# limacv/VideoLoop3D

Hardware: AMD Instinct MI355X
Metric: rendered Mpix/s (fwd+bwd) D=32 planes 720p (higher is better)
Workload: dtype f32; 1 GPU; cfg3 stage-2 MPV render fwd+bwd: D=32 planes, T=50 frames, 720x1280, mpv convention, plane stack (D,T,H,W,4) f32 resident in HBM; parallelism=single GPU, variant=0

## Files before the change

### include/vl3d.h

```cpp
#ifndef VL3D_H
#define VL3D_H

#include <stdint.h>

#ifdef __cplusplus
extern "C" {
#endif

typedef void *vl3d_stream_t;

enum { VL3D_OK = 0, VL3D_EINVAL = 1, VL3D_ELAUNCH = 2, VL3D_EUNSUPPORTED = 3 };

enum { VL3D_ACT_NONE = 0, VL3D_ACT_SIGMOID = 1, VL3D_ACT_RELU = 2, VL3D_ACT_CLAMP = 3, VL3D_ACT_ABS = 4 };
enum { VL3D_COORD_UTILS_MPI = 0, VL3D_COORD_AFFINE = 1, VL3D_COORD_AFFINE_PLANES = 2 };
enum { VL3D_BORDER_ZEROS = 0, VL3D_BORDER_HARDCUT = 1 };
enum { VL3D_ACT_PRE = 0, VL3D_ACT_POST = 1, VL3D_ACT_BAKED = 2 };
enum { VL3D_F32 = 0, VL3D_F16 = 1, VL3D_U8 = 2 };

const char *vl3d_last_error(void);
int vl3d_version(void);

typedef struct vl3d_render_desc {
    int32_t D, T, Hs, Ws;
    int32_t H, W;
    int32_t row0, col0;
    int32_t coord_mode, border_mode, act_order, rgb_act, alpha_act;
    int32_t stack_dtype;
    float pixel_center;
    float sx, sy, ox, oy;
    int32_t variant;
    int32_t cull_row0, cull_col0, cull_Hs, cull_Ws;
    int32_t grad_flags;
    uint32_t uv_noise_seed;
} vl3d_render_desc;
enum { VL3D_GRAD_CULLED_UNWRITTEN = 1 };

int vl3d_render_fwd(const vl3d_render_desc *desc, const void *stack, const float *homos, const uint8_t *quad_keep, int32_t QH, int32_t QW,
                    void *cull_scratch, float *rgb, float *alpha, float *alpha_sums, vl3d_stream_t stream);
int vl3d_render_fwd_frames(const vl3d_render_desc *desc, const void *stack, int32_t frame0, int32_t T_alloc, const float *homos,
                           const uint8_t *quad_keep, int32_t QH, int32_t QW, void *cull_scratch, float *rgb, float *alpha,
                           vl3d_stream_t stream);

typedef struct vl3d_baked_frames {
    int32_t frame0;
    int32_t n_cams;
    const int32_t *frame_cam, *frame_t;
} vl3d_baked_frames;
typedef struct vl3d_baked_out {
    float *rgb, *alpha;
    uint8_t *frames;
    int32_t channels;
    const float *bg;
} vl3d_baked_out;
typedef struct vl3d_baked_times {
    int32_t n_cams;
    int32_t reserved;
    const int32_t *frame_cam;
    const float *frame_time;
} vl3d_baked_times;
int vl3d_bake_rgba8(int64_t n_texels, const void *stack, int32_t stack_dtype, int32_t rgb_act, int32_t alpha_act, uint8_t *out,
                    vl3d_stream_t stream);
int64_t vl3d_render_path_cull_scratch_bytes(const vl3d_render_desc *desc, int32_t n_cams);
int vl3d_render_fwd_baked(const vl3d_render_desc *desc, const uint8_t *baked, int32_t T_alloc, const float *homos,
                          const vl3d_baked_frames *sel, const uint8_t *quad_keep, int32_t QH, int32_t QW, void *cull_scratch,
                          const vl3d_baked_out *out, vl3d_stream_t stream);
int vl3d_render_fwd_baked_pool(const vl3d_render_desc *desc, const int32_t *blocks, const uint8_t *pool, int32_t T_model, const float *homos,
                               const vl3d_baked_frames *sel, const uint8_t *quad_keep, int32_t QH, int32_t QW, uint32_t culled_rgba8,
                               void *cull_scratch, const vl3d_baked_out *out, vl3d_stream_t stream);
int vl3d_render_fwd_baked_times(const vl3d_render_desc *desc, const uint8_t *baked, int32_t T_alloc, const float *homos,
                                const vl3d_baked_times *sel, const uint8_t *quad_keep, int32_t QH, int32_t QW, void *cull_scratch,
                                const vl3d_baked_out *out, vl3d_stream_t stream);
int vl3d_render_fwd_baked_pool_times(const vl3d_render_desc *desc, const int32_t *blocks, const uint8_t *pool, int32_t T_model,
                                     const float *homos, const vl3d_baked_times *sel, const uint8_t *quad_keep, int32_t QH, int32_t QW,
                                     uint32_t culled_rgba8, void *cull_scratch, const vl3d_baked_out *out, vl3d_stream_t stream);

int vl3d_pool_from_atlas_rgba8(int32_t D, int32_t T, int32_t Hs, int32_t Ws, int32_t th, int32_t tw, int32_t QH, int32_t QW,
                               const int32_t *blocks, const int32_t *tile_src, const uint8_t *static_atlas, int32_t As_h, int32_t As_w,
                               const uint8_t *dyn_atlas, int32_t Ad_h, int32_t Ad_w, int32_t frame, uint32_t culled_rgba8, uint8_t *pool,
                               vl3d_stream_t stream);

int64_t vl3d_baked_trim_scratch_bytes(int32_t D, int32_t Hs, int32_t Ws);
int vl3d_baked_trim_classify(int32_t D, int32_t T, int32_t Hs, int32_t Ws, const int32_t *blocks, const uint8_t *pool, int64_t n_slots,
                             uint32_t culled_rgba8, void *scratch, int64_t scratch_bytes, int32_t *block_slots, uint8_t *texel_class,
                             vl3d_stream_t stream);
int vl3d_baked_trim_move(int32_t D, int32_t T, int32_t Hs, int32_t Ws, const int32_t *blocks, const uint8_t *pool, int64_t n_slots,
                         const int32_t *new_blocks, uint8_t *new_pool, int64_t new_n_slots, vl3d_stream_t stream);

int64_t vl3d_render_bwd_scratch_bytes(const vl3d_render_desc *desc);
int vl3d_render_bwd(const vl3d_render_desc *desc, const void *stack, const float *homos, const uint8_t *quad_keep, int32_t QH, int32_t QW,
                    const float *rgb, const float *alpha, const float *grad_rgb, const float *grad_alpha, const float *grad_reg,
                    const void *reg_state, const float *grad_alpha_sums, float *grad_stack, void *scratch, int64_t scratch_bytes,
                    vl3d_stream_t stream);

enum { VL3D_BWD_ENTRY_RENDER = 0, VL3D_BWD_ENTRY_MASK = 1, VL3D_BWD_ENTRY_ADAM = 2 };
enum { VL3D_BWD_ATOMICS = 0, VL3D_BWD_TILE = 1, VL3D_BWD_PAIR = 2, VL3D_BWD_PAIR12 = 3 };
typedef struct vl3d_bwd_choice {
    int32_t family;
    int32_t width, rows;
    int32_t reg, mask, adam, cull, f16;
    int32_t owner4;
    int32_t gather9;
} vl3d_bwd_choice;
int vl3d_render_bwd_choice(const vl3d_render_desc *desc, int32_t entry, int32_t has_quad_keep, int32_t has_reg_grads, int64_t scratch_bytes,
                           int32_t fused_step, vl3d_bwd_choice *out);

int64_t vl3d_render_cull_scratch_bytes(const vl3d_render_desc *desc);

int vl3d_render_fwd_plane_rows(const vl3d_render_desc *desc, const void *stack, const int32_t *plane_row0, int32_t R, const float *homos,
                               float *rgb, float *alpha, vl3d_stream_t stream);
int64_t vl3d_render_plane_rows_scratch_bytes(const vl3d_render_desc *desc, int32_t R);
int vl3d_render_bwd_plane_rows(const vl3d_render_desc *desc, const void *stack, const int32_t *plane_row0, int32_t R, const float *homos,
                               const float *rgb, const float *alpha, const float *grad_rgb, const float *grad_alpha, void *grad_stack,
                               void *scratch, int64_t scratch_bytes, vl3d_stream_t stream);

int vl3d_tie_static_grad(int32_t D, int32_t T, int32_t Hs, int32_t Ws, const uint8_t *quad_keep, const uint8_t *quad_dyn,
                         int32_t QH, int32_t QW, float *grad, int32_t mode, vl3d_stream_t stream);

int vl3d_adam_step_tiles(int32_t D, int32_t T, int32_t Hs, int32_t Ws, const uint8_t *quad_keep, const uint8_t *quad_dyn, int32_t QH, int32_t QW,
                         float *param, const float *grad, float *exp_avg, float *exp_avg_sq, float lr, float beta1, float beta2,
                         float eps, int64_t step, vl3d_stream_t stream);

int32_t vl3d_adam_window_tile(void);
typedef struct vl3d_adam_window {
    int32_t D, T;
    int32_t Hs, Ws;
    int32_t y0, x0, wh, ww;
    float *param, *exp_avg, *exp_avg_sq;
    int32_t *last_step;
    const float *hist;
    float lr, beta1, beta2, eps;
    int64_t step;
    const int32_t *plane_boxes;
    void *boxes_scratch;
    const uint8_t *quad_keep, *quad_dyn;
    int32_t QH, QW;
    void *class_scratch;
    const int32_t *blocks;
} vl3d_adam_window;
int vl3d_adam_window_catchup(const vl3d_adam_window *w, int32_t upto, float *compact, float culled_alpha, int32_t mirror_static,
                             vl3d_stream_t stream);
int vl3d_adam_window_step(const vl3d_adam_window *w, const float *grad_compact, int32_t static_tied, vl3d_stream_t stream);
int vl3d_adam_flush_older(const vl3d_adam_window *w, int32_t upto, int32_t min_depth, vl3d_stream_t stream);
void vl3d_adam_step_scalars(float lr, float beta1, float beta2, int64_t step, float *lr_bc1, float *bc2s);

int64_t vl3d_render_bwd_adam_class_bytes(const vl3d_render_desc *desc);
int vl3d_render_bwd_adam(const vl3d_render_desc *desc, const void *stack, const float *homos, const float *rgb, const float *alpha,
                         const float *grad_rgb, const float *grad_alpha, const float *grad_reg, const void *reg_state,
                         const float *grad_alpha_sums, float *grad_stack, void *scratch, int64_t scratch_bytes,
                         const vl3d_adam_window *adam, vl3d_stream_t stream);

int vl3d_packed_unpack_frames(int32_t D, int32_t T, int32_t Hs, int32_t Ws, const int32_t *blocks, const float *pool, int32_t n,
                              const int32_t *frames, float culled_alpha, float *out, vl3d_stream_t stream);
int vl3d_render_fwd_packed(const vl3d_render_desc *desc, const int32_t *blocks, const float *pool, const int32_t *frames, int32_t n,
                           const float *homos, const uint8_t *quad_keep, int32_t QH, int32_t QW, float culled_alpha, float *rgb,
                           float *alpha, vl3d_stream_t stream);

int64_t vl3d_render_reg_state_bytes(const vl3d_render_desc *desc);
int vl3d_render_reg_fwd(const vl3d_render_desc *desc, const void *stack, const float *homos, const uint8_t *quad_keep, int32_t QH, int32_t QW,
                        double *sums, void *reg_state, vl3d_stream_t stream);
int vl3d_render_fwd_reg(const vl3d_render_desc *desc, const void *stack, const float *homos, const uint8_t *quad_keep, int32_t QH, int32_t QW,
                        float *rgb, float *alpha, float *alpha_sums, double *sums, void *reg_state, vl3d_stream_t stream);

int vl3d_render_fwd_mask(const vl3d_render_desc *desc, const void *stack, const float *mask, const float *homos, float *rgb,
                         float *alpha, float *label, float *alpha_sums, double *sums, void *reg_state, vl3d_stream_t stream);
int vl3d_render_bwd_mask(const vl3d_render_desc *desc, const void *stack, const float *mask, const float *homos, const float *rgb,
                         const float *alpha, const float *grad_rgb, const float *grad_alpha, const float *grad_label,
                         const float *grad_reg, const void *reg_state, const float *grad_alpha_sums, float *grad_stack,
                         float *grad_mask, void *scratch, int64_t scratch_bytes, vl3d_stream_t stream);

int vl3d_label_noise_fwd(const vl3d_render_desc *desc, const float *stack, const float *mask, const float *homos, float *label, vl3d_stream_t stream);
int vl3d_label_noise_bwd(const vl3d_render_desc *desc, const float *stack, const float *mask, const float *homos, const float *grad_label,
                         float *grad_mask, vl3d_stream_t stream);

int vl3d_warp_fwd(int32_t N, int32_t C, int32_t Hs, int32_t Ws, int32_t h, int32_t w,
                  const float *homos, const float *images, float *out, vl3d_stream_t stream);
int vl3d_warp_bwd(int32_t N, int32_t C, int32_t Hs, int32_t Ws, int32_t h, int32_t w,
                  const float *homos, const float *grad_out, float *grad_images, vl3d_stream_t stream);

int vl3d_overcompose_fwd(int64_t P, int32_t D, int32_t C, const float *alpha, const float *content,
                         float *rgb, float *blendweight, vl3d_stream_t stream);
int vl3d_overcompose_bwd(int64_t P, int32_t D, int32_t C, const float *alpha, const float *content,
                         const float *grad_rgb, const float *grad_bw,
                         float *grad_alpha, float *grad_content, vl3d_stream_t stream);

int vl3d_overcompose_nto0_fwd(int32_t B, int32_t D, int32_t C, int64_t HW,
                              const float *alpha, int64_t a_sb, int64_t a_sd,
                              const float *content, int64_t c_sb, int64_t c_sd, int64_t c_sc,
                              float *rgb, float *trans, vl3d_stream_t stream);
int vl3d_overcompose_nto0_bwd(int32_t B, int32_t D, int32_t C, int64_t HW,
                              const float *alpha, int64_t a_sb, int64_t a_sd,
                              const float *content, int64_t c_sb, int64_t c_sd, int64_t c_sc,
                              const float *grad_rgb, float *grad_alpha, float *grad_content,
                              vl3d_stream_t stream);

typedef struct vl3d_loss_desc {
    int32_t Tx, Ty, H, W;
    int32_t ps, pt, stride, stridet;
    int32_t use_alpha;
    float alpha;
    int64_t x_sc, x_st, x_sr;
    int64_t y_sc, y_st, y_sr;
    int32_t variant;
} vl3d_loss_desc;

int64_t vl3d_patchnn_scratch_bytes(const vl3d_loss_desc *desc);

enum { VL3D_NN_ENTRY_PLAIN = 0, VL3D_NN_ENTRY_PREPARED = 1, VL3D_NN_ENTRY_GRAMS = 2 };
enum { VL3D_NN_LAYOUT_GRAM16 = 1, VL3D_NN_LAYOUT_PIXEL_MAJOR = 2 };
typedef struct vl3d_nn_choice {
    int32_t kernel;
    int32_t tyt, nl, nw, xs, ch;
    int32_t runsum;
    int32_t threads;
    int32_t kc;
    int32_t lds_bytes;
    int32_t scratch_layout;
} vl3d_nn_choice;
int vl3d_patchnn_choice(const vl3d_loss_desc *desc, int32_t entry, int32_t has_scratch, int32_t x_pitch, int32_t x_frames, int32_t y_pitch,
                        vl3d_nn_choice *out);
typedef struct vl3d_fold_choice {
    int32_t staged;
    int32_t shape;
    int32_t fw, fh, threads;
    int32_t nb;
    int32_t lds_bytes;
} vl3d_fold_choice;
int vl3d_vote_fold_choice(const vl3d_loss_desc *desc, int32_t fused, vl3d_fold_choice *out);

int vl3d_patchnn(const vl3d_loss_desc *desc, const float *x, const float *y, int32_t *nn,
                 void *scratch, vl3d_stream_t stream);

int64_t vl3d_gram_major_bytes(int32_t T, int32_t H, int32_t W);
int vl3d_video_to_gram_major(const float *y, int64_t sc, int64_t st, int64_t sr, int32_t T, int32_t H, int32_t W, float *out,
                             vl3d_stream_t stream);
int vl3d_patchnn_prepared(const vl3d_loss_desc *desc, const float *x, const float *y_gram, int32_t y_pitch, int32_t y_rows,
                          int32_t y_row0, int32_t y_col0, int32_t *nn, void *scratch, vl3d_stream_t stream);
int vl3d_patchnn_grams(const vl3d_loss_desc *desc, const float *x_gram, int32_t x_pitch, int32_t x_rows, int32_t x_frames, const float *y_gram,
                       int32_t y_pitch, int32_t y_rows, int32_t y_row0, int32_t y_col0, int32_t *nn, vl3d_stream_t stream);

int vl3d_nn_vectors(int64_t B, int32_t n1, int32_t n2, int32_t d, const float *X, const float *Y,
                    int32_t use_alpha, float alpha, int64_t *nn, vl3d_stream_t stream);

int vl3d_vote_fold(const vl3d_loss_desc *desc, const float *y, const int32_t *nn,
                   float *sum, float *weight, int32_t normalize, vl3d_stream_t stream);

int vl3d_patch_l1(const vl3d_loss_desc *desc, const float *x, const float *y, const int32_t *nn, float *err,
                  vl3d_stream_t stream);

int vl3d_vote_fold_robust(const vl3d_loss_desc *desc, const float *y, const int32_t *nn, const float *x, int32_t rho_kind,
                          float rou, float scale, float *y2x, float *weight, float *grad_x, double *loss_sum,
                          vl3d_stream_t stream);

int vl3d_vote_fold_robust_strided(const vl3d_loss_desc *desc, const float *y, const int32_t *nn, const float *x, int32_t rho_kind,
                                  float rou, float scale, float *y2x, float *weight, float *grad_x, int64_t gx_sc, int64_t gx_st,
                                  int64_t gx_sr, double *loss_sum, vl3d_stream_t stream);

int vl3d_scale_inplace(int64_t n, float *x, const float *scale, vl3d_stream_t stream);

int vl3d_loop_gain(int32_t T, int32_t F, int32_t h, int32_t w, const float *rgb, const float *res, double *log_sum, vl3d_stream_t stream);
int vl3d_loop_gain_strided(int32_t T, int32_t F, int32_t h, int32_t w, const float *rgb, const float *res, int64_t r_sf, int64_t r_sc, int64_t r_sr,
                           double *log_sum, vl3d_stream_t stream);
int vl3d_loop_pad_fwd(int32_t T, int32_t pad, int32_t h, int32_t w, const float *rgb, const double *log_sum, float *x, vl3d_stream_t stream);
int vl3d_loop_pad_fwd_gram(int32_t T, int32_t pad, int32_t h, int32_t w, const float *rgb, const double *log_sum, float *x, float *x_gram,
                           vl3d_stream_t stream);
int vl3d_loop_pad_bwd(int32_t T, int32_t pad, int32_t h, int32_t w, const float *grad_x, int64_t gx_sc, int64_t gx_st, const double *log_sum,
                      float *grad_rgb, vl3d_stream_t stream);

int vl3d_pixel_terms(int64_t n, const float *alpha, const float *alpha_sums, float eps, double *sums, float *grad_alpha_sums, float *grad_alpha,
                     vl3d_stream_t stream);

int vl3d_stage1_loss(int32_t B, int32_t C, int32_t h, int32_t w, const float *rgbl, int64_t sb, int64_t sc, int64_t sp, const float *target,
                     const float *target_mask, int32_t scale_invariant, double *log_sum, double *sums, float *grad, vl3d_stream_t stream);

typedef struct vl3d_stage1_objective_desc {
    int32_t B, h, w;
    int32_t scale_invariant;
    float w_img, w_loop, w_sparsity, w_density, w_rgb_smooth, w_a_smooth;
    float sparsity_scale, eps;
    float smooth_coef[4];
} vl3d_stage1_objective_desc;
int vl3d_stage1_objective(const vl3d_stage1_objective_desc *desc, const float *rgb, const float *label, const float *alpha, const float *alpha_sums,
                          const float *smooth_sums, const float *target, int64_t t_sb, int64_t t_sc, int64_t t_sr, const float *target_mask,
                          int64_t m_sb, int64_t m_sr, double *scratch, float *out, float *grad_rgb,
                          float *grad_label, float *grad_alpha, float *grad_alpha_sums, float *grad_smooth, vl3d_stream_t stream);

int vl3d_linear_head_fwd(int32_t n, uint64_t groups, int32_t ngroups, const float *main_term, const float *rest, const float *coef, float *out,
                         vl3d_stream_t stream);
int vl3d_linear_head_bwd(int32_t n, const float *coef, const float *grad_total, float *grad_terms, vl3d_stream_t stream);

enum { VL3D_RHO_MSE = 0, VL3D_RHO_ABS = 1, VL3D_RHO_BARRON = 2 };
int vl3d_robust_fwd(int64_t n, const float *x, const float *y2x, int32_t kind, float rou, float scale,
                    double *loss_sum, vl3d_stream_t stream);
int vl3d_robust_bwd(int64_t n, const float *x, const float *y2x, int32_t kind, float rou, float scale,
                    const float *grad_out, float inv_n, float *grad_x, vl3d_stream_t stream);

typedef struct vl3d_eval_desc {
    int32_t F, T;
    int32_t row0, col0, h, w;
    int64_t gt_sf, gt_sr;
    int64_t pred_sf, pred_sr;
} vl3d_eval_desc;
int64_t vl3d_eval_scratch_bytes(const vl3d_eval_desc *desc);
int vl3d_eval_view(const vl3d_eval_desc *desc, const uint8_t *gt, const uint8_t *pred, const uint8_t *mask, int64_t mask_ones,
                   int64_t *sse, double *ssim_sum, int32_t *gt_min, double *dyn_sum, void *scratch, vl3d_stream_t stream);

#ifdef __cplusplus
}
#endif
#endif
```

### videoloop3d_amd/csrc/vl3d_render.hip

```cpp
#include <string>
#include "vl3d_render_args.h"

using namespace vl3d_render_detail;

namespace {

typedef int (*ConvFn)(bool, const vl3d_render_desc *, const RenderArgs &, hipStream_t);
ConvFn conv_of(const vl3d_render_desc *d) {
    const int c = d->coord_mode, b = d->border_mode, o = d->act_order;
    if (c == VL3D_COORD_UTILS_MPI && b == VL3D_BORDER_ZEROS && o == VL3D_ACT_PRE) return conv_utils_zeros_pre;
    if (c == VL3D_COORD_UTILS_MPI && b == VL3D_BORDER_ZEROS && o == VL3D_ACT_POST) return conv_utils_zeros_post;
    if (c == VL3D_COORD_UTILS_MPI && b == VL3D_BORDER_HARDCUT && o == VL3D_ACT_PRE) return conv_utils_hardcut_pre;
    if (c == VL3D_COORD_AFFINE_PLANES && b == VL3D_BORDER_HARDCUT && o == VL3D_ACT_POST) return conv_affine_planes_hardcut_post;
    if (c == VL3D_COORD_AFFINE && b == VL3D_BORDER_HARDCUT && o == VL3D_ACT_POST)
        return (d->rgb_act == VL3D_ACT_SIGMOID && d->alpha_act == VL3D_ACT_SIGMOID) ? conv_affine_hardcut_post_sig : conv_affine_hardcut_post_other;
    if (o == VL3D_ACT_BAKED) {
        if (c == VL3D_COORD_AFFINE && b == VL3D_BORDER_HARDCUT && d->rgb_act == VL3D_ACT_SIGMOID && d->alpha_act == VL3D_ACT_SIGMOID)
            return conv_affine_hardcut_baked;
        vl3d_set_error("unsupported with act_order VL3D_ACT_BAKED: built is (affine, hardcut, baked) with sigmoid / sigmoid activations, fp32 and fp16 stacks");
        return nullptr;
    }
    vl3d_set_error("unsupported (coord_mode, border_mode, act_order): built are (utils_mpi, zeros, pre|post), (utils_mpi, hardcut, pre), "
                   "(affine, hardcut, post), (affine, hardcut, baked)");
    return nullptr;
}
int dispatch(bool bwd, const vl3d_render_desc *d, const RenderArgs &a, hipStream_t s) {
    const ConvFn conv = conv_of(d);
    return conv ? conv(bwd, d, a, s) : VL3D_EUNSUPPORTED;
}

int check_desc(const vl3d_render_desc *d) {
    VL3D_REQUIRE(d != nullptr, "null render desc");
    if (vl3d_check_variant(d->variant) != VL3D_OK) return VL3D_EINVAL;
    VL3D_REQUIRE(d->D > 0 && d->T > 0 && d->Hs > 0 && d->Ws > 0 && d->H > 0 && d->W > 0, "non-positive render dims");
    VL3D_REQUIRE((int64_t)d->Hs * d->Ws < (1ll << 31), "plane too large for 32-bit texel index");
    VL3D_REQUIRE(d->Hs < (1 << 24) && d->Ws < (1 << 24), "plane side too large (24-bit row arithmetic)");
    VL3D_REQUIRE(d->stack_dtype == VL3D_F32 || d->stack_dtype == VL3D_F16, "stack_dtype must be VL3D_F32 or VL3D_F16");
    VL3D_REQUIRE(d->coord_mode != VL3D_COORD_AFFINE_PLANES || (d->sx == 1.0f && d->sy == 1.0f && d->ox == 0.0f && d->oy == 0.0f),
                 "VL3D_COORD_AFFINE_PLANES: the texel transforms live in the per-plane records (sx = sy = 1, ox = oy = 0)");
    VL3D_REQUIRE(d->stack_dtype == VL3D_F32 || (d->rgb_act == VL3D_ACT_SIGMOID && d->alpha_act == VL3D_ACT_SIGMOID),
                 "fp16 plane stacks are implemented for the shipped (sigmoid, sigmoid) activations only");
    VL3D_REQUIRE(d->stack_dtype == VL3D_F32 || d->Ws >= 2, "fp16 plane stacks need Ws >= 2");
    VL3D_REQUIRE(d->uv_noise_seed == 0 || (d->border_mode == VL3D_BORDER_HARDCUT && d->coord_mode != VL3D_COORD_UTILS_MPI),
                 "uv_noise_seed (add_uv_noise, MPV.py:420-423) belongs to the planar MPV / MPI convention: affine coordinates, VL3D_BORDER_HARDCUT");
    return VL3D_OK;
}

int check_cull(const vl3d_render_desc *desc, const uint8_t *quad_keep, int32_t QH, int32_t QW, const char *who) {
    if (!quad_keep) return VL3D_OK;
    if (desc->coord_mode == VL3D_COORD_AFFINE_PLANES) return refuse(who, "tile culling is not available with per-plane texel transforms");
    const int rc = check_cull_grid(desc, QH, QW, who);
    if (rc != VL3D_OK) return rc;
    if (!(QH > 0 || (desc->coord_mode == VL3D_COORD_AFFINE && desc->border_mode == VL3D_BORDER_HARDCUT)))
        return refuse(who, "tile-exact layout: the planar MPV / MPI convention only (VL3D_COORD_AFFINE, VL3D_BORDER_HARDCUT)");
    return VL3D_OK;
}

}

extern "C" int64_t vl3d_render_cull_scratch_bytes(const vl3d_render_desc *desc) {
    if (!desc || desc->H <= 0 || desc->W <= 0) return 0;
    return (int64_t)((desc->W + 63) / 64) * ((desc->H + 3) / 4) * 16;
}

static int64_t owner_table_off(const vl3d_render_desc *desc) {
    const int64_t b = (int64_t)plan_win_off(desc->D) * sizeof(float) + bwd_max_tiles(desc->H, desc->W) * desc->D * 16;
    return (b + 255) & ~(int64_t)255;
}

extern "C" int64_t vl3d_render_bwd_scratch_bytes(const vl3d_render_desc *desc) {
    if (!desc || desc->D <= 0 || desc->H <= 0 || desc->W <= 0) return 0;
    return owner_table_off(desc) + ((int64_t)desc->D * desc->Hs * desc->Ws + 16 * (int64_t)desc->Ws + 64) * 2;
}

static void set_reg_state(RenderArgs &a, const vl3d_render_desc *d, const void *reg_state);
static int check_mask_desc(const vl3d_render_desc *d, const char *who);
static int check_adam_desc(const vl3d_render_desc *desc, bool has_quad_map);

static void set_bwd_io(RenderArgs &a, const vl3d_render_desc *desc, const void *stack, const float *homos, const float *rgb, const float *alpha,
                       const float *grad_rgb, const float *grad_alpha, const float *grad_reg, const void *reg_state, const float *grad_alpha_sums,
                       float *grad_stack) {
    if (grad_reg) set_reg_state(a, desc, reg_state);
    a.stack = (const float *)stack; a.homos = homos;
    a.rgb = const_cast<float *>(rgb); a.alpha = const_cast<float *>(alpha);
    a.g_rgb = grad_rgb; a.g_alpha = grad_alpha; a.g_reg = grad_reg; a.g_asum = grad_alpha_sums; a.g_stack = grad_stack;
}
static void set_bwd_setting(RenderArgs &a, const vl3d_render_desc *desc, const BwdSetting &set, void *scratch) {
    a.bwd_policy = set.policy; a.gather9 = set.gather9; a.owner4 = set.owner4;
    if (set.policy == BWD_NONE) return;
    a.plan = (const float *)scratch;
    a.owner = reinterpret_cast<const unsigned short *>(reinterpret_cast<const char *>(scratch) + owner_table_off(desc));
}
static bool bwd_tile_ok(const vl3d_render_desc *desc, int64_t scratch_bytes) {
    return scratch_bytes >= vl3d_render_bwd_scratch_bytes(desc) && desc->uv_noise_seed == 0;
}

extern "C" int vl3d_render_bwd_choice(const vl3d_render_desc *desc, int32_t entry, int32_t has_quad_keep, int32_t has_reg_grads,
                                      int64_t scratch_bytes, int32_t fused_step, vl3d_bwd_choice *out) {
    int rc = check_desc(desc);
    if (rc != VL3D_OK) return rc;
    VL3D_REQUIRE(out != nullptr, "vl3d_render_bwd_choice: null out");
    VL3D_REQUIRE(entry >= VL3D_BWD_ENTRY_RENDER && entry <= VL3D_BWD_ENTRY_ADAM && (fused_step != 0) == (entry == VL3D_BWD_ENTRY_ADAM),
                 "vl3d_render_bwd_choice: entry is VL3D_BWD_ENTRY_RENDER, _MASK or _ADAM, and fused_step names the last");
    if (entry == VL3D_BWD_ENTRY_MASK) {
        rc = check_mask_desc(desc, "vl3d_render_bwd_mask");
        if (rc != VL3D_OK) return rc;
        VL3D_REQUIRE(!has_quad_keep && desc->uv_noise_seed == 0, "vl3d_render_bwd_mask: dense models without add_uv_noise");
    }
    if (entry == VL3D_BWD_ENTRY_ADAM) {
        rc = check_adam_desc(desc, has_quad_keep != 0);
        if (rc != VL3D_OK) return rc;
        VL3D_REQUIRE(desc->uv_noise_seed == 0 && scratch_bytes >= vl3d_render_bwd_scratch_bytes(desc),
                     "vl3d_render_bwd_adam: no add_uv_noise, scratch of vl3d_render_bwd_scratch_bytes()");
    }
    if (!conv_of(desc)) return VL3D_EUNSUPPORTED;
    VL3D_REQUIRE(!has_quad_keep || desc->coord_mode != VL3D_COORD_AFFINE_PLANES, "tile culling is not available with per-plane texel transforms");
    static const float present = 0.0f;
    const bool adam = entry == VL3D_BWD_ENTRY_ADAM, qk = has_quad_keep != 0;
    RenderArgs a = render_args_of(desc);
    a.g_reg = has_reg_grads ? &present : nullptr;
    a.mask = entry == VL3D_BWD_ENTRY_MASK ? &present : nullptr;
    a.ad.p = adam ? reinterpret_cast<float4 *>(const_cast<float *>(&present)) : nullptr;
    a.quad_keep = qk ? reinterpret_cast<const unsigned char *>(&present) : nullptr;
    a.g_f16 = desc->stack_dtype == VL3D_F16;
    a.grad_culled_unwritten = (qk && (adam || (desc->grad_flags & VL3D_GRAD_CULLED_UNWRITTEN))) ? 1 : 0;
    const BwdSetting set = bwd_setting_of(entry, desc->variant & 0xf, bwd_tile_ok(desc, scratch_bytes), qk);
    a.bwd_policy = set.policy; a.gather9 = set.gather9; a.owner4 = set.owner4;
    const bool planes = desc->coord_mode == VL3D_COORD_AFFINE_PLANES;
    const BwdFacts f = bwd_facts_of(a, planes ? VL3D_COORD_AFFINE : desc->coord_mode, desc->border_mode, desc->act_order, desc->rgb_act, desc->alpha_act,
                                    a.g_f16 != 0, planes ? 16 : 9);
    const BwdChoice c = choose_bwd(f);
    const bool none = c.family == VL3D_BWD_ATOMICS;
    *out = vl3d_bwd_choice{c.family, none ? 0 : BWD_REGIONS[c.shape].width, none ? 0 : BWD_REGIONS[c.shape].rows,
                           c.reg, c.mask, c.adam, c.cull, c.f16, c.owner4, f.set.gather9};
    return VL3D_OK;
}

struct RegLayout { int64_t masks, signs, patch, total; };
static RegLayout reg_layout(const vl3d_render_desc *d) {
    auto up = [](int64_t v) { return (v + 255) & ~(int64_t)255; };
    const int64_t px = (int64_t)d->H * d->W, words = (int64_t)((d->D + 3) / 4) * d->T * px * 8;
    RegLayout l;
    l.masks = up(px);
    l.signs = l.masks + up(px * 16);
    l.patch = l.signs + up(words);
    l.total = l.patch + up(words);
    return l;
}
static void set_reg_state(RenderArgs &a, const vl3d_render_desc *d, const void *reg_state) {
    char *b = reinterpret_cast<char *>(const_cast<void *>(reg_state));
    const RegLayout l = reg_layout(d);
    a.reg_flags = reinterpret_cast<unsigned char *>(b);
    a.reg_masks = reinterpret_cast<unsigned long long *>(b + l.masks);
    a.reg_signs = reinterpret_cast<unsigned short *>(b + l.signs);
    a.reg_patch = reinterpret_cast<unsigned short *>(b + l.patch);
}
extern "C" int64_t vl3d_render_reg_state_bytes(const vl3d_render_desc *desc) {
    if (!desc || desc->D <= 0 || desc->T <= 0 || desc->H <= 0 || desc->W <= 0) return 0;
    return reg_layout(desc).total;
}

static int check_mask_desc(const vl3d_render_desc *d, const char *who) {
    if (d->coord_mode == VL3D_COORD_AFFINE && d->border_mode == VL3D_BORDER_HARDCUT && d->act_order == VL3D_ACT_POST &&
        d->rgb_act == VL3D_ACT_SIGMOID && d->alpha_act == VL3D_ACT_SIGMOID && d->stack_dtype == VL3D_F32)
        return VL3D_OK;
    vl3d_set_error((std::string(who) + ": the loop-mask channel is built for the planar convention stage 1 ships -- (affine, hardcut, post), "
                   "sigmoid / sigmoid, fp32 stack (MPI.py:452-594); render the label in a pass of its own otherwise").c_str());
    return VL3D_EUNSUPPORTED;
}

enum FwdEntry { FWD, FWD_FRAMES, FWD_REG, REG_FWD, FWD_MASK };

static int render_fwd(FwdEntry e, const char *who, const vl3d_render_desc *desc, const void *stack, const float *mask, int32_t frame0,
                      int32_t T_alloc, const float *homos, const uint8_t *quad_keep, int32_t QH, int32_t QW, void *cull_scratch, float *rgb,
                      float *alpha, float *label, float *alpha_sums, double *sums, void *reg_state, vl3d_stream_t stream) {
    int rc = check_desc(desc);
    if (rc != VL3D_OK) return rc;
    const bool plain = e == FWD || e == FWD_FRAMES;
    const bool image = e != REG_FWD;
    if (e == FWD_MASK) {
        rc = check_mask_desc(desc, who);
        if (rc != VL3D_OK) return rc;
        if (!(mask && label)) return refuse(who, "null pointer");
        if (desc->uv_noise_seed != 0)
            return refuse(who, "add_uv_noise jitters the colour samples only (MPI.py:519-522, 568-572): render the label in a pass of its own");
        if ((sums == nullptr) != (reg_state == nullptr)) return refuse(who, "sums and reg_state come together (both NULL: no layer regularisers)");
    }
    const bool reg = e == FWD_REG || e == REG_FWD || (e == FWD_MASK && sums);
    if (!(stack && homos && (!image || (rgb && alpha)) && (!reg || (sums && reg_state)))) return refuse(who, "null pointer");
    if (reg && desc->D > 128) return refuse(who, "the layer regularisers support at most 128 planes (coverage masks)");
    if (!quad_keep) { QH = QW = 0; cull_scratch = nullptr; }
    rc = check_cull(desc, quad_keep, QH, QW, who);
    if (rc != VL3D_OK) return rc;
    if (plain && quad_keep && !cull_scratch) return refuse(who, "tile culling: the forward needs vl3d_render_cull_scratch_bytes() of scratch");
    if (!((int64_t)desc->Hs * desc->Ws * 16 < (1ll << 32))) return refuse(who, "frame too large for 32-bit byte offsets");
    RenderArgs a = render_args_of(desc);
    a.stack = (const float *)stack; a.homos = homos; a.rgb = rgb; a.alpha = alpha; a.asum = alpha_sums;
    a.mask = mask; a.label = label;
    a.quad_keep = quad_keep;
    set_cull_geometry(a, desc, QH, QW);
    if (plain) a.cull_masks = (const unsigned long long *)cull_scratch;
    if (plain || e == FWD_MASK) a.fwd_variant = (desc->variant >> 8) & 0xf;
    if (plain) a.ablate = (desc->variant >> 4) & 0xf;
    a.g_f16 = desc->stack_dtype == VL3D_F16;
    if (reg) {
        a.reg_sums = sums;
        set_reg_state(a, desc, reg_state);
        a.reg_fwd = e == REG_FWD ? 1 : (quad_keep ? 3 : 2);
    }
    if (e == FWD_FRAMES) {
        if (T_alloc <= 0) return refuse(who, "T_alloc must be the clip length of the stack allocation");
        if (!(frame0 >= 0 && frame0 + desc->T <= T_alloc)) return refuse(who, "the run of frames leaves the clip");
        a.stack = reinterpret_cast<const float *>(reinterpret_cast<const char *>(stack) + (size_t)frame0 * desc->Hs * desc->Ws * (a.g_f16 ? 8 : 16));
        a.Tstride = T_alloc;
    }
    rc = dispatch(false, desc, a, (hipStream_t)stream);
    if (rc != VL3D_OK) return rc;
    VL3D_CHECK_LAUNCH();
    return VL3D_OK;
}

extern "C" int vl3d_render_fwd(const vl3d_render_desc *desc, const void *stack, const float *homos, const uint8_t *quad_keep, int32_t QH,
                               int32_t QW, void *cull_scratch, float *rgb, float *alpha, float *alpha_sums, vl3d_stream_t stream) {
    return render_fwd(FWD, "vl3d_render_fwd", desc, stack, nullptr, 0, 0, homos, quad_keep, QH, QW, cull_scratch, rgb, alpha, nullptr, alpha_sums,
                      nullptr, nullptr, stream);
}

extern "C" int vl3d_render_fwd_frames(const vl3d_render_desc *desc, const void *stack, int32_t frame0, int32_t T_alloc, const float *homos,
                                      const uint8_t *quad_keep, int32_t QH, int32_t QW, void *cull_scratch, float *rgb, float *alpha,
                                      vl3d_stream_t stream) {
    return render_fwd(FWD_FRAMES, "vl3d_render_fwd_frames", desc, stack, nullptr, frame0, T_alloc, homos, quad_keep, QH, QW, cull_scratch, rgb,
                      alpha, nullptr, nullptr, nullptr, nullptr, stream);
}

extern "C" int vl3d_render_fwd_reg(const vl3d_render_desc *desc, const void *stack, const float *homos, const uint8_t *quad_keep, int32_t QH,
                                   int32_t QW, float *rgb, float *alpha, float *alpha_sums, double *sums, void *reg_state,
                                   vl3d_stream_t stream) {
    return render_fwd(FWD_REG, "vl3d_render_fwd_reg", desc, stack, nullptr, 0, 0, homos, quad_keep, QH, QW, nullptr, rgb, alpha, nullptr,
                      alpha_sums, sums, reg_state, stream);
}

extern "C" int vl3d_render_reg_fwd(const vl3d_render_desc *desc, const void *stack, const float *homos, const uint8_t *quad_keep, int32_t QH,
                                   int32_t QW, double *sums, void *reg_state, vl3d_stream_t stream) {
    return render_fwd(REG_FWD, "vl3d_render_reg_fwd", desc, stack, nullptr, 0, 0, homos, quad_keep, QH, QW, nullptr, nullptr, nullptr, nullptr,
                      nullptr, sums, reg_state, stream);
}

extern "C" int vl3d_render_fwd_mask(const vl3d_render_desc *desc, const void *stack, const float *mask, const float *homos, float *rgb,
                                    float *alpha, float *label, float *alpha_sums, double *sums, void *reg_state, vl3d_stream_t stream) {
    return render_fwd(FWD_MASK, "vl3d_render_fwd_mask", desc, stack, mask, 0, 0, homos, nullptr, 0, 0, nullptr, rgb, alpha, label, alpha_sums,
                      sums, reg_state, stream);
}

extern "C" int vl3d_render_bwd_mask(const vl3d_render_desc *desc, const void *stack, const float *mask, const float *homos, const float *rgb,
                                    const float *alpha, const float *grad_rgb, const float *grad_alpha, const float *grad_label,
                                    const float *grad_reg, const void *reg_state, const float *grad_alpha_sums, float *grad_stack,
                                    float *grad_mask, void *scratch, int64_t scratch_bytes, vl3d_stream_t stream) {
    int rc = check_desc(desc);
    if (rc != VL3D_OK) return rc;
    rc = check_mask_desc(desc, "vl3d_render_bwd_mask");
    if (rc != VL3D_OK) return rc;
    VL3D_REQUIRE(stack && mask && homos && rgb && alpha && grad_rgb && grad_label && grad_stack && grad_mask, "null pointer passed to vl3d_render_bwd_mask");
    VL3D_REQUIRE(!grad_reg || reg_state, "vl3d_render_bwd_mask: grad_reg needs the reg_state the forward with regularisers filled");
    VL3D_REQUIRE((int64_t)desc->Hs * desc->Ws * 16 < (1ll << 32), "frame too large for 32-bit byte offsets");
    RenderArgs a = render_args_of(desc);
    set_bwd_io(a, desc, stack, homos, rgb, alpha, grad_rgb, grad_alpha, grad_reg, reg_state, grad_alpha_sums, grad_stack);
    a.mask = mask; a.g_label = grad_label; a.g_mask = grad_mask;
    VL3D_REQUIRE(desc->uv_noise_seed == 0, "vl3d_render_bwd_mask: add_uv_noise jitters the colour samples only (MPI.py:519-522, 568-572): render the label in a pass of its own");
    const BwdSetting set = bwd_setting_of(VL3D_BWD_ENTRY_MASK, desc->variant & 0xf, bwd_tile_ok(desc, scratch ? scratch_bytes : 0), false);
    set_bwd_setting(a, desc, set, scratch);
    if (set.policy == BWD_NONE) {
        const size_t texels = (size_t)desc->D * desc->T * desc->Hs * desc->Ws;
        VL3D_HIP(hipMemsetAsync(grad_stack, 0, texels * 16, (hipStream_t)stream));
        VL3D_HIP(hipMemsetAsync(grad_mask, 0, texels * 4, (hipStream_t)stream));
    }
    rc = dispatch(true, desc, a, (hipStream_t)stream);
    if (rc != VL3D_OK) return rc;
    VL3D_CHECK_LAUNCH();
    return VL3D_OK;
}

extern "C" int vl3d_render_bwd(const vl3d_render_desc *desc, const void *stack, const float *homos, const uint8_t *quad_keep, int32_t QH,
                               int32_t QW, const float *rgb, const float *alpha, const float *grad_rgb, const float *grad_alpha,
                               const float *grad_reg, const void *reg_state, const float *grad_alpha_sums, float *grad_stack, void *scratch,
                               int64_t scratch_bytes, vl3d_stream_t stream) {
    int rc = check_desc(desc);
    if (rc != VL3D_OK) return rc;
    if (!quad_keep) QH = QW = 0;
    rc = check_cull(desc, quad_keep, QH, QW, "vl3d_render_bwd");
    if (rc != VL3D_OK) return rc;
    VL3D_REQUIRE(stack && homos && rgb && alpha && grad_rgb && grad_stack, "vl3d_render_bwd: null pointer");
    VL3D_REQUIRE(!grad_reg || reg_state, "vl3d_render_bwd: grad_reg needs the reg_state the forward with regularisers filled");
    RenderArgs a = render_args_of(desc);
    set_bwd_io(a, desc, stack, homos, rgb, alpha, grad_rgb, grad_alpha, grad_reg, reg_state, grad_alpha_sums, grad_stack);
    a.quad_keep = quad_keep;
    set_cull_geometry(a, desc, QH, QW);
    a.g_f16 = desc->stack_dtype == VL3D_F16;
    a.grad_culled_unwritten = (quad_keep && (desc->grad_flags & VL3D_GRAD_CULLED_UNWRITTEN)) ? 1 : 0;
    a.ablate = (desc->variant >> 4) & 0xf;
    const BwdSetting set = bwd_setting_of(VL3D_BWD_ENTRY_RENDER, desc->variant & 0xf, bwd_tile_ok(desc, scratch ? scratch_bytes : 0), quad_keep != nullptr);
    set_bwd_setting(a, desc, set, scratch);
    if (set.policy == BWD_NONE) {
        const size_t bytes = (size_t)desc->D * desc->T * desc->Hs * desc->Ws * (desc->stack_dtype == VL3D_F16 ? 8 : 16);
        VL3D_HIP(hipMemsetAsync(grad_stack, 0, bytes, (hipStream_t)stream));
    }
    rc = dispatch(true, desc, a, (hipStream_t)stream);
    if (rc != VL3D_OK) return rc;
    VL3D_CHECK_LAUNCH();
    return VL3D_OK;
}

extern "C" int64_t vl3d_render_bwd_adam_class_bytes(const vl3d_render_desc *desc) {
    if (!desc || desc->D <= 0 || desc->Hs <= 0 || desc->Ws <= 0) return 0;
    return ((int64_t)desc->D * desc->Hs * desc->Ws + 16 * (int64_t)desc->Ws + 64) * 8;
}

static int check_adam_desc(const vl3d_render_desc *desc, bool has_quad_map) {
    const int bv = desc->variant & 0xf;
    if (!(desc->coord_mode == VL3D_COORD_AFFINE && desc->border_mode == VL3D_BORDER_HARDCUT && desc->act_order == VL3D_ACT_POST &&
          desc->rgb_act == VL3D_ACT_SIGMOID && desc->alpha_act == VL3D_ACT_SIGMOID && desc->stack_dtype == VL3D_F32 &&
          (has_quad_map ? (bv == 0 || bv == 3 || bv == 5) : (desc->T >= 2 && bv == 0)))) {
        vl3d_set_error("vl3d_render_bwd_adam: built for the stage-2 iteration -- (affine, hardcut, post), sigmoid / sigmoid, fp32 stack, "
                       "T >= 2 and variant 0 for a dense model; use vl3d_render_bwd + vl3d_adam_window_step otherwise");
        return VL3D_EUNSUPPORTED;
    }
    return VL3D_OK;
}

static vl3d_adam_epilogue adam_epilogue_of(const vl3d_adam_window &w) {
    const int ts = vl3d_adam::TS;
    const float2 sc = vl3d_adam::adam_step_scalars(w.lr, w.beta1, w.beta2, w.step);
    vl3d_adam_epilogue e{};
    e.p = reinterpret_cast<float4 *>(w.param); e.m = reinterpret_cast<float4 *>(w.exp_avg); e.v = reinterpret_cast<float4 *>(w.exp_avg_sq);
    e.last_step = w.last_step;
    e.boxes = (w.plane_boxes && w.D <= 128) ? reinterpret_cast<const int4 *>(w.boxes_scratch) : nullptr;
    e.y0 = w.y0; e.x0 = w.x0; e.Hs = w.Hs; e.Ws = w.Ws;
    e.tiles_y = (w.Hs + ts - 1) / ts; e.tiles_x = (w.Ws + ts - 1) / ts;
    e.step = (int)w.step;
    e.lr_bc1 = sc.x; e.beta1 = w.beta1; e.beta2 = w.beta2; e.eps = w.eps; e.bc2s = sc.y;
    e.quad_dyn = w.quad_keep ? w.quad_dyn : nullptr;
    e.cls = w.quad_keep ? reinterpret_cast<uint2 *>(w.class_scratch) : nullptr;
    e.blocks = w.blocks;
    return e;
}

extern "C" int vl3d_render_bwd_adam(const vl3d_render_desc *desc, const void *stack, const float *homos, const float *rgb, const float *alpha,
                                    const float *grad_rgb, const float *grad_alpha, const float *grad_reg, const void *reg_state,
                                    const float *grad_alpha_sums, float *grad_stack, void *scratch, int64_t scratch_bytes,
                                    const vl3d_adam_window *adam, vl3d_stream_t stream) {
    int rc = check_desc(desc);
    if (rc != VL3D_OK) return rc;
    VL3D_REQUIRE(adam != nullptr, "vl3d_render_bwd_adam: null adam window");
    if (desc->uv_noise_seed) {
        vl3d_set_error("vl3d_render_bwd_adam: add_uv_noise takes the atomics backward (vl3d_render_bwd + vl3d_adam_window_step)");
        return VL3D_EUNSUPPORTED;
    }
    VL3D_REQUIRE(stack && homos && rgb && alpha && grad_rgb && grad_stack && scratch, "null pointer passed to vl3d_render_bwd_adam");
    VL3D_REQUIRE(!grad_reg || reg_state, "vl3d_render_bwd_adam: grad_reg needs the reg_state the forward with regularisers filled");
    const uint8_t *qk = adam->quad_keep;
    rc = check_adam_desc(desc, qk != nullptr);
    if (rc != VL3D_OK) return rc;
    VL3D_REQUIRE(scratch_bytes >= vl3d_render_bwd_scratch_bytes(desc), "vl3d_render_bwd_adam: scratch smaller than vl3d_render_bwd_scratch_bytes()");
    VL3D_REQUIRE(adam->param && adam->exp_avg && adam->exp_avg_sq && adam->last_step && adam->hist && adam->step >= 1 &&
                     adam->step < (1ll << 31), "vl3d_render_bwd_adam: null pointer / bad step in the adam window");
    VL3D_REQUIRE((int64_t)desc->Hs * desc->Ws * 16 < (1ll << 32) && (int64_t)adam->Hs * adam->Ws * 16 < (1ll << 32),
                 "frame too large for 32-bit byte offsets");
    if (qk) {
        rc = check_cull(desc, qk, adam->QH, adam->QW, "vl3d_render_bwd_adam");
        if (rc != VL3D_OK) return rc;
        VL3D_REQUIRE(adam->class_scratch, "vl3d_render_bwd_adam: a tile-culled model needs class_scratch (vl3d_render_bwd_adam_class_bytes())");
        VL3D_REQUIRE(adam->step < (1ll << 29), "vl3d_render_bwd_adam: tile-culled models keep the step in 29 bits of the texel records");
    } else {
        VL3D_REQUIRE(!adam->blocks, "vl3d_render_bwd_adam: the packed layout belongs to a tile-culled model (quad maps)");
    }
    if (qk) {
        VL3D_REQUIRE(desc->cull_Hs == adam->Hs && desc->cull_Ws == adam->Ws && desc->cull_row0 == adam->y0 && desc->cull_col0 == adam->x0,
                     "vl3d_render_bwd_adam: desc->cull_* must name the optimiser's window (y0, x0) of its (Hs, Ws) planes");
    }
    VL3D_REQUIRE(adam->D == desc->D && adam->T == desc->T && adam->wh == desc->Hs && adam->ww == desc->Ws,
                 "vl3d_render_bwd_adam: the adam window's D, T, wh, ww must be desc->D, desc->T, desc->Hs, desc->Ws (the stack is the window's compact copy)");
    hipStream_t s = (hipStream_t)stream;
    rc = vl3d_adam_window_before_render(*adam, s);
    if (rc != VL3D_OK) return rc;
    RenderArgs a = render_args_of(desc);
    set_bwd_io(a, desc, stack, homos, rgb, alpha, grad_rgb, grad_alpha, grad_reg, reg_state, grad_alpha_sums, grad_stack);
    a.quad_keep = qk; a.QH = adam->QH; a.QW = adam->QW;
    set_cull_geometry(a, desc, adam->QH, adam->QW);
    a.grad_culled_unwritten = qk ? 1 : 0;
    set_bwd_setting(a, desc, bwd_setting_of(VL3D_BWD_ENTRY_ADAM, desc->variant & 0xf, true, qk != nullptr), scratch);
    a.ad = adam_epilogue_of(*adam);
    rc = dispatch(true, desc, a, s);
// ... 4 lines not shown
```

### videoloop3d_amd/csrc/vl3d_render_core.h

```cpp
#pragma once
#include <stddef.h>
#include "vl3d_common.h"
#include "vl3d_bake_rule.h"

#include "vl3d_adam.h"
#include "vl3d_render_bwd_choice.h"

#ifndef VL3D_HS
#define VL3D_HS 9
#define VL3D_HN 9
#endif

namespace vl3d_render_detail {

#ifndef VL3D_PAIR_MIN_WAVES
#define VL3D_PAIR_MIN_WAVES 4
#endif
#ifndef VL3D_FWD2X_MIN_WAVES
#define VL3D_FWD2X_MIN_WAVES 4
#endif

#ifdef VL3D_REG_ABLATE
#define VL3D_REGAB(bit) ((VL3D_REG_ABLATE & (bit)) != 0)
#else
// ... 246 lines not shown
template <> struct TapVal<true, VL3D_ACT_POST> { typedef u2 type; };

template <bool F16>
__device__ __forceinline__ void load_taps2(const char *__restrict__ plane, const Taps2 &t, TapStep st, u2 v[4]) {
    static_assert(F16, "packed taps are fp16 texels");
    const size_t o = (size_t)(t.off >> 1);
    typedef unsigned u4 __attribute__((ext_vector_type(4)));
    typedef u4 u4_a8 __attribute__((aligned(8)));
    const u4 r0 = *reinterpret_cast<const u4_a8 *>(plane + o);
    const u4 r1 = *reinterpret_cast<const u4_a8 *>(plane + st.dy + o);
    v[0] = u2{r0.x, r0.y}; v[1] = u2{r0.z, r0.w};
    v[2] = u2{r1.x, r1.y}; v[3] = u2{r1.z, r1.w};
}

template <int HI>
__device__ __forceinline__ float fma_mix(unsigned hpair, float w, float acc) {
    float r;
    if constexpr (HI) asm("v_fma_mix_f32 %0, %1, %2, %3 op_sel:[1,0,0] op_sel_hi:[1,0,0]" : "=v"(r) : "v"(hpair), "v"(w), "v"(acc));
    else asm("v_fma_mix_f32 %0, %1, %2, %3 op_sel:[0,0,0] op_sel_hi:[1,0,0]" : "=v"(r) : "v"(hpair), "v"(w), "v"(acc));
    return r;
}

__device__ __forceinline__ float dot3p(float a0, float b0, float a1, float b1, float a2, float b2, float c) {
    return fmaf(a0, b0, fmaf(a1, b1, fmaf(a2, b2, c)));
}

template <int RACT, int AACT>
__device__ __forceinline__ f4 act4(f4 s) {
    return f4{act_fwd<RACT>(s.x), act_fwd<RACT>(s.y), act_fwd<RACT>(s.z), act_fwd<AACT>(s.w)};
}

template <int RACT, int AACT>
__device__ __forceinline__ f4 baked4(f4 s) {
    return f4{(float)bake_channel(act_fwd<RACT>(s.x)), (float)bake_channel(act_fwd<RACT>(s.y)), (float)bake_channel(act_fwd<RACT>(s.z)),
              (float)bake_channel(act_fwd<AACT>(s.w))};
}

template <int ORDER, int RACT, int AACT>
__device__ __forceinline__ f4 shade2(const Taps2 &t, const f4 v[4], f4 *pre_out = nullptr) {
    f4 s;
    if constexpr (ORDER == VL3D_ACT_POST) {
        s = v[0] * t.w[0] + (v[1] * t.w[1] + (v[2] * t.w[2] + v[3] * t.w[3]));
        if (pre_out) *pre_out = s;
        s = act4<RACT, AACT>(s);
    } else if constexpr (ORDER == VL3D_ACT_BAKED) {
        const f4 w255 = t.w * (1.0f / 255.0f);
        s = baked4<RACT, AACT>(v[3]) * w255[3];
        s = __builtin_elementwise_fma(baked4<RACT, AACT>(v[2]), f4{w255[2], w255[2], w255[2], w255[2]}, s);
        s = __builtin_elementwise_fma(baked4<RACT, AACT>(v[1]), f4{w255[1], w255[1], w255[1], w255[1]}, s);
        s = __builtin_elementwise_fma(baked4<RACT, AACT>(v[0]), f4{w255[0], w255[0], w255[0], w255[0]}, s);
        if (pre_out) *pre_out = s;
    } else {
        s = act4<RACT, AACT>(v[0]) * t.w[0] + (act4<RACT, AACT>(v[1]) * t.w[1] + (act4<RACT, AACT>(v[2]) * t.w[2] + act4<RACT, AACT>(v[3]) * t.w[3]));
        if (pre_out) *pre_out = s;
    }
    s.w *= t.cov;
    return s;
}

template <int ORDER, int RACT, int AACT>
__device__ __forceinline__ f4 shade2(const Taps2 &t, const u2 v[4], f4 *pre_out = nullptr) {
    static_assert(ORDER == VL3D_ACT_POST, "packed taps: sample-then-activate only");
    f4 s;
    s.x = fma_mix<0>(v[0].x, t.w[0], fma_mix<0>(v[1].x, t.w[1], fma_mix<0>(v[2].x, t.w[2], fma_mix<0>(v[3].x, t.w[3], 0.0f))));
    s.y = fma_mix<1>(v[0].x, t.w[0], fma_mix<1>(v[1].x, t.w[1], fma_mix<1>(v[2].x, t.w[2], fma_mix<1>(v[3].x, t.w[3], 0.0f))));
    s.z = fma_mix<0>(v[0].y, t.w[0], fma_mix<0>(v[1].y, t.w[1], fma_mix<0>(v[2].y, t.w[2], fma_mix<0>(v[3].y, t.w[3], 0.0f))));
    s.w = fma_mix<1>(v[0].y, t.w[0], fma_mix<1>(v[1].y, t.w[1], fma_mix<1>(v[2].y, t.w[2], fma_mix<1>(v[3].y, t.w[3], 0.0f))));
    if (pre_out) *pre_out = s;
    s = act4<RACT, AACT>(s);
    s.w *= t.cov;
    return s;
}

__device__ __forceinline__ void load_mask_taps(const float *__restrict__ mplane, unsigned off16, TapStep st, float m[4]) {
    const char *b = reinterpret_cast<const char *>(mplane) + (size_t)(off16 >> 2);
    m[0] = *reinterpret_cast<const float *>(b);
    m[1] = *reinterpret_cast<const float *>(b + (st.dx >> 2));
    m[2] = *reinterpret_cast<const float *>(b + (st.dy >> 2));
    m[3] = *reinterpret_cast<const float *>(b + (st.dy >> 2) + (st.dx >> 2));
}
__device__ __forceinline__ float mask_blend(const float m[4], f4 w) { return m[0] * w[0] + (m[1] * w[1] + (m[2] * w[2] + m[3] * w[3])); }

__device__ __forceinline__ int xcd_remap(int b, int nb);
__device__ __forceinline__ int reg_sign(float v) {
    int r;
    asm("v_med3_i32 %0, %1, -1, 1" : "=v"(r) : "v"(__float_as_int(v)));
    return r;
}
__device__ __forceinline__ int reg_signs4(f4 diff) {
    return reg_sign(diff.x) + (reg_sign(diff.y) << 2) + (reg_sign(diff.z) << 4) + (reg_sign(diff.w) << 6);
}
constexpr int REG_BIAS = 0x55;
constexpr unsigned REG_ZERO = 0x5555u;
__device__ __forceinline__ f4 reg_grad(unsigned w_own, unsigned w_left, unsigned w_up, unsigned w_patch, unsigned fl, f4 gx, f4 gy) {
    const unsigned l = (fl & 4u) ? w_patch : w_left, u = (fl & 8u) ? (w_patch >> 8) : (w_up >> 8);
    const int ls = (fl & 4u) ? 1 : -1, us = (fl & 8u) ? 1 : -1, lo = (fl & 4u) ? -2 : 0, uo = (fl & 8u) ? -2 : 0;
    f4 r;
#pragma unroll
    for (int c = 0; c < 4; ++c) {
        const int ix = (int)__builtin_amdgcn_ubfe(w_own, 2 * c, 2) + ls * (int)__builtin_amdgcn_ubfe(l, 2 * c, 2) + lo;
        const int iy = (int)__builtin_amdgcn_ubfe(w_own, 8 + 2 * c, 2) + us * (int)__builtin_amdgcn_ubfe(u, 2 * c, 2) + uo;
        r[c] = fmaf(gy[c], (float)iy, gx[c] * (float)ix);
    }
    return r;
}

__device__ __forceinline__ f4 reg_grad32(unsigned w_own, unsigned w_left, unsigned w_up, unsigned w_patch, unsigned bo, unsigned fl, f4 gx, f4 gy) {
    f4 r;
    if (__builtin_expect((fl & 12u) == 0u, 1)) {
#pragma unroll
        for (int c = 0; c < 4; ++c) {
            const int ix = (int)__builtin_amdgcn_ubfe(w_own, bo + 2 * c, 2) - (int)__builtin_amdgcn_ubfe(w_left, bo + 2 * c, 2);
            const int iy = (int)__builtin_amdgcn_ubfe(w_own, bo + 8 + 2 * c, 2) - (int)__builtin_amdgcn_ubfe(w_up, bo + 8 + 2 * c, 2);
            r[c] = fmaf(gy[c], (float)iy, gx[c] * (float)ix);
        }
    } else {
        r = reg_grad((w_own >> bo) & 0xffffu, (w_left >> bo) & 0xffffu, (w_up >> bo) & 0xffffu, (w_patch >> bo) & 0xffffu, fl, gx, gy);
    }
    return r;
}

template <int COORD, int BORDER>
__global__ __launch_bounds__(256) void reg_masks_k(RenderArgs a) {
    if (blockIdx.x == 0 && blockIdx.y == 0 && threadIdx.x < 4 && a.reg_sums) a.reg_sums[threadIdx.x] = 0.0;
    const int x = blockIdx.x * 64 + (threadIdx.x & 63), y = blockIdx.y * 4 + (threadIdx.x >> 6);
    if (x >= a.W || y >= a.H) return;
    const float px = (float)(a.col0 + x) + a.pc, py = (float)(a.row0 + y) + a.pc;
    unsigned long long m0 = 0ull, m1 = 0ull;
    for (int d = 0; d < a.D; ++d) {
        float h[VL3D_HN];
        load_uniform(a.homos + VL3D_HS * d, h);
        const TapsI t = make_taps_i<COORD, BORDER>(h, px, py, a.Hs, a.Ws, a.sx, a.sy, a.ox, a.oy, plane_cull(a, d));
        if (t.cov > 0.0f) { if (d < 64) m0 |= 1ull << d; else m1 |= 1ull << (d - 64); }
    }
    a.reg_masks[2 * ((size_t)y * a.W + x)] = m0;
    a.reg_masks[2 * ((size_t)y * a.W + x) + 1] = m1;
}

__global__ __launch_bounds__(256) void reg_flags_k(RenderArgs a) {
    const int x = blockIdx.x * 64 + (threadIdx.x & 63), y = blockIdx.y * 4 + (threadIdx.x >> 6);
    if (x >= a.W || y >= a.H) return;
    const size_t p = (size_t)y * a.W + x;
    const unsigned long long *M = a.reg_masks;
    const unsigned long long m0 = M[2 * p], m1 = M[2 * p + 1];
    auto differs = [&](size_t q) { return M[2 * q] != m0 || M[2 * q + 1] != m1; };
    unsigned f = 0;
    if (x + 1 < a.W && differs(p + 1)) f |= 1u;
    if (y + 1 < a.H && differs(p + a.W)) f |= 2u;
    if (x >= 1 && differs(p - 1)) f |= 4u;
    if (y >= 1 && differs(p - a.W)) f |= 8u;
    a.reg_flags[p] = (unsigned char)f;
}

__device__ __forceinline__ int reg_pop_plane(unsigned long long &m0, unsigned long long &m1) {
    const bool lo = m0 != 0ull;
    const unsigned long long m = lo ? m0 : m1;
    if (!m) return -1;
    const int d = __builtin_ctzll(m) + (lo ? 0 : 64);
    const unsigned long long c = m & (m - 1);
    m0 = lo ? c : m0;
    m1 = lo ? m1 : c;
    return d;
}

template <int COORD, int BORDER, int ORDER, int RACT, int AACT, bool F16>
__device__ __forceinline__ f4 reg_sample(const RenderArgs &a, const float *hs, float px, float py, int d, int t) {
    float h[VL3D_HN];
#pragma unroll
    for (int i = 0; i < VL3D_HN; ++i) h[i] = hs[VL3D_HS * d + i];
    const Taps2 tp = make_taps2<COORD, BORDER>(h, px, py, a.Hs, a.Ws, a.sx, a.sy, a.ox, a.oy, plane_cull(a, d), UvNoise{a.uv_seed, d});
    const char *plane = reinterpret_cast<const char *>(a.stack) + ((size_t)d * a.T + t) * ((size_t)a.Hs * a.Ws * (F16 ? 8 : 16));
    typename TapVal<F16, ORDER>::type tv[4];
    load_taps2<F16>(plane, tp, make_tap_step<F16>(a.Hs, a.Ws), tv);
    return shade2<ORDER, RACT, AACT>(tp, tv) * tp.cov;
}

template <int COORD, int BORDER, int ORDER, int RACT, int AACT, bool F16, bool PATCH, bool RENDER = false>
__global__ __launch_bounds__(512) void reg_slot_fwd_k(RenderArgs a, int tiles_x, int tiles_y) {
    static_assert(!(PATCH && RENDER), "the composite rides the kernel that visits every covered plane of every pixel");
    constexpr int FW = 64, FH = 8, NT = FW * FH;
    __shared__ float4 s_v[2][NT];
    __shared__ int s_d[2][NT];
    __shared__ float red[4][FH];
    __shared__ int s_kmax;
    __shared__ float s_h[128 * VL3D_HS];
    for (int i = threadIdx.x; i < a.D * VL3D_HS; i += NT) s_h[i] = a.homos[i];
    const int b = xcd_remap(blockIdx.x, gridDim.x);
    const int tile_x = b % tiles_x, rest = b / tiles_x;
    const int tile_y = rest % tiles_y, t = rest / tiles_y;
    const int tid = threadIdx.x, lane = tid & 63, row = tid >> 6;
    const int x = tile_x * (FW - 1) + lane, y = tile_y * (FH - 1) + row;
    const bool inimg = (x < a.W) && (y < a.H);
    const bool owner = inimg && lane < FW - 1 && row < FH - 1;
    const size_t p = (size_t)min(y, a.H - 1) * a.W + min(x, a.W - 1);
    const unsigned fl = owner ? a.reg_flags[p] : 0u;
    if (PATCH && !__syncthreads_or((fl & 3u) != 0u)) return;
    const bool irr_r = (fl & 1u) != 0u, irr_d = (fl & 2u) != 0u;
    const bool own_r = owner && x + 1 < a.W && (!PATCH || irr_r), own_d = owner && y + 1 < a.H && (!PATCH || irr_d);
    unsigned long long m0 = inimg ? a.reg_masks[2 * p] : 0ull, m1 = inimg ? a.reg_masks[2 * p + 1] : 0ull;
    if (tid == 0) s_kmax = 0;
    __syncthreads();
    atomicMax(&s_kmax, __builtin_popcountll(m0) + __builtin_popcountll(m1));
    __syncthreads();
    const int kmax = s_kmax;
    const float px = (float)(a.col0 + min(x, a.W - 1)) + a.pc, py = (float)(a.row0 + min(y, a.H - 1)) + a.pc;
    const size_t plane_px = (size_t)a.T * a.H * a.W, fpix = ((size_t)t * a.H + min(y, a.H - 1)) * a.W + min(x, a.W - 1);
    unsigned long long *const sg64 = reinterpret_cast<unsigned long long *>(a.reg_signs);
    unsigned char *const patch8 = reinterpret_cast<unsigned char *>(a.reg_patch);
    float sxc = 0.f, syc = 0.f, sxa = 0.f, sya = 0.f;
    float Tr = 1.0f, cr = 0.f, cg = 0.f, cb = 0.f, A = 0.f, n1 = 0.f, n2 = 0.f;
    unsigned long long sgw = 0ull;
    int sgg = -1;
    for (int k = 0; k < kmax; ++k) {
        const int buf = k & 1;
        const int d = reg_pop_plane(m0, m1);
        f4 v = f4{0.f, 0.f, 0.f, 0.f};
        if (d >= 0) v = reg_sample<COORD, BORDER, ORDER, RACT, AACT, F16>(a, s_h, px, py, d, t);
        if constexpr (RENDER) {
            const float w = v.w * Tr;
            cr += w * v.x; cg += w * v.y; cb += w * v.z; A += w;
            n1 += v.w; n2 = fmaf(v.w, v.w, n2);
            Tr *= (1.0f - v.w);
        }
        s_v[buf][tid] = make_float4(v.x, v.y, v.z, v.w);
        s_d[buf][tid] = d;
        __syncthreads();
        int code = PATCH ? 0 : (int)REG_ZERO;
        if (own_r) {
            const float4 r = s_v[buf][tid + 1];
            const int dn = s_d[buf][tid + 1];
            if (d >= 0 || dn >= 0) {
                const f4 df = v - f4{r.x, r.y, r.z, r.w};
                sxc += fabsf(df.x) + fabsf(df.y) + fabsf(df.z);
                sxa += fabsf(df.w);
                const int c = reg_signs4(df);
                code += c;
                if (irr_r && dn >= 0)
                    patch8[((((size_t)(dn >> 2) * plane_px + fpix + 1) << 2) + (dn & 3)) * 2] = (unsigned char)(REG_BIAS - c);
            }
        }
        if (own_d) {
            const float4 r = s_v[buf][tid + FW];
            const int dn = s_d[buf][tid + FW];
            if (d >= 0 || dn >= 0) {
                const f4 df = v - f4{r.x, r.y, r.z, r.w};
                syc += fabsf(df.x) + fabsf(df.y) + fabsf(df.z);
                sya += fabsf(df.w);
                const int c = reg_signs4(df);
                code += c << 8;
                if (irr_d && dn >= 0)
                    patch8[((((size_t)(dn >> 2) * plane_px + fpix + a.W) << 2) + (dn & 3)) * 2 + 1] = (unsigned char)(REG_BIAS - c);
            }
        }
        if (owner && d >= 0) {
            if constexpr (PATCH) {
                if (code) {
                    unsigned short *w = a.reg_signs + ((((size_t)(d >> 2) * plane_px + fpix) << 2) + (d & 3));
                    *w = (unsigned short)((int)*w + code);
                }
            } else {
                if ((d >> 2) != sgg) {
                    if (sgg >= 0) sg64[(size_t)sgg * plane_px + fpix] = sgw;
                    sgg = d >> 2; sgw = 0ull;
                }
                sgw |= (unsigned long long)(unsigned)code << (16 * (d & 3));
            }
        }
    }
    if (!PATCH && owner && sgg >= 0) sg64[(size_t)sgg * plane_px + fpix] = sgw;
    if constexpr (RENDER) if (owner) {
        a.rgb[fpix * 3 + 0] = cr; a.rgb[fpix * 3 + 1] = cg; a.rgb[fpix * 3 + 2] = cb;
        a.alpha[fpix] = A;
        if (a.asum) { a.asum[fpix * 2 + 0] = n1; a.asum[fpix * 2 + 1] = n2; }
    }
    float v4[4] = {sxc, syc, sxa, sya};
#pragma unroll
    for (int k = 0; k < 4; ++k) {
#pragma unroll
        for (int off = 32; off > 0; off >>= 1) v4[k] += __shfl_down(v4[k], off, 64);
        if (lane == 0) red[k][row] = v4[k];
    }
    __syncthreads();
    if (tid < 4) {
        double sum = 0.0;
        for (int r = 0; r < FH; ++r) sum += (double)red[tid][r];
        if (sum != 0.0) atomicAdd(a.reg_sums + tid, sum);
    }
}

template <int COORD, int BORDER, int ORDER, int RACT, int AACT, bool F16>
void launch_reg_prepass(const RenderArgs &a, hipStream_t s) {
    const dim3 g((a.W + 63) / 64, (a.H + 3) / 4);
    hipLaunchKernelGGL((reg_masks_k<COORD, BORDER>), g, dim3(256), 0, s, a);
    hipLaunchKernelGGL(reg_flags_k, g, dim3(256), 0, s, a);
}
template <int COORD, int BORDER, int ORDER, int RACT, int AACT, bool F16, bool PATCH, bool RENDER = false>
void launch_reg_slots(const RenderArgs &a, hipStream_t s) {
    const int tx = (a.W + 62) / 63, ty = (a.H + 6) / 7;
    hipLaunchKernelGGL((reg_slot_fwd_k<COORD, BORDER, ORDER, RACT, AACT, F16, PATCH, RENDER>), dim3((unsigned)(tx * ty * a.T)), dim3(512), 0, s, a, tx, ty);
}

constexpr int TILE_X = 64, TILE_Y = 4;

template <int COORD, int BORDER, int ORDER, int RACT, int AACT, bool F16, bool MASK = false>
__global__ __launch_bounds__(TILE_X *TILE_Y) void render_bwd_k(RenderArgs a) {
    if (a.plan && reinterpret_cast<const int *>(a.plan)[0]) return;
    const int x = blockIdx.x * TILE_X + (threadIdx.x & (TILE_X - 1));
    const int y = blockIdx.y * TILE_Y + (threadIdx.x / TILE_X);
    const int t = blockIdx.z;
    if (x >= a.W || y >= a.H) return;
    const float px = (float)(a.col0 + x) + a.pc, py = (float)(a.row0 + y) + a.pc;
    constexpr size_t TEXB = F16 ? 8 : 16;
    const size_t frame = (size_t)a.Hs * a.Ws * 4;
    const size_t plane_stride = (size_t)a.T * frame;
    const char *plane = reinterpret_cast<const char *>(a.stack) + (size_t)t * a.Hs * a.Ws * TEXB;
    char *gplane = reinterpret_cast<char *>(a.g_stack) + (size_t)t * a.Hs * a.Ws * TEXB;
    const size_t pix = ((size_t)t * a.H + y) * a.W + x;
    const float Gr = a.g_rgb[pix * 3 + 0], Gg = a.g_rgb[pix * 3 + 1], Gb = a.g_rgb[pix * 3 + 2];
    const float gA = a.g_alpha ? a.g_alpha[pix] : 0.0f;
    const float S = dot3p(Gr, a.rgb[pix * 3 + 0], Gg, a.rgb[pix * 3 + 1], Gb, a.rgb[pix * 3 + 2], gA * a.alpha[pix]);
    const float gN1 = a.g_asum ? a.g_asum[pix * 2 + 0] : 0.0f, gN2 = a.g_asum ? 2.0f * a.g_asum[pix * 2 + 1] : 0.0f;
    const unsigned fl = a.g_reg ? a.reg_flags[(size_t)y * a.W + x] : 0u;
    float Tr = 1.0f, P = 0.0f;
    const TapStep st = make_tap_step<F16>(a.Hs, a.Ws), gst = make_tap_step<false>(a.Hs, a.Ws);
    const float gL = MASK ? a.g_label[pix] : 0.0f;
    const size_t mframe = (size_t)a.Hs * a.Ws;
    for (int d = 0; d < a.D; ++d, plane += (size_t)a.T * a.Hs * a.Ws * TEXB, gplane += (size_t)a.T * a.Hs * a.Ws * TEXB) {
        const Taps2 tp = make_taps2<COORD, BORDER>(a.homos + VL3D_HS * d, px, py, a.Hs, a.Ws, a.sx, a.sy, a.ox, a.oy, plane_cull(a, d), UvNoise{a.uv_seed, d});
        if (tp.cov == 0.0f) continue;
        typename TapVal<F16, ORDER>::type tv[4];
        f4 pre;
        load_taps2<F16>(plane, tp, st, tv);
        const f4 o = shade2<ORDER, RACT, AACT>(tp, tv, &pre);
        const float q = dot3p(Gr, o.x, Gg, o.y, Gb, o.z, gA);
        const float w = o.w * Tr;
        if constexpr (MASK) {
            float mt[4];
            load_mask_taps(a.mask + ((size_t)d * a.T + t) * mframe, tp.off, gst, mt);
            const float sm = act_fwd<VL3D_ACT_SIGMOID>(mask_blend(mt, tp.w));
            const float gm = gL * w * (sm * (1.0f - sm));
            float *gmp = a.g_mask + ((size_t)d * a.T + t) * mframe + (tp.off >> 4);
#pragma unroll
            for (int i = 0; i < 4; ++i)
                if (tp.w[i] != 0.0f) atomicAdd(gmp + ((i & 1) ? (gst.dx >> 4) : 0u) + ((i & 2) ? (gst.dy >> 4) : 0u), gm * tp.w[i]);
        }
        P = fmaf(w, q, P);
        const float om = 1.0f - o.w;
        const float behind = (om > 1e-12f) ? (S - P) * fast_rcp(om) : 0.0f;
        f4 go = f4{w * Gr, w * Gg, w * Gb, fmaf(Tr, q, -behind) + fmaf(gN2, o.w, gN1)};
        Tr *= om;
        if (a.g_reg) {
            const f4 gx = f4{a.g_reg[0], a.g_reg[0], a.g_reg[0], a.g_reg[2]}, gy = f4{a.g_reg[1], a.g_reg[1], a.g_reg[1], a.g_reg[3]};
            const size_t idx = (((((size_t)(d >> 2) * a.T + t) * a.H + y) * a.W + x) << 2) + (d & 3);
            const unsigned w_left = x >= 1 ? a.reg_signs[idx - 4] : REG_ZERO, w_up = y >= 1 ? a.reg_signs[idx - 4 * (size_t)a.W] : REG_ZERO;
            go += reg_grad(a.reg_signs[idx], w_left, w_up, (fl & 12u) ? a.reg_patch[idx] : 0u, fl, gx, gy);
        }
        if constexpr (ORDER == VL3D_ACT_POST)
            go = f4{go.x * act_bwd<RACT>(pre.x, o.x), go.y * act_bwd<RACT>(pre.y, o.y), go.z * act_bwd<RACT>(pre.z, o.z),
                    go.w * act_bwd<AACT>(pre.w, o.w)};
#pragma unroll
        for (int i = 0; i < 4; ++i) {
            if (tp.w[i] != 0.0f) {
                f4 c = go * tp.w[i];
                if constexpr (ORDER == VL3D_ACT_PRE || ORDER == VL3D_ACT_BAKED) {
                    const f4 sv = tv[i];
                    c = f4{c.x * act_bwd<RACT>(sv.x, act_fwd<RACT>(sv.x)), c.y * act_bwd<RACT>(sv.y, act_fwd<RACT>(sv.y)),
                           c.z * act_bwd<RACT>(sv.z, act_fwd<RACT>(sv.z)), c.w * act_bwd<AACT>(sv.w, act_fwd<AACT>(sv.w))};
                }
                atomic_add_grad_texel<F16>(gplane, (size_t)tp.off + ((i & 1) ? gst.dx : 0u) + ((i & 2) ? gst.dy : 0u), c);
            }
        }
    }
}

__device__ __forceinline__ int xcd_remap(int b, int nb) {
    const int q = nb >> 3, r = nb & 7, xcd = b & 7, k = b >> 3;
    return (xcd < r ? xcd * (q + 1) : r * (q + 1) + (xcd - r) * q) + k;
}

template <int COORD, bool CAMS = false>
__global__ __launch_bounds__(256) void cull_fwd_plan_k(RenderArgs a, int TY, int tiles_x, int tiles_y, unsigned long long *masks) {
    const int i = blockIdx.x * 256 + threadIdx.x;
    if (i >= tiles_x * tiles_y * a.D) return;
    const int d = i % a.D, tile = i / a.D, tile_x = tile % tiles_x, tile_y = tile / tiles_x;
    const int x0 = tile_x * 64, x1 = min(x0 + 63, a.W - 1), y0 = tile_y * TY, y1 = min(y0 + TY - 1, a.H - 1);
    const float *h = a.homos + VL3D_HS * d;
    if constexpr (CAMS) {
        h += (size_t)blockIdx.y * a.D * VL3D_HS;
        masks += (size_t)blockIdx.y * tiles_x * tiles_y * 2;
    }
    float tnx = 1e30f, txx = -1e30f, tny = 1e30f, txy = -1e30f;
    for (int c = 0; c < 4; ++c) {
        const float cx = (float)a.col0 + a.pc + (float)((c & 1) ? x1 : x0), cy = (float)a.row0 + a.pc + (float)((c & 2) ? y1 : y0);
        const float X = h[0] * cx + h[1] * cy + h[2], Y = h[3] * cx + h[4] * cy + h[5], Z = h[6] * cx + h[7] * cy + h[8];
        const float ctx = texel_coord<COORD>(X / Z, (float)a.Ws / 2.0f, (float)(a.Ws - 1), a.sx, a.ox);
        const float cty = texel_coord<COORD>(Y / Z, (float)a.Hs / 2.0f, (float)(a.Hs - 1), a.sy, a.oy);
        tnx = fminf(tnx, ctx); txx = fmaxf(txx, ctx); tny = fminf(tny, cty); txy = fmaxf(txy, cty);
    }
    if (box_touches_kept_quad(a, d, tnx, txx, tny, txy)) atomicOr(masks + (size_t)tile * 2 + (d >> 6), 1ull << (d & 63));
}

template <int COORD>
void launch_cull_fwd_plan(const RenderArgs &a, int TY, int tiles_x, int tiles_y, hipStream_t s) {
    auto *masks = const_cast<unsigned long long *>(a.cull_masks);
    (void)hipMemsetAsync(masks, 0, (size_t)tiles_x * tiles_y * 16, s);
    const int n = tiles_x * tiles_y * a.D;
    hipLaunchKernelGGL((cull_fwd_plan_k<COORD>), dim3((n + 255) / 256), dim3(256), 0, s, a, TY, tiles_x, tiles_y, masks);
}
template <int COORD>
void launch_cull_fwd_plan_cams(const RenderArgs &a, int n_cams, int TY, int tiles_x, int tiles_y, hipStream_t s) {
    auto *masks = const_cast<unsigned long long *>(a.cull_masks);
    (void)hipMemsetAsync(masks, 0, (size_t)n_cams * tiles_x * tiles_y * 16, s);
    const int n = tiles_x * tiles_y * a.D;
    hipLaunchKernelGGL((cull_fwd_plan_k<COORD, true>), dim3((n + 255) / 256, n_cams), dim3(256), 0, s, a, TY, tiles_x, tiles_y, masks);
}

struct PlaneList {
    unsigned long long m0, m1;
    __device__ __forceinline__ PlaneList(const unsigned long long *cull_masks, int tile) {
        typedef const __attribute__((address_space(4))) unsigned long long *cu64_p;
        const cu64_p mk = (cu64_p)(cull_masks + (size_t)tile * 2);
        m0 = mk[0]; m1 = mk[1];
    }
    __device__ __forceinline__ int next() {
        int d = -1;
        if (m0) { d = __builtin_ctzll(m0); m0 &= m0 - 1; }
        else if (m1) { d = 64 + __builtin_ctzll(m1); m1 &= m1 - 1; }
        return d;
    }
};

template <int COORD, int BORDER, int ORDER, int RACT, int AACT, int TY, bool SWZ, bool F16, bool CULL = false, bool MASK = false>
__global__ __launch_bounds__(64 * TY) void render_fwd2_k(RenderArgs a, int tiles_x, int tiles_y) {
    static_assert(!(MASK && (CULL || F16)), "the loop-mask channel: dense fp32 stage-1 stacks");
    int b = blockIdx.x;
    if constexpr (SWZ) b = xcd_remap(b, gridDim.x);
    const int tile_x = b % tiles_x, rest = b / tiles_x;
    const int tile_y = rest % tiles_y, t = rest / tiles_y;
    const int x = tile_x * 64 + (threadIdx.x & 63);
    const int y = tile_y * TY + (threadIdx.x >> 6);
    if (x >= a.W || y >= a.H) return;
    const float px = (float)(a.col0 + x) + a.pc, py = (float)(a.row0 + y) + a.pc;
    const size_t frame_b = (size_t)a.Hs * a.Ws * (F16 ? 8 : 16);
    const size_t plane_stride_b = (size_t)a.Tstride * frame_b;
    const char *plane = reinterpret_cast<const char *>(a.stack) + (size_t)t * frame_b;
    float Tr = 1.0f, cr = 0.f, cg = 0.f, cb = 0.f, A = 0.f, n1 = 0.f, n2 = 0.f;
    const TapStep st = make_tap_step<F16>(a.Hs, a.Ws);
    typedef typename TapVal<F16, ORDER>::type tapv_t;
    tapv_t vA[4], vB[4];
    float mA[4] = {0.f, 0.f, 0.f, 0.f}, mB[4] = {0.f, 0.f, 0.f, 0.f}, lab = 0.f;
    const float *mplane = MASK ? a.mask + (size_t)t * a.Hs * a.Ws : nullptr;
    const size_t mplane_stride = (size_t)a.T * a.Hs * a.Ws;
#define VL3D_COMPOSITE(T_, V_, M_)                                    \
    {                                                                 \
        const f4 o = shade2<ORDER, RACT, AACT>(T_, V_);               \
        const float w = o.w * Tr;                                     \
        cr += w * o.x; cg += w * o.y; cb += w * o.z; A += w;          \
        n1 += o.w; n2 = fmaf(o.w, o.w, n2);                           \
        Tr *= (1.0f - o.w);                                           \
        if constexpr (MASK) lab = fmaf(w, act_fwd<VL3D_ACT_SIGMOID>(mask_blend(M_, T_.w)), lab);      \
    }
    if constexpr (CULL) {
        PlaneList list(a.cull_masks, tile_y * tiles_x + tile_x);
        auto fetch = [&](int d, Taps2 &t, tapv_t *v) {
            float h[VL3D_HN];
            load_uniform(a.homos + VL3D_HS * d, h);
            t = make_taps2<COORD, BORDER>(h, px, py, a.Hs, a.Ws, a.sx, a.sy, a.ox, a.oy, plane_cull(a, d), UvNoise{a.uv_seed, d});
            load_taps2<F16>(plane + (size_t)d * plane_stride_b, t, st, v);
            asm volatile("" ::: "memory");
        };
        int dA = list.next();
        if (dA >= 0) {
            Taps2 tA, tB;
            fetch(dA, tA, vA);
            for (;;) {
                const int dB = list.next();
                fetch(dB < 0 ? dA : dB, tB, vB);
                VL3D_COMPOSITE(tA, vA, mA)
                if (dB < 0) break;
                const int dC = list.next();
                fetch(dC < 0 ? dB : dC, tA, vA);
                VL3D_COMPOSITE(tB, vB, mB)
                if (dC < 0) break;
                dA = dC;
            }
        }
    } else {
    const QuadCull noq = QuadCull{nullptr, 0, 0, 0.f, 0.f, 0.f, 0.f, 0};
    Taps2 tA = make_taps2<COORD, BORDER>(a.homos, px, py, a.Hs, a.Ws, a.sx, a.sy, a.ox, a.oy, noq, UvNoise{a.uv_seed, 0}), tB = tA;
    load_taps2<F16>(plane, tA, st, vA);
    if constexpr (MASK) load_mask_taps(mplane, tA.off, st, mA);
    for (int d = 0;; d += 2) {
        {
            const int dn = min(d + 1, a.D - 1);
            float h[VL3D_HN];
            load_uniform(a.homos + VL3D_HS * dn, h);
            tB = make_taps2<COORD, BORDER>(h, px, py, a.Hs, a.Ws, a.sx, a.sy, a.ox, a.oy, noq, UvNoise{a.uv_seed, dn});
            load_taps2<F16>(plane + (size_t)dn * plane_stride_b, tB, st, vB);
            if constexpr (MASK) load_mask_taps(mplane + (size_t)dn * mplane_stride, tB.off, st, mB);
            asm volatile("" ::: "memory");
        }
        VL3D_COMPOSITE(tA, vA, mA)
        if (d + 1 >= a.D) break;
        {
            const int dn = min(d + 2, a.D - 1);
            float h[VL3D_HN];
            load_uniform(a.homos + VL3D_HS * dn, h);
            tA = make_taps2<COORD, BORDER>(h, px, py, a.Hs, a.Ws, a.sx, a.sy, a.ox, a.oy, noq, UvNoise{a.uv_seed, dn});
            load_taps2<F16>(plane + (size_t)dn * plane_stride_b, tA, st, vA);
            if constexpr (MASK) load_mask_taps(mplane + (size_t)dn * mplane_stride, tA.off, st, mA);
            asm volatile("" ::: "memory");
        }
        VL3D_COMPOSITE(tB, vB, mB)
        if (d + 2 >= a.D) break;
    }
    }
#undef VL3D_COMPOSITE
    const size_t pix = ((size_t)t * a.H + y) * a.W + x;
    a.rgb[pix * 3 + 0] = cr; a.rgb[pix * 3 + 1] = cg; a.rgb[pix * 3 + 2] = cb;
    a.alpha[pix] = A;
    if (a.asum) { a.asum[pix * 2 + 0] = n1; a.asum[pix * 2 + 1] = n2; }
    if constexpr (MASK) a.label[pix] = lab;
}

template <int COORD, int BORDER, int ORDER, int RACT, int AACT, int TY, bool F16, bool CULL = false>
__global__ __launch_bounds__(64 * TY, VL3D_FWD2X_MIN_WAVES) void render_fwd2x_k(RenderArgs a, int tiles_x, int tiles_y) {
    const int b = xcd_remap(blockIdx.x, gridDim.x);
    const int tile_x = b % tiles_x, rest = b / tiles_x;
    const int tile_y = rest % tiles_y, t0 = (rest / tiles_y) * 2;
    const bool has1 = t0 + 1 < a.T;
    const int x = tile_x * 64 + (threadIdx.x & 63);
    const int y = tile_y * TY + (threadIdx.x >> 6);
    if (x >= a.W || y >= a.H) return;
    const float px = (float)(a.col0 + x) + a.pc, py = (float)(a.row0 + y) + a.pc;
    const size_t frame_b = (size_t)a.Hs * a.Ws * (F16 ? 8 : 16);
    const size_t plane_stride_b = (size_t)a.Tstride * frame_b;
    const char *plane0 = reinterpret_cast<const char *>(a.stack) + (size_t)t0 * frame_b;
    const char *plane1 = plane0 + (has1 ? frame_b : 0);
    float Tr0 = 1.0f, cr0 = 0.f, cg0 = 0.f, cb0 = 0.f, A0 = 0.f, n10 = 0.f, n20 = 0.f;
    float Tr1 = 1.0f, cr1 = 0.f, cg1 = 0.f, cb1 = 0.f, A1 = 0.f, n11 = 0.f, n21 = 0.f;
    const TapStep st = make_tap_step<F16>(a.Hs, a.Ws);
    typedef typename TapVal<F16, ORDER>::type tapv_t;
    tapv_t vA0[4], vA1[4], vB0[4], vB1[4];
#define VL3D_COMPOSITE2(T_, V0_, V1_)                                        \
    {                                                                        \
        const f4 o0 = shade2<ORDER, RACT, AACT>(T_, V0_);                    \
        const f4 o1 = shade2<ORDER, RACT, AACT>(T_, V1_);                    \
        const float w0 = o0.w * Tr0, w1 = o1.w * Tr1;                        \
        cr0 += w0 * o0.x; cg0 += w0 * o0.y; cb0 += w0 * o0.z; A0 += w0;      \
        cr1 += w1 * o1.x; cg1 += w1 * o1.y; cb1 += w1 * o1.z; A1 += w1;      \
        n10 += o0.w; n20 = fmaf(o0.w, o0.w, n20);                            \
        n11 += o1.w; n21 = fmaf(o1.w, o1.w, n21);                            \
        Tr0 *= (1.0f - o0.w); Tr1 *= (1.0f - o1.w);                          \
    }
    if constexpr (CULL) {
        PlaneList list(a.cull_masks, tile_y * tiles_x + tile_x);
        auto fetch = [&](int d, Taps2 &t, tapv_t *v0, tapv_t *v1) {
            float h[VL3D_HN];
            load_uniform(a.homos + VL3D_HS * d, h);
            t = make_taps2<COORD, BORDER>(h, px, py, a.Hs, a.Ws, a.sx, a.sy, a.ox, a.oy, plane_cull(a, d));
            load_taps2<F16>(plane0 + (size_t)d * plane_stride_b, t, st, v0);
            load_taps2<F16>(plane1 + (size_t)d * plane_stride_b, t, st, v1);
            asm volatile("" ::: "memory");
        };
        int dA = list.next();
        if (dA >= 0) {
            Taps2 tA, tB;
            fetch(dA, tA, vA0, vA1);
            for (;;) {
                const int dB = list.next();
                fetch(dB < 0 ? dA : dB, tB, vB0, vB1);
                VL3D_COMPOSITE2(tA, vA0, vA1)
                if (dB < 0) break;
                const int dC = list.next();
                fetch(dC < 0 ? dB : dC, tA, vA0, vA1);
                VL3D_COMPOSITE2(tB, vB0, vB1)
                if (dC < 0) break;
                dA = dC;
            }
        }
    } else {
    Taps2 tA = make_taps2<COORD, BORDER>(a.homos, px, py, a.Hs, a.Ws, a.sx, a.sy, a.ox, a.oy), tB = tA;
    load_taps2<F16>(plane0, tA, st, vA0);
    load_taps2<F16>(plane1, tA, st, vA1);
    for (int d = 0;; d += 2) {
        {
            const int dn = min(d + 1, a.D - 1);
            float h[VL3D_HN];
            load_uniform(a.homos + VL3D_HS * dn, h);
            tB = make_taps2<COORD, BORDER>(h, px, py, a.Hs, a.Ws, a.sx, a.sy, a.ox, a.oy);
            load_taps2<F16>(plane0 + (size_t)dn * plane_stride_b, tB, st, vB0);
            load_taps2<F16>(plane1 + (size_t)dn * plane_stride_b, tB, st, vB1);
            asm volatile("" ::: "memory");
        }
        VL3D_COMPOSITE2(tA, vA0, vA1)
        if (d + 1 >= a.D) break;
        {
            const int dn = min(d + 2, a.D - 1);
            float h[VL3D_HN];
            load_uniform(a.homos + VL3D_HS * dn, h);
            tA = make_taps2<COORD, BORDER>(h, px, py, a.Hs, a.Ws, a.sx, a.sy, a.ox, a.oy);
            load_taps2<F16>(plane0 + (size_t)dn * plane_stride_b, tA, st, vA0);
            load_taps2<F16>(plane1 + (size_t)dn * plane_stride_b, tA, st, vA1);
            asm volatile("" ::: "memory");
        }
        VL3D_COMPOSITE2(tB, vB0, vB1)
        if (d + 2 >= a.D) break;
    }
    }
#undef VL3D_COMPOSITE2
    size_t pix = ((size_t)t0 * a.H + y) * a.W + x;
    a.rgb[pix * 3 + 0] = cr0; a.rgb[pix * 3 + 1] = cg0; a.rgb[pix * 3 + 2] = cb0;
    a.alpha[pix] = A0;
    if (a.asum) { a.asum[pix * 2 + 0] = n10; a.asum[pix * 2 + 1] = n20; }
    if (has1) {
        pix += (size_t)a.H * a.W;
        a.rgb[pix * 3 + 0] = cr1; a.rgb[pix * 3 + 1] = cg1; a.rgb[pix * 3 + 2] = cb1;
        a.alpha[pix] = A1;
        if (a.asum) { a.asum[pix * 2 + 0] = n11; a.asum[pix * 2 + 1] = n21; }
    }
}

struct Taps2R {
    Taps2 u, l;
    unsigned off2;
    bool own;
};
template <int COORD, int BORDER, int ORDER, int RACT, int AACT>
__global__ __launch_bounds__(512, 4) void render_fwd2r_k(RenderArgs a, int tiles_x, int tiles_y) {
    const int b = xcd_remap(blockIdx.x, gridDim.x);
    const int tile_x = b % tiles_x, rest = b / tiles_x;
    const int tile_y = rest % tiles_y, t = rest / tiles_y;
    const int x = tile_x * 64 + (threadIdx.x & 63);
    const int y = tile_y * 16 + (int)(threadIdx.x >> 6) * 2;
    if (x >= a.W || y >= a.H) return;
    const bool hasL = y + 1 < a.H;
    const float px = (float)(a.col0 + x) + a.pc, pyU = (float)(a.row0 + y) + a.pc, pyL = (float)(a.row0 + y + 1) + a.pc;
    const size_t frame_b = (size_t)a.Hs * a.Ws * 16;
    const size_t plane_stride_b = (size_t)a.Tstride * frame_b;
    const char *plane = reinterpret_cast<const char *>(a.stack) + (size_t)t * frame_b;
    float TrU = 1.0f, crU = 0.f, cgU = 0.f, cbU = 0.f, AU = 0.f, n1U = 0.f, n2U = 0.f;
    float TrL = 1.0f, crL = 0.f, cgL = 0.f, cbL = 0.f, AL = 0.f, n1L = 0.f, n2L = 0.f;
    const TapStep st = make_tap_step<false>(a.Hs, a.Ws);
    Taps2R tA, tB;
    f4 vA[6], vB[6];
    auto fetch = [&](int d, Taps2R &tp, f4 *v) {
        float h[VL3D_HN];
        load_uniform(a.homos + VL3D_HS * d, h);
        tp.u = make_taps2<COORD, BORDER>(h, px, pyU, a.Hs, a.Ws, a.sx, a.sy, a.ox, a.oy);
        tp.l = make_taps2<COORD, BORDER>(h, px, pyL, a.Hs, a.Ws, a.sx, a.sy, a.ox, a.oy);
        tp.own = hasL && tp.l.off != tp.u.off + st.dy;
        tp.off2 = hasL ? tp.l.off : tp.u.off;
        const char *__restrict__ p = plane + (size_t)d * plane_stride_b;
        v[0] = load_texel<false>(p, tp.u.off);
        v[1] = load_texel<false>(p + st.dx, tp.u.off);
        v[2] = load_texel<false>(p + st.dy, tp.u.off);
        v[3] = load_texel<false>(p + st.dy + st.dx, tp.u.off);
        v[4] = load_texel<false>(p + st.dy, tp.off2);
        v[5] = load_texel<false>(p + st.dy + st.dx, tp.off2);
        asm volatile("" ::: "memory");
    };
#define VL3D_COMPOSITE1(O_, S_)                                                                     \
    {                                                                                               \
        const float w = O_.w * Tr##S_;                                                              \
        cr##S_ += w * O_.x; cg##S_ += w * O_.y; cb##S_ += w * O_.z; A##S_ += w;                     \
        n1##S_ += O_.w; n2##S_ = fmaf(O_.w, O_.w, n2##S_);                                          \
        Tr##S_ *= (1.0f - O_.w);                                                                    \
    }
#define VL3D_COMPOSITE2R(T_, V_, D_)                                                                \
    {                                                                                               \
        const f4 oU = shade2<ORDER, RACT, AACT>(T_.u, V_);                                          \
        VL3D_COMPOSITE1(oU, U)                                                                      \
        f4 oL;                                                                                      \
        if (__builtin_amdgcn_ballot_w64(T_.own) != 0ull) {                                          \
            f4 vl[4] = {V_[2], V_[3], V_[4], V_[5]};                                                \
            if (T_.own) {                                                                           \
                const char *__restrict__ p = plane + (size_t)(D_) * plane_stride_b;                 \
                vl[0] = load_texel<false>(p, T_.l.off);                                             \
                vl[1] = load_texel<false>(p + st.dx, T_.l.off);                                     \
            }                                                                                       \
            oL = shade2<ORDER, RACT, AACT>(T_.l, vl);                                               \
            asm volatile("; render_fwd2r_k own taps" ::: "memory");                                 \
        } else {                                                                                    \
            oL = shade2<ORDER, RACT, AACT>(T_.l, V_ + 2);                                           \
        }                                                                                           \
        VL3D_COMPOSITE1(oL, L)                                                                      \
    }
    fetch(0, tA, vA);
    for (int d = 0;; d += 2) {
        fetch(min(d + 1, a.D - 1), tB, vB);
        VL3D_COMPOSITE2R(tA, vA, d)
        if (d + 1 >= a.D) break;
        fetch(min(d + 2, a.D - 1), tA, vA);
        VL3D_COMPOSITE2R(tB, vB, d + 1)
        if (d + 2 >= a.D) break;
    }
#undef VL3D_COMPOSITE2R
#undef VL3D_COMPOSITE1
    const size_t pix = ((size_t)t * a.H + y) * a.W + x;
    a.rgb[pix * 3 + 0] = crU; a.rgb[pix * 3 + 1] = cgU; a.rgb[pix * 3 + 2] = cbU;
    a.alpha[pix] = AU;
    if (a.asum) { a.asum[pix * 2 + 0] = n1U; a.asum[pix * 2 + 1] = n2U; }
    if (hasL) {
        const size_t pl = pix + a.W;
        a.rgb[pl * 3 + 0] = crL; a.rgb[pl * 3 + 1] = cgL; a.rgb[pl * 3 + 2] = cbL;
        a.alpha[pl] = AL;
        if (a.asum) { a.asum[pl * 2 + 0] = n1L; a.asum[pl * 2 + 1] = n2L; }
    }
}

template <int COORD, int BORDER, int ORDER, int RACT, int AACT, bool F16>
void launch_fwd2x(const RenderArgs &a, hipStream_t s) {
    constexpr int TY = 8;
    const int tiles_x = (a.W + 63) / 64, tiles_y = (a.H + TY - 1) / TY;
    const dim3 grid((unsigned)(tiles_x * tiles_y * ((a.T + 1) / 2))), block(64 * TY);
    if (a.quad_keep && a.cull_masks) {
        launch_cull_fwd_plan<COORD>(a, TY, tiles_x, tiles_y, s);
        hipLaunchKernelGGL((render_fwd2x_k<COORD, BORDER, ORDER, RACT, AACT, TY, F16, true>), grid, block, 0, s, a, tiles_x, tiles_y);
        return;
    }
    if constexpr (!F16 && !(ORDER == VL3D_ACT_PRE && BORDER == VL3D_BORDER_HARDCUT)) {
        if (a.fwd_variant != 7) {
            const int tiles_y2 = (a.H + 15) / 16;
            hipLaunchKernelGGL((render_fwd2r_k<COORD, BORDER, ORDER, RACT, AACT>), dim3((unsigned)(tiles_x * tiles_y2 * a.T)), dim3(512), 0, s, a, tiles_x, tiles_y2);
            return;
        }
    }
    hipLaunchKernelGGL((render_fwd2x_k<COORD, BORDER, ORDER, RACT, AACT, TY, F16>), grid, block, 0, s, a, tiles_x, tiles_y);
}

template <int COORD, int BORDER, int ORDER, int RACT, int AACT, int TY, bool SWZ, bool F16 = false>
void launch_fwd2(const RenderArgs &a, hipStream_t s) {
    const int tiles_x = (a.W + 63) / 64, tiles_y = (a.H + TY - 1) / TY;
    if (a.quad_keep && a.cull_masks) {
        launch_cull_fwd_plan<COORD>(a, TY, tiles_x, tiles_y, s);
        hipLaunchKernelGGL((render_fwd2_k<COORD, BORDER, ORDER, RACT, AACT, TY, SWZ, F16, true>), dim3((unsigned)(tiles_x * tiles_y * a.T)),
                           dim3(64 * TY), 0, s, a, tiles_x, tiles_y);
        return;
    }
    hipLaunchKernelGGL((render_fwd2_k<COORD, BORDER, ORDER, RACT, AACT, TY, SWZ, F16>), dim3((unsigned)(tiles_x * tiles_y * a.T)),
                       dim3(64 * TY), 0, s, a, tiles_x, tiles_y);
}

constexpr int RW = 64;
constexpr int PLAN_HDR = 16;
constexpr int PLAN_REC = 12;
__host__ __device__ inline int plan_win_off(int D) { return (PLAN_HDR + PLAN_REC * D + 3) & ~3; }

template <int COORD>
__device__ void texel_homography(const float *h, int Hs, int Ws, float sx, float sy, float ox, float oy, double M[9]) {
    double ax, ay, bx, by;
    if constexpr (COORD == VL3D_COORD_UTILS_MPI) { ax = (double)(Ws - 1) / Ws; ay = (double)(Hs - 1) / Hs; bx = by = 0.0; }
    else { ax = sx; ay = sy; bx = ox; by = oy; }
    for (int j = 0; j < 3; ++j) {
        M[0 + j] = ax * h[0 + j] + bx * h[6 + j];
        M[3 + j] = ay * h[3 + j] + by * h[6 + j];
        M[6 + j] = h[6 + j];
    }
}

template <int COORD>
__global__ void bwd_plan_k(RenderArgs a, int rows, float *plan) {
    __shared__ int ok_all;
    if (threadIdx.x == 0) ok_all = 1;
    __syncthreads();
    for (int d = threadIdx.x; d < a.D; d += blockDim.x) {
        double M[9];
        texel_homography<COORD>(a.homos + VL3D_HS * d, a.Hs, a.Ws, a.sx, a.sy, a.ox, a.oy, M);
        const double det = M[0] * (M[4] * M[8] - M[5] * M[7]) - M[1] * (M[3] * M[8] - M[5] * M[6]) +
                           M[2] * (M[3] * M[7] - M[4] * M[6]);
        bool ok = (det == det) && fabs(det) > 1e-30;
        double I[9];
        I[0] = (M[4] * M[8] - M[5] * M[7]) / det; I[1] = (M[2] * M[7] - M[1] * M[8]) / det; I[2] = (M[1] * M[5] - M[2] * M[4]) / det;
        I[3] = (M[5] * M[6] - M[3] * M[8]) / det; I[4] = (M[0] * M[8] - M[2] * M[6]) / det; I[5] = (M[2] * M[3] - M[0] * M[5]) / det;
        I[6] = (M[3] * M[7] - M[4] * M[6]) / det; I[7] = (M[1] * M[6] - M[0] * M[7]) / det; I[8] = (M[0] * M[4] - M[1] * M[3]) / det;
        for (int i = 0; i < 9; ++i) plan[PLAN_HDR + PLAN_REC * d + i] = (float)I[i];
        double rxm = 0.0, rym = 0.0;
        for (int gy = 0; gy < 3 && ok; ++gy)
            for (int gx = 0; gx < 3 && ok; ++gx) {
                const double x = a.col0 + a.pc + (gx == 0 ? -2.0 : (gx == 1 ? 0.5 * a.W : a.W + 1.0));
                const double y = a.row0 + a.pc + (gy == 0 ? -2.0 : (gy == 1 ? 0.5 * a.H : a.H + 1.0));
                const double X = M[0] * x + M[1] * y + M[2], Y = M[3] * x + M[4] * y + M[5], Z = M[6] * x + M[7] * y + M[8];
                if (!(Z > 1e-20)) { ok = false; break; }
                const double j00 = (M[0] * Z - X * M[6]) / (Z * Z), j01 = (M[1] * Z - X * M[7]) / (Z * Z);
                const double j10 = (M[3] * Z - Y * M[6]) / (Z * Z), j11 = (M[4] * Z - Y * M[7]) / (Z * Z);
                const double dj = j00 * j11 - j01 * j10;
                if (!(fabs(dj) > 1e-12)) { ok = false; break; }
                const double i_r0 = (fabs(j11) + fabs(j01)) / fabs(dj), i_r1 = (fabs(j10) + fabs(j00)) / fabs(dj);
                if (!(i_r0 < 1.4 && i_r1 < 1.4)) ok = false;
                rxm = fmax(rxm, i_r0); rym = fmax(rym, i_r1);
                if (!(fabs(j00) + fabs(j01) < 4.0 && fabs(j10) + fabs(j11) < 4.0)) ok = false;
            }
        plan[PLAN_HDR + PLAN_REC * d + 9] = (float)fmin(1.02 * rxm + 1e-3, 1.45);
        plan[PLAN_HDR + PLAN_REC * d + 10] = (float)fmin(1.02 * rym + 1e-3, 1.45);
        if (!ok) atomicAnd(&ok_all, 0);
    }
    __syncthreads();
    if (threadIdx.x == 0) { reinterpret_cast<int *>(plan)[0] = ok_all; reinterpret_cast<int *>(plan)[1] = 0; }
    if (threadIdx.x < 4) plan[4 + threadIdx.x] = 0.0f;
    if (threadIdx.x >= 8 && threadIdx.x < 16) plan[threadIdx.x] = 0.0f;
    if (threadIdx.x == 2 || threadIdx.x == 3) plan[threadIdx.x] = 0.0f;
}

template <int COORD>
__global__ __launch_bounds__(256) void bwd_windows_k(RenderArgs a, int iw, int ih, int rh, int tiles_x, int tiles_y, int *win) {
    const int i = blockIdx.x * 256 + threadIdx.x;
    if (i >= tiles_x * tiles_y * a.D) return;
    const int d = i % a.D, tile = i / a.D, tile_x = tile % tiles_x, tile_y = tile / tiles_x;
    const int ix0 = tile_x * iw, ix1 = min(ix0 + iw - 1, a.W - 1), iy0 = tile_y * ih, iy1 = min(iy0 + ih - 1, a.H - 1);
    const float el = (ix0 == 0) ? 1.6f : 0.55f, er = (ix1 == a.W - 1) ? 1.6f : 0.55f;
    const float et = (iy0 == 0) ? 1.6f : 0.55f, eb = (iy1 == a.H - 1) ? 1.6f : 0.55f;
    const float *h = a.homos + VL3D_HS * d;
    float mnx = 1e30f, mxx = -1e30f, mny = 1e30f, mxy = -1e30f;
    for (int c = 0; c < 4; ++c) {
        const float cx = (float)a.col0 + a.pc + ((c & 1) ? (float)ix1 + er : (float)ix0 - el);
        const float cy = (float)a.row0 + a.pc + ((c & 2) ? (float)iy1 + eb : (float)iy0 - et);
        const float X = h[0] * cx + h[1] * cy + h[2], Y = h[3] * cx + h[4] * cy + h[5], Z = h[6] * cx + h[7] * cy + h[8];
        const float ctx = texel_coord<COORD>(X / Z, (float)a.Ws / 2.0f, (float)(a.Ws - 1), a.sx, a.ox);
        const float cty = texel_coord<COORD>(Y / Z, (float)a.Hs / 2.0f, (float)(a.Hs - 1), a.sy, a.oy);
        mnx = fminf(mnx, ctx); mxx = fmaxf(mxx, ctx); mny = fminf(mny, cty); mxy = fmaxf(mxy, cty);
    }
    if (a.q_th) {
        const float qlo_x = fminf(fmaxf(ceilf((mnx - 0.01f + a.q_x0) * a.q_inv_cw - 1e-3f) - 1.0f, 0.0f), (float)(a.QW - 1));
        const float qhi_x = fminf(fmaxf(floorf((mxx + 0.01f + a.q_x0) * a.q_inv_cw + 1e-3f), 0.0f), (float)(a.QW - 1));
        const float qlo_y = fminf(fmaxf(ceilf((mny - 0.01f + a.q_y0) * a.q_inv_ch - 1e-3f) - 1.0f, 0.0f), (float)(a.QH - 1));
        const float qhi_y = fminf(fmaxf(floorf((mxy + 0.01f + a.q_y0) * a.q_inv_ch + 1e-3f), 0.0f), (float)(a.QH - 1));
        mnx += qlo_x; mxx += qhi_x; mny += qlo_y; mxy += qhi_y;
    }
    const int wX0 = max(0, (int)ceilf(fmaxf(mnx - 0.01f, -2.0f))), wY0 = max(0, (int)ceilf(fmaxf(mny - 0.01f, -2.0f)));
    const int wX1 = min(a.Ws - 1, (int)floorf(fminf(mxx + 0.01f, (float)a.Ws)));
    const int wY1 = min(a.Hs - 1, (int)floorf(fminf(mxy + 0.01f, (float)a.Hs)));
    const int ww = min(max(0, wX1 - wX0 + 1), 0xffff), wh = min(max(0, wY1 - wY0 + 1), 0x3fff);
    int4 rec;
    const bool empty = ww == 0 || wh == 0;
    rec.x = empty ? 0 : wX0; rec.y = empty ? 0 : wY0; rec.z = empty ? 0 : (ww | (wh << 16)); rec.w = __float_as_int(1.0f / (float)max(ww, 1));
    {
        float ax, ay;
        if constexpr (COORD == VL3D_COORD_UTILS_MPI) { ax = (float)(a.Ws - 1) / (float)a.Ws; ay = (float)(a.Hs - 1) / (float)a.Hs; }
        else { ax = a.sx; ay = a.sy; }
        bool apart = !a.gather9;
        for (int c = 0; c < 4; ++c) {
            const float cx = (float)a.col0 + a.pc + (float)((c & 1) ? tile_x * iw + iw - 1 + rh + 1 : ix0 - rh - 1);
            const float cy = (float)a.row0 + a.pc + (float)((c & 2) ? tile_y * ih + ih - 1 + rh + 1 : iy0 - rh - 1);
            const float X = h[0] * cx + h[1] * cy + h[2], Y = h[3] * cx + h[4] * cy + h[5], Z = h[6] * cx + h[7] * cy + h[8];
            const float iz2 = 1.0f / (Z * Z);
            const float j00 = ax * (h[0] * Z - X * h[6]) * iz2, j01 = ax * (h[1] * Z - X * h[7]) * iz2;
            const float j10 = ay * (h[3] * Z - Y * h[6]) * iz2, j11 = ay * (h[4] * Z - Y * h[7]) * iz2;
            apart = apart && (Z > 0.0f) && (j00 - fabsf(j01) >= 1.001f) && (j11 - fabsf(j10) >= 1.001f);
        }
        if (apart && !empty) rec.z |= 0x40000000;
    }
    if (a.quad_keep) {
        const int qx0 = max(ix0 - rh, 0), qx1 = min(tile_x * iw + iw - 1 + rh, a.W - 1);
        const int qy0 = max(iy0 - rh, 0), qy1 = min(tile_y * ih + ih - 1 + rh, a.H - 1);
        float tnx = 1e30f, txx = -1e30f, tny = 1e30f, txy = -1e30f;
        for (int c = 0; c < 4; ++c) {
            const float cx = (float)a.col0 + a.pc + (float)((c & 1) ? qx1 : qx0), cy = (float)a.row0 + a.pc + (float)((c & 2) ? qy1 : qy0);
            const float X = h[0] * cx + h[1] * cy + h[2], Y = h[3] * cx + h[4] * cy + h[5], Z = h[6] * cx + h[7] * cy + h[8];
            const float ctx = texel_coord<COORD>(X / Z, (float)a.Ws / 2.0f, (float)(a.Ws - 1), a.sx, a.ox);
            const float cty = texel_coord<COORD>(Y / Z, (float)a.Hs / 2.0f, (float)(a.Hs - 1), a.sy, a.oy);
            tnx = fminf(tnx, ctx); txx = fmaxf(txx, ctx); tny = fminf(tny, cty); txy = fmaxf(txy, cty);
        }
        if (!box_touches_kept_quad(a, d, tnx, txx, tny, txy)) rec.z |= (int)0x80000000;
    }
    reinterpret_cast<int4 *>(win)[i] = rec;
}

__device__ __forceinline__ void lattice_texel(const RenderArgs &a, int x, int y, float &lx, float &ly) {
    lx = (float)x; ly = (float)y;
    if (a.q_th) {
        lx -= fminf(floorf(((float)x + a.q_x0 + 0.5f) * (1.0f / (float)a.q_tw)), (float)(a.QW - 1));
        ly -= fminf(floorf(((float)y + a.q_y0 + 0.5f) * (1.0f / (float)a.q_th)), (float)(a.QH - 1));
    }
}

__device__ __forceinline__ void owner_pixel(const float *__restrict__ hi, float tx, float ty, float pc, int col0, int row0,
                                            float &px, float &py) {
    const float X = hi[0] * tx + hi[1] * ty + hi[2];
    const float Y = hi[3] * tx + hi[4] * ty + hi[5];
    const float Z = hi[6] * tx + hi[7] * ty + hi[8];
    const float rz = fast_rcp(Z);
    px = X * rz - pc - (float)col0;
    py = Y * rz - pc - (float)row0;
}

__device__ __forceinline__ bool adam_texel(const RenderArgs &a, int d, int cx, int cy, int &from, unsigned &off) {
    const int X = a.ad.x0 + cx, Y = a.ad.y0 + cy;
    if (a.ad.boxes) {
        const cint_p b = (cint_p)a.ad.boxes + 4 * d;
        if (Y < b[0] || Y >= b[1] || X < b[2] || X >= b[3]) return false;
    }
    static_assert(vl3d_adam::TS == 8, "bookkeeping tiles of 8 x 8 texels");
    from = a.ad.last_step[((size_t)d * a.ad.tiles_y + (Y >> 3)) * a.ad.tiles_x + (X >> 3)];
    off = (unsigned)(Y * a.ad.Ws + X) << 4;
    return true;
}
__device__ __forceinline__ void adam_texel_inbox(const RenderArgs &a, int d, int cx, int cy, int &from, size_t &off) {
    const int X = a.ad.x0 + cx, Y = a.ad.y0 + cy;
    const size_t tile = ((size_t)d * a.ad.tiles_y + (Y >> 3)) * a.ad.tiles_x + (X >> 3);
    from = a.ad.last_step[tile];
    if (a.ad.blocks) off = ((size_t)(a.ad.blocks[tile] >> 1) * 64 + (size_t)((Y & 7) * 8 + (X & 7))) << 4;
    else off = (size_t)((unsigned)(Y * a.ad.Ws + X) << 4);
}
__device__ __forceinline__ size_t adam_frame_base(const RenderArgs &a, int d, int t) {
    return a.ad.blocks ? (size_t)t * 1024 : ((size_t)d * a.T + t) * ((size_t)a.ad.Hs * a.ad.Ws * 16);
}
template <typename OFF>
__device__ __forceinline__ void adam_texel_step_mv(const RenderArgs &a, size_t fb, OFF off, int from, f4 pcur, f4 g, f4 m0, f4 v0) {
    char *pb = reinterpret_cast<char *>(a.ad.p) + fb, *mb = reinterpret_cast<char *>(a.ad.m) + fb, *vb = reinterpret_cast<char *>(a.ad.v) + fb;
    float4 mm = make_float4(m0.x, m0.y, m0.z, m0.w), vv = make_float4(v0.x, v0.y, v0.z, v0.w);
    vl3d_adam::replay_moments(mm, vv, from, a.ad.step - 1, a.ad.beta1, a.ad.beta2);
    float4 pp = make_float4(pcur.x, pcur.y, pcur.z, pcur.w);
    vl3d_adam::adam_upd4(pp, make_float4(g.x, g.y, g.z, g.w), mm, vv, a.ad.lr_bc1, a.ad.beta1, a.ad.beta2, a.ad.eps, a.ad.bc2s);
    __builtin_nontemporal_store(f4{pp.x, pp.y, pp.z, pp.w}, reinterpret_cast<f4 *>(pb + (size_t)off));
    __builtin_nontemporal_store(f4{mm.x, mm.y, mm.z, mm.w}, reinterpret_cast<f4 *>(mb + (size_t)off));
    __builtin_nontemporal_store(f4{vv.x, vv.y, vv.z, vv.w}, reinterpret_cast<f4 *>(vb + (size_t)off));
}
template <typename OFF>
__device__ __forceinline__ void adam_texel_step(const RenderArgs &a, size_t fb, OFF off, int from, f4 pcur, f4 g) {
    const char *mb = reinterpret_cast<const char *>(a.ad.m) + fb, *vb = reinterpret_cast<const char *>(a.ad.v) + fb;
    adam_texel_step_mv(a, fb, off, from, pcur, g, *reinterpret_cast<const f4 *>(mb + (size_t)off), *reinterpret_cast<const f4 *>(vb + (size_t)off));
}

__global__ __launch_bounds__(256) void bwd_owner_table_k(RenderArgs a, int iw, int ih, int rh, int tiles_x, unsigned short *owner, int rw = 64,
                                                         int slot_bits = 10) {
    if (!reinterpret_cast<const int *>(a.plan)[0]) return;
    const int x = blockIdx.x * 64 + (threadIdx.x & 63);
    const int y = blockIdx.y * 4 + (threadIdx.x >> 6);
    const int d = blockIdx.z;
    if (x >= a.Ws || y >= a.Hs) return;
    float qx, qy, lx, ly;
    lattice_texel(a, x, y, lx, ly);
    owner_pixel(a.plan + PLAN_HDR + PLAN_REC * d, lx, ly, a.pc, a.col0, a.row0, qx, qy);
    const float rxf = fminf(fmaxf(rintf(qx), 0.0f), (float)(a.W - 1)), ryf = fminf(fmaxf(rintf(qy), 0.0f), (float)(a.H - 1));
    const int rx = (int)rxf, ry = (int)ryf;
    const int tx = (int)((rxf + 0.5f) * (1.0f / (float)iw)), ty = (int)((ryf + 0.5f) * (1.0f / (float)ih));
    const unsigned lc = (unsigned)((ry - ty * ih + rh) * rw + (rx - tx * iw + rh));
    const unsigned ymask = slot_bits == 9 ? 15u : 7u;
    const unsigned ent = ((((unsigned)ty & ymask) << 3 | (unsigned)(tx & 7)) << slot_bits) | lc;
    const unsigned e1 = __shfl_down(ent, 1, 64), e2 = __shfl_down(ent, 2, 64), e3 = __shfl_down(ent, 3, 64);
    unsigned short *dst = owner + ((size_t)d * a.Hs + y) * a.Ws + x;
    if ((a.Ws & 3) == 0 && x + 3 < a.Ws) {
        if ((threadIdx.x & 3) == 0) *reinterpret_cast<uint2 *>(dst) = make_uint2(ent | e1 << 16, e2 | e3 << 16);
    } else {
        *dst = (unsigned short)ent;
    }
    int cls = 1;
    if (a.ad.p && a.ad.cls) {
        const int X = a.ad.x0 + x, Y = a.ad.y0 + y;
        bool inbox = true;
        if (a.ad.boxes) {
            const cint_p b = (cint_p)a.ad.boxes + 4 * d;
            inbox = !(Y < b[0] || Y >= b[1] || X < b[2] || X >= b[3]);
        }
        cls = inbox ? vl3d_adam::texel_class(vl3d_adam::Quads{a.quad_keep, a.ad.quad_dyn, a.QH, a.QW, a.q_th, a.q_tw}, d, X, Y, a.ad.Hs, a.ad.Ws) : 3;
        int rfrom = 0;
        size_t roff = 0;
        if (cls == 1) adam_texel_inbox(a, d, x, y, rfrom, roff);
        a.ad.cls[((size_t)d * a.Hs + y) * a.Ws + x] = make_uint2((unsigned)cls | ((unsigned)rfrom << 2), (unsigned)(roff >> 4));
    }
    const bool safe = (qx > 0.5f) && (qx < (float)a.W - 1.5f) && (qy > 0.5f) && (qy < (float)a.H - 1.5f);
    if (safe) return;
    const size_t frame = (size_t)a.Hs * a.Ws;
    if (a.ad.p) {
        const int4 rec = reinterpret_cast<const int4 *>(reinterpret_cast<const int *>(a.plan) + plan_win_off(a.D))[(size_t)(ty * tiles_x + tx) * a.D + d];
        const int ww = rec.z & 0xffff, wh = (rec.z >> 16) & 0x3fff;
        if (rec.z >= 0 && x >= rec.x && x < rec.x + ww && y >= rec.y && y < rec.y + wh) return;
        int from;
        unsigned off;
        if (cls == 2) {
            float4 *g = reinterpret_cast<float4 *>(a.g_stack) + (size_t)d * a.T * frame + (size_t)y * a.Ws + x;
            for (int t = 0; t < a.T; ++t, g += frame) *g = make_float4(0.f, 0.f, 0.f, 0.f);
            return;
        }
        if (cls != 1) return;
        const f4 *pc = reinterpret_cast<const f4 *>(a.stack) + (size_t)d * a.T * frame + (size_t)y * a.Ws + x;
        if (a.ad.cls) {
            size_t offp;
            adam_texel_inbox(a, d, x, y, from, offp);
            for (int t = 0; t < a.T; ++t, pc += frame) adam_texel_step(a, adam_frame_base(a, d, t), offp, from, *pc, f4{0.f, 0.f, 0.f, 0.f});
            return;
        }
        if (!adam_texel(a, d, x, y, from, off)) return;
        for (int t = 0; t < a.T; ++t, pc += frame) adam_texel_step(a, adam_frame_base(a, d, t), off, from, *pc, f4{0.f, 0.f, 0.f, 0.f});
        return;
    }
    if (a.g_f16) {
        float2 *g = reinterpret_cast<float2 *>(a.g_stack) + (size_t)d * a.T * frame + (size_t)y * a.Ws + x;
        for (int t = 0; t < a.T; ++t, g += frame) *g = make_float2(0.f, 0.f);
    } else {
        float4 *g = reinterpret_cast<float4 *>(a.g_stack) + (size_t)d * a.T * frame + (size_t)y * a.Ws + x;
        for (int t = 0; t < a.T; ++t, g += frame) *g = make_float4(0.f, 0.f, 0.f, 0.f);
    }
    if (a.g_mask) {
        float *g = a.g_mask + (size_t)d * a.T * frame + (size_t)y * a.Ws + x;
        for (int t = 0; t < a.T; ++t, g += frame) *g = 0.f;
    }
}

__global__ __launch_bounds__(256) void bwd_owner_table4_k(RenderArgs a, int iw, int ih, int rh, unsigned short *owner, int rw, int slot_bits) {
    if (!reinterpret_cast<const int *>(a.plan)[0]) return;
    const int x0 = (blockIdx.x * 64 + (threadIdx.x & 63)) * 4;
    const int y = blockIdx.y * 4 + (threadIdx.x >> 6);
    const int d = blockIdx.z;
    if (x0 >= a.Ws || y >= a.Hs) return;
    const float *hi = a.plan + PLAN_HDR + PLAN_REC * d;
    const unsigned ymask = slot_bits == 9 ? 15u : 7u;
    const float inv_iw = 1.0f / (float)iw, inv_ih = 1.0f / (float)ih;
    unsigned ent[4];
    bool unsafe[4];
#pragma unroll
    for (int k = 0; k < 4; ++k) {
        float qx, qy, lx, ly;
        lattice_texel(a, x0 + k, y, lx, ly);
        owner_pixel(hi, lx, ly, a.pc, a.col0, a.row0, qx, qy);
        const float rxf = fminf(fmaxf(rintf(qx), 0.0f), (float)(a.W - 1)), ryf = fminf(fmaxf(rintf(qy), 0.0f), (float)(a.H - 1));
        const int rx = (int)rxf, ry = (int)ryf;
        const int tx = (int)((rxf + 0.5f) * inv_iw), ty = (int)((ryf + 0.5f) * inv_ih);
        const unsigned lc = (unsigned)((ry - ty * ih + rh) * rw + (rx - tx * iw + rh));
        ent[k] = ((((unsigned)ty & ymask) << 3 | (unsigned)(tx & 7)) << slot_bits) | lc;
        unsafe[k] = !((qx > 0.5f) && (qx < (float)a.W - 1.5f) && (qy > 0.5f) && (qy < (float)a.H - 1.5f));
    }
    const size_t row = ((size_t)d * a.Hs + y) * a.Ws;
    unsigned short *dst = owner + row + x0;
    if ((a.Ws & 3) == 0) {
        *reinterpret_cast<uint2 *>(dst) = make_uint2(ent[0] | ent[1] << 16, ent[2] | ent[3] << 16);
    } else {
#pragma unroll
        for (int k = 0; k < 4; ++k)
            if (x0 + k < a.Ws) dst[k] = (unsigned short)ent[k];
    }
#pragma unroll
    for (int k = 0; k < 4; ++k) {
        if (!unsafe[k] || x0 + k >= a.Ws) continue;
        if (a.g_f16) reinterpret_cast<float2 *>(a.g_stack)[row + x0 + k] = make_float2(0.f, 0.f);
        else reinterpret_cast<float4 *>(a.g_stack)[row + x0 + k] = make_float4(0.f, 0.f, 0.f, 0.f);
        if (a.g_mask) a.g_mask[row + x0 + k] = 0.f;
    }
}

__global__ __launch_bounds__(256) void bwd_fill_zero_if_infeasible_k(float2 *g, size_t n8, const float *plan) {
    if (reinterpret_cast<const int *>(plan)[0]) return;
    for (size_t i = (size_t)blockIdx.x * 256 + threadIdx.x; i < n8; i += (size_t)gridDim.x * 256) g[i] = make_float2(0.f, 0.f);
}
__global__ __launch_bounds__(256) void bwd_fill_zero_f32_if_infeasible_k(float *g, size_t n, const float *plan) {
    if (reinterpret_cast<const int *>(plan)[0]) return;
    for (size_t i = (size_t)blockIdx.x * 256 + threadIdx.x; i < n; i += (size_t)gridDim.x * 256) g[i] = 0.f;
}

template <int COORD, int BORDER, int ORDER, int RACT, int AACT, int ROWS, bool REG, bool F16, bool CULL = false, bool MASK = false, bool ADAM = false, int RWT = 64>
__global__ __launch_bounds__(RWT *ROWS, ((REG || MASK || (CULL && COORD == VL3D_COORD_UTILS_MPI)) ? 4 : ((CULL && RWT == 32) ? 6 : 8))) void render_bwd_tile_k(RenderArgs a) {
    static_assert(!(MASK && (CULL || F16 || ORDER != VL3D_ACT_POST)), "the loop-mask channel: dense fp32 stage-1 stacks, sample-then-activate");
    static_assert(!(ADAM && (F16 || MASK || !REG)), "the fused optimiser step: fp32 stacks, the instantiation with the 128-register budget");
    static_assert(RWT == 64 || RWT == 32, "region width");
    if (!reinterpret_cast<const int *>(a.plan)[0]) return;
    constexpr int RW = RWT;
    constexpr int SLOT_BITS = RW * ROWS > 512 ? 10 : 9;
    constexpr unsigned SLOT_MASK = (1u << SLOT_BITS) - 1u;
    constexpr int NT = RW * ROWS;
    __shared__ float s_gm[MASK ? 2 : 1][MASK ? NT : 1];
    constexpr int RH = 1;
    __shared__ float4 s_g[2][NT];
    __shared__ float2 s_t[2][NT];
    const int tid = threadIdx.x, lane = tid & (RW - 1), row = tid / RW;
    const int bid = xcd_remap(blockIdx.x, gridDim.x);
    const int tile_x = bid % a.tiles_x, rest = bid / a.tiles_x;
    const int tile_y = rest % a.tiles_y, t = rest / a.tiles_y;
    const int rx0 = tile_x * (RW - 2 * RH) - RH, ry0 = tile_y * (ROWS - 2 * RH) - RH;
    const int x = rx0 + lane, y = ry0 + row;
    const bool inimg = (x >= 0) && (x < a.W) && (y >= 0) && (y < a.H);
    const int ix0 = max(rx0 + RH, 0), ix1 = min(rx0 + RW - 1 - RH, a.W - 1);
    const int iy0 = max(ry0 + RH, 0), iy1 = min(ry0 + ROWS - 1 - RH, a.H - 1);
    const float px = (float)(a.col0 + x) + a.pc, py = (float)(a.row0 + y) + a.pc;
    constexpr size_t TEXB = F16 ? 8 : 16;
    const size_t frame = (size_t)a.Hs * a.Ws * 4;
    const size_t plane_stride = (size_t)a.T * frame;
    const size_t plane_stride_b = (size_t)a.T * a.Hs * a.Ws * TEXB;
    const char *plane = reinterpret_cast<const char *>(a.stack) + (size_t)t * a.Hs * a.Ws * TEXB;
    char *gplane = reinterpret_cast<char *>(a.g_stack) + (size_t)t * a.Hs * a.Ws * TEXB;
    float Gr = 0.f, Gg = 0.f, Gb = 0.f, gA = 0.f, S = 0.f, gN1 = 0.f, gN2 = 0.f;
    if (inimg) {
        const size_t pix = ((size_t)t * a.H + y) * a.W + x;
        Gr = a.g_rgb[pix * 3 + 0]; Gg = a.g_rgb[pix * 3 + 1]; Gb = a.g_rgb[pix * 3 + 2];
        gA = a.g_alpha ? a.g_alpha[pix] : 0.0f;
        S = dot3p(Gr, a.rgb[pix * 3 + 0], Gg, a.rgb[pix * 3 + 1], Gb, a.rgb[pix * 3 + 2], gA * a.alpha[pix]);
        if constexpr (REG) if (a.g_asum) { gN1 = a.g_asum[pix * 2 + 0]; gN2 = 2.0f * a.g_asum[pix * 2 + 1]; }
    }
    float gL = 0.f;
    if constexpr (MASK) if (inimg) gL = a.g_label[((size_t)t * a.H + y) * a.W + x];
    const float *mplane = MASK ? a.mask + (size_t)t * a.Hs * a.Ws : nullptr;
    float *gmplane = MASK ? a.g_mask + (size_t)t * a.Hs * a.Ws : nullptr;
    const size_t mplane_stride = (size_t)a.T * a.Hs * a.Ws;
    float Tr = 1.0f, P = 0.0f;
    float gsx_c = 0.f, gsy_c = 0.f, gsx_a = 0.f, gsy_a = 0.f;
    unsigned fl = 0u;
    const uint2 *sgp = nullptr;
    uint2 wg_own = make_uint2(0u, 0u), wg_l = wg_own, wg_u = wg_own, wg_p = wg_own;
    int wg_idx = -1;
    const bool has_l = inimg && x >= 1, has_u = inimg && y >= 1;
    const bool reg_on = REG && a.g_reg != nullptr;
    if constexpr (REG) if (reg_on) {
        gsx_c = a.g_reg[0]; gsy_c = a.g_reg[1]; gsx_a = a.g_reg[2]; gsy_a = a.g_reg[3];
        const int xc = min(max(x, 0), a.W - 1), yc = min(max(y, 0), a.H - 1);
        sgp = reinterpret_cast<const uint2 *>(a.reg_signs) + ((size_t)t * a.H + yc) * a.W + xc;
        if (inimg) fl = a.reg_flags[(size_t)y * a.W + x];
    }
    const size_t sg_plane = (size_t)a.T * a.H * a.W;
    constexpr bool provider = true;
    const TapStep st = make_tap_step<F16>(a.Hs, a.Ws);
    const unsigned my_tile_id = (unsigned)(tile_y * a.tiles_x + tile_x);
    const unsigned my_tile = (unsigned)((tile_y & (SLOT_BITS == 9 ? 15 : 7)) << 3 | (tile_x & 7));
    const unsigned toff_thread = (unsigned)(row * a.Ws + lane);
    const cint_p wrec = (cint_p)a.plan + plan_win_off(a.D) + (size_t)my_tile_id * a.D * 4;
    int nswept = 0;
    for (int d = 0; d < a.D; ++d, plane += plane_stride_b, gplane += plane_stride_b, mplane += mplane_stride, gmplane += mplane_stride) {
        float h[VL3D_HN];
        load_uniform(a.homos + VL3D_HS * d, h);
        const int X0 = wrec[4 * d], Y0 = wrec[4 * d + 1], wwh = wrec[4 * d + 2];
        const int ww = wwh & 0xffff, wh = (wwh >> 16) & 0x3fff;
        const bool culled = CULL && wwh < 0;
        const bool apart = (wwh & 0x40000000) != 0;
        const int buf = CULL ? (nswept & 1) : (d & 1);
        if constexpr (CULL) nswept += culled ? 0 : 1;
        if constexpr (REG || RWT == 32) { if (CULL && culled && (ADAM || a.grad_culled_unwritten)) continue; }
        const unsigned win0 = (unsigned)(Y0 * a.Ws + X0);
        const unsigned short *oplane = a.owner + (size_t)d * a.Hs * a.Ws;
        const unsigned e0 = oplane[win0 + toff_thread];
        const uint2 *rplane = nullptr;
        uint2 rec0 = make_uint2(0u, 0u);
        if constexpr (ADAM && CULL) {
            rplane = a.ad.cls + (size_t)d * a.Hs * a.Ws;
            rec0 = rplane[win0 + toff_thread];
        }
        if (CULL && culled) {
            const f4 z = f4{0.f, 0.f, 0.f, 0.f};
            if (row < wh && lane < ww && (e0 >> SLOT_BITS) == my_tile)
                store_grad_texel<F16>(gplane, (win0 + toff_thread) << 4, z);
            for (int wy = row; wy < wh; wy += ROWS)
                for (int wx = lane + (wy == row ? RW : 0); wx < ww; wx += RW) {
                    const unsigned tix = win0 + (unsigned)(wy * a.Ws + wx);
                    if ((oplane[tix] >> SLOT_BITS) == my_tile)
                        store_grad_texel<F16>(gplane, tix << 4, z);
                }
            continue;
        }
        float2 tc = make_float2(0.f, 0.f);
        float4 gval = make_float4(0.f, 0.f, 0.f, 0.f);
        f4 o = f4{0.f, 0.f, 0.f, 0.f}, pre = o;
        Taps2 tp{};
        float gm = 0.f, msig = 0.f;
        if (inimg) {
            if constexpr (CULL) tp = make_taps2<COORD, BORDER>(h, px, py, a.Hs, a.Ws, a.sx, a.sy, a.ox, a.oy, plane_cull(a, d));
            else tp = make_taps2<COORD, BORDER>(h, px, py, a.Hs, a.Ws, a.sx, a.sy, a.ox, a.oy);
            const char *src = plane;
            if VL3D_ABLATE(a.ablate, 4) {
                src = reinterpret_cast<const char *>(a.stack);
                tp.off &= 0xfff0u;
            }
            typename TapVal<F16, ORDER>::type tv[4];
            load_taps2<F16>(src, tp, st, tv);
            float mt[4];
            if constexpr (MASK) load_mask_taps(mplane, tp.off, st, mt);
            o = shade2<ORDER, RACT, AACT>(tp, tv, &pre);
            if constexpr (MASK) msig = act_fwd<VL3D_ACT_SIGMOID>(mask_blend(mt, tp.w));
        }
        f4 sg = f4{0.f, 0.f, 0.f, 0.f};
        if constexpr (REG) if (reg_on) {
            if ((d >> 2) != wg_idx) {
                wg_idx = d >> 2;
                const uint2 *w = sgp + (size_t)(d >> 2) * sg_plane;
                const uint2 zz = make_uint2(0x55555555u, 0x55555555u);
                wg_own = w[0]; wg_l = w[has_l ? -1 : 0]; wg_u = w[has_u ? -(ptrdiff_t)a.W : 0];
                if (!has_l) wg_l = zz;
                if (!has_u) wg_u = zz;
                if (fl & 12u) wg_p = reinterpret_cast<const uint2 *>(a.reg_patch)[w - reinterpret_cast<const uint2 *>(a.reg_signs)];
            }
            const bool hi = (d & 2) != 0;
            sg = reg_grad32(hi ? wg_own.y : wg_own.x, hi ? wg_l.y : wg_l.x, hi ? wg_u.y : wg_u.x, hi ? wg_p.y : wg_p.x, 16u * (d & 1), fl,
                            f4{gsx_c, gsx_c, gsx_c, gsx_a}, f4{gsy_c, gsy_c, gsy_c, gsy_a});
        }
        if (inimg) {
            const float q = dot3p(Gr, o.x, Gg, o.y, Gb, o.z, gA);
            const float w = o.w * Tr;
            if constexpr (MASK) gm = gL * w * (msig * (1.0f - msig));
            P = fmaf(w, q, P);
            const float om = 1.0f - o.w;
            const float behind = (om > 1e-12f) ? (S - P) * fast_rcp(om) : 0.0f;
            if constexpr (REG) sg.w += fmaf(gN2, o.w, gN1);
            gval = make_float4(fmaf(w, Gr, sg.x), fmaf(w, Gg, sg.y), fmaf(w, Gb, sg.z), fmaf(Tr, q, -behind) + sg.w);
            Tr *= om;
            if constexpr (ORDER == VL3D_ACT_POST)
                gval = make_float4(gval.x * act_bwd<RACT>(pre.x, o.x), gval.y * act_bwd<RACT>(pre.y, o.y),
                                   gval.z * act_bwd<RACT>(pre.z, o.z), gval.w * act_bwd<AACT>(pre.w, o.w));
            tc = make_float2(tp.tx, tp.ty);
            if (!(tp.cov > 0.0f && provider)) gval = make_float4(0.f, 0.f, 0.f, 0.f);
        }
        s_t[buf][tid] = tc;
        s_g[buf][tid] = gval;
        if constexpr (MASK) s_gm[buf][tid] = gm;
        f4 pre_m = f4{0.f, 0.f, 0.f, 0.f}, pre_v = pre_m, pre_p = pre_m;
        if constexpr (ADAM && CULL) {
            const bool mine0 = row < wh && lane < ww && (e0 >> SLOT_BITS) == my_tile && (rec0.x & 3u) == 1u;
            const size_t fb = adam_frame_base(a, d, t), o = mine0 ? (size_t)rec0.y << 4 : 0;
            pre_m = *reinterpret_cast<const f4 *>(reinterpret_cast<const char *>(a.ad.m) + fb + o);
            pre_v = *reinterpret_cast<const f4 *>(reinterpret_cast<const char *>(a.ad.v) + fb + o);
            pre_p = load_texel<false>(plane, mine0 ? (win0 + toff_thread) << 4 : 0u);
            asm volatile("" ::: "memory");
        }
        __syncthreads();
        if VL3D_ABLATE(a.ablate, 1) continue;
        auto gather = [&](unsigned e, int wx, int wy, unsigned tix, uint2 rec = make_uint2(0u, 0u), bool pre = false) {
            if ((e >> SLOT_BITS) != my_tile) return;
            const int lc = (int)(e & SLOT_MASK);
            const f2 tau = f2{(float)(X0 + wx), (float)(Y0 + wy)};
            f4 acc = f4{0.f, 0.f, 0.f, 0.f};
            float accm = 0.f;
            if VL3D_ABLATE(a.ablate, 8) {
            } else if (apart) {
                const f2 c0 = *reinterpret_cast<const f2 *>(&s_t[buf][lc]);
                const int li0 = lc - (tau.x < c0.x ? 1 : 0) - (tau.y < c0.y ? RW : 0);
#pragma unroll
                for (int k = 0; k < 4; ++k) {
                    const int li = li0 + (k >> 1) * RW + (k & 1);
                    const f2 dc = *reinterpret_cast<const f2 *>(&s_t[buf][li]) - tau;
                    const float wgt = tent_weight(dc.x) * tent_weight(dc.y);
                    acc += *reinterpret_cast<const f4 *>(&s_g[buf][li]) * wgt;
                    if constexpr (MASK) accm = fmaf(s_gm[buf][li], wgt, accm);
                }
            } else {
#pragma unroll
            for (int dy = -1; dy <= 1; ++dy)
#pragma unroll
                for (int dx = -1; dx <= 1; ++dx) {
                    const int li = lc + dy * RW + dx;
                    const f2 dc = *reinterpret_cast<const f2 *>(&s_t[buf][li]) - tau;
                    const float wgt = tent_weight(dc.x) * tent_weight(dc.y);
                    if (!a.gather9 && __builtin_amdgcn_ballot_w64(wgt != 0.0f) == 0ull) continue;
                    acc += *reinterpret_cast<const f4 *>(&s_g[buf][li]) * wgt;
                    if constexpr (MASK) accm = fmaf(s_gm[buf][li], wgt, accm);
                }
            }
            if constexpr (ORDER == VL3D_ACT_PRE || ORDER == VL3D_ACT_BAKED) {
                const f4 sv = load_texel<F16>(plane, tix << 4);
                acc = f4{acc.x * act_bwd<RACT>(sv.x, act_fwd<RACT>(sv.x)), acc.y * act_bwd<RACT>(sv.y, act_fwd<RACT>(sv.y)),
                         acc.z * act_bwd<RACT>(sv.z, act_fwd<RACT>(sv.z)), acc.w * act_bwd<AACT>(sv.w, act_fwd<AACT>(sv.w))};
            }
            if constexpr (ADAM) {
                int from;
                if constexpr (CULL) {
                    const unsigned c = rec.x & 3u;
                    if (c == 2) store_grad_texel<false>(gplane, tix << 4, acc);
                    if (c != 1) return;
                    from = (int)(rec.x >> 2);
                    const size_t offp = (size_t)rec.y << 4;
                    if (pre) adam_texel_step_mv(a, adam_frame_base(a, d, t), offp, from, pre_p, acc, pre_m, pre_v);
                    else adam_texel_step(a, adam_frame_base(a, d, t), offp, from, load_texel<false>(plane, tix << 4), acc);
                } else {
                    unsigned off;
                    if (!adam_texel(a, d, X0 + wx, Y0 + wy, from, off)) return;
                    adam_texel_step(a, adam_frame_base(a, d, t), off, from, load_texel<false>(plane, tix << 4), acc);
                }
            } else if (!VL3D_ABLATE(a.ablate, 2)) store_grad_texel<F16>(gplane, tix << 4, acc);
            if constexpr (MASK) __builtin_nontemporal_store(accm, gmplane + tix);
        };
        auto rec_at = [&](unsigned tix) { if constexpr (ADAM && CULL) return rplane[tix]; else return make_uint2(0u, 0u); };
        if (row < wh && lane < ww) gather(e0, lane, row, win0 + toff_thread, rec0, true);
        const int nec = ww - RW;
        if (nec > 0 && nec <= RW) {
            const int sh = nec > 1 ? 32 - __builtin_clz((unsigned)(nec - 1)) : 0, rpw = RW >> sh, rmain = min(wh, ROWS);
            const int c = lane & ((1 << sh) - 1), r = lane >> sh;
            for (int wy0 = row * rpw; wy0 < rmain; wy0 += ROWS * rpw) {
                const int wy = wy0 + r, wx = RW + c;
                if (c < nec && wy < rmain) {
                    const unsigned tix = win0 + (unsigned)(wy * a.Ws + wx);
                    gather(oplane[tix], wx, wy, tix, rec_at(tix));
                }
            }
        } else if (nec > RW) {
            for (int wx = lane + RW; wx < ww && row < wh; wx += RW) {
                const unsigned tix = win0 + (unsigned)(row * a.Ws + wx);
                gather(oplane[tix], wx, row, tix, rec_at(tix));
            }
        }
        for (int wy = row + ROWS; wy < wh; wy += ROWS)
            for (int wx = lane; wx < ww; wx += RW) {
                const unsigned tix = win0 + (unsigned)(wy * a.Ws + wx);
                gather(oplane[tix], wx, wy, tix, rec_at(tix));
            }
    }
}



constexpr int PROWS = 16;

template <int ORDER, int RACT, int AACT, bool F16, bool ADAM = false, int PW = 32, int PR = PROWS>
__device__ __forceinline__ void pair_gather_plane(const RenderArgs &a, const float4 *sg0, const float4 *sg1, const float2 *st, int X0, int Y0,
                                                  int ww, int wh, bool apart, unsigned my_tile, unsigned e0, const unsigned short *oplane,
                                                  const char *plane0, char *gplane0, size_t f1, size_t frame_b, bool has1, int col, int row,
                                                  int d = 0, int t0 = 0) {
    const unsigned win0 = (unsigned)(Y0 * a.Ws + X0);
    auto gather = [&](unsigned e, int wx, int wy, unsigned tix) {
        constexpr int SLOT_BITS = PW == 64 ? 10 : 9;
        if ((e >> SLOT_BITS) != my_tile) return;
        const int lc = (int)(e & ((1u << SLOT_BITS) - 1u));
        const f2 tau = f2{(float)(X0 + wx), (float)(Y0 + wy)};
        f4 acc0 = f4{0.f, 0.f, 0.f, 0.f}, acc1 = acc0;
        if (apart) {
            const f2 c0 = *reinterpret_cast<const f2 *>(&st[lc]);
            const int li0 = lc - (tau.x < c0.x ? 1 : 0) - (tau.y < c0.y ? PW : 0);
#pragma unroll
            for (int k = 0; k < 4; ++k) {
                const int li = li0 + (k >> 1) * PW + (k & 1);
                const f2 dc = *reinterpret_cast<const f2 *>(&st[li]) - tau;
                const float wgt = tent_weight(dc.x) * tent_weight(dc.y);
                acc0 += *reinterpret_cast<const f4 *>(&sg0[li]) * wgt;
                acc1 += *reinterpret_cast<const f4 *>(&sg1[li]) * wgt;
            }
        } else {
#pragma unroll
            for (int dy = -1; dy <= 1; ++dy)
#pragma unroll
                for (int dx = -1; dx <= 1; ++dx) {
                    const int li = lc + dy * PW + dx;
                    const f2 dc = *reinterpret_cast<const f2 *>(&st[li]) - tau;
                    const float wgt = tent_weight(dc.x) * tent_weight(dc.y);
                    if (!a.gather9 && __builtin_amdgcn_ballot_w64(wgt != 0.0f) == 0ull) continue;
                    acc0 += *reinterpret_cast<const f4 *>(&sg0[li]) * wgt;
                    acc1 += *reinterpret_cast<const f4 *>(&sg1[li]) * wgt;
                }
        }
        if constexpr (ORDER == VL3D_ACT_PRE || ORDER == VL3D_ACT_BAKED) {
            const f4 sv0 = load_texel<F16>(plane0, tix << 4), sv1 = load_texel<F16>(plane0 + f1, tix << 4);
            acc0 = f4{acc0.x * act_bwd<RACT>(sv0.x, act_fwd<RACT>(sv0.x)), acc0.y * act_bwd<RACT>(sv0.y, act_fwd<RACT>(sv0.y)),
                      acc0.z * act_bwd<RACT>(sv0.z, act_fwd<RACT>(sv0.z)), acc0.w * act_bwd<AACT>(sv0.w, act_fwd<AACT>(sv0.w))};
            acc1 = f4{acc1.x * act_bwd<RACT>(sv1.x, act_fwd<RACT>(sv1.x)), acc1.y * act_bwd<RACT>(sv1.y, act_fwd<RACT>(sv1.y)),
                      acc1.z * act_bwd<RACT>(sv1.z, act_fwd<RACT>(sv1.z)), acc1.w * act_bwd<AACT>(sv1.w, act_fwd<AACT>(sv1.w))};
        }
        if constexpr (ADAM) {
            static_assert(!F16, "the fused optimiser step: fp32 stacks");
            int from;
            unsigned off;
            if (!adam_texel(a, d, X0 + wx, Y0 + wy, from, off)) return;
            const size_t fbytes = (size_t)a.ad.Hs * a.ad.Ws * 16, fb = ((size_t)d * a.T + t0) * fbytes;
            adam_texel_step(a, fb, off, from, load_texel<false>(plane0, tix << 4), acc0);
            if (has1) adam_texel_step(a, fb + fbytes, off, from, load_texel<false>(plane0 + f1, tix << 4), acc1);
        } else {
            store_grad_texel<F16>(gplane0, tix << 4, acc0);
            if (has1) store_grad_texel<F16>(gplane0 + frame_b, tix << 4, acc1);
        }
    };
    if (row < wh && col < ww) gather(e0, col, row, win0 + (unsigned)(row * a.Ws + col));
    const int nec = ww - PW;
    if (nec > 0) {
        const int necp = min(nec, PW);
        const int sh = necp > 1 ? 32 - __builtin_clz((unsigned)(necp - 1)) : 0, rpg = PW >> sh, rmain = min(wh, PR);
        const int c = col & ((1 << sh) - 1), r = col >> sh;
        for (int wxb = PW; wxb < ww; wxb += (1 << sh))
            for (int wy0 = row * rpg; wy0 < rmain; wy0 += PR * rpg) {
                const int wy = wy0 + r, wx = wxb + c;
                if (c < necp && wx < ww && wy < rmain) {
                    const unsigned tix = win0 + (unsigned)(wy * a.Ws + wx);
                    gather(oplane[tix], wx, wy, tix);
                }
            }
    }
    for (int wy = row + PR; wy < wh; wy += PR)
        for (int wx = col; wx < ww; wx += PW) {
            const unsigned tix = win0 + (unsigned)(wy * a.Ws + wx);
            gather(oplane[tix], wx, wy, tix);
        }
}

#define VL3D_PAIR_GRAD(o, pre, Gr, Gg, Gb, gA, S, P, Tr, gv, ex)                                                               \
    {                                                                                                                          \
        const float q = dot3p(Gr, o.x, Gg, o.y, Gb, o.z, gA);                                                                  \
        const float w = o.w * Tr;                                                                                              \
        P = fmaf(w, q, P);                                                                                                     \
        const float om = 1.0f - o.w;                                                                                           \
        const float behind = (om > 1e-12f) ? (S - P) * fast_rcp(om) : 0.0f;                                                    \
        gv = make_float4(fmaf(w, Gr, ex.x), fmaf(w, Gg, ex.y), fmaf(w, Gb, ex.z), fmaf(Tr, q, -behind) + ex.w);                \
        Tr *= om;                                                                                                              \
        if constexpr (ORDER == VL3D_ACT_POST)                                                                                  \
            gv = make_float4(gv.x * act_bwd<RACT>(pre.x, o.x), gv.y * act_bwd<RACT>(pre.y, o.y),                              \
                             gv.z * act_bwd<RACT>(pre.z, o.z), gv.w * act_bwd<AACT>(pre.w, o.w));                              \
    }

template <int COORD, int BORDER, int ORDER, int RACT, int AACT, bool F16, bool REG = false, bool ADAM = false, int PW = 32>
__global__ __launch_bounds__(PW * PROWS, VL3D_PAIR_MIN_WAVES) void render_bwd_pair_k(RenderArgs a) {
    static_assert(PW == 32 || PW == 64, "region width");
    constexpr int PNT = PW * PROWS;
    if (!reinterpret_cast<const int *>(a.plan)[0]) return;
    __shared__ float4 s_g[2][2][PNT];
    __shared__ float2 s_t[2][PNT];
    const int tid = threadIdx.x, col = tid & (PW - 1), row = tid / PW;
    const int bid = xcd_remap(blockIdx.x, gridDim.x);
    const int tile_x = bid % a.tiles_x, rest = bid / a.tiles_x;
    const int tile_y = rest % a.tiles_y, t0 = (rest / a.tiles_y) * 2;
    const bool has1 = t0 + 1 < a.T;
    const int rx0 = tile_x * (PW - 2) - 1, ry0 = tile_y * (PROWS - 2) - 1;
    const int x = rx0 + col, y = ry0 + row;
    const bool inimg = (x >= 0) && (x < a.W) && (y >= 0) && (y < a.H);
    const float px = (float)(a.col0 + x) + a.pc, py = (float)(a.row0 + y) + a.pc;
    constexpr size_t TEXB = F16 ? 8 : 16;
    const size_t frame_b = (size_t)a.Hs * a.Ws * TEXB;
    const size_t plane_stride_b = (size_t)a.T * frame_b;
    const char *plane0 = reinterpret_cast<const char *>(a.stack) + (size_t)t0 * frame_b;
    char *gplane0 = reinterpret_cast<char *>(a.g_stack) + (size_t)t0 * frame_b;
    const size_t f1 = has1 ? frame_b : 0;
    float Gr0 = 0.f, Gg0 = 0.f, Gb0 = 0.f, gA0 = 0.f, S0 = 0.f, Gr1 = 0.f, Gg1 = 0.f, Gb1 = 0.f, gA1 = 0.f, S1 = 0.f;
    if (inimg) {
        size_t pix = ((size_t)t0 * a.H + y) * a.W + x;
        Gr0 = a.g_rgb[pix * 3 + 0]; Gg0 = a.g_rgb[pix * 3 + 1]; Gb0 = a.g_rgb[pix * 3 + 2];
        gA0 = a.g_alpha ? a.g_alpha[pix] : 0.0f;
        S0 = dot3p(Gr0, a.rgb[pix * 3 + 0], Gg0, a.rgb[pix * 3 + 1], Gb0, a.rgb[pix * 3 + 2], gA0 * a.alpha[pix]);
        if (has1) pix += (size_t)a.H * a.W;
        Gr1 = a.g_rgb[pix * 3 + 0]; Gg1 = a.g_rgb[pix * 3 + 1]; Gb1 = a.g_rgb[pix * 3 + 2];
        gA1 = a.g_alpha ? a.g_alpha[pix] : 0.0f;
        S1 = dot3p(Gr1, a.rgb[pix * 3 + 0], Gg1, a.rgb[pix * 3 + 1], Gb1, a.rgb[pix * 3 + 2], gA1 * a.alpha[pix]);
    }
    float gN10 = 0.f, gN20 = 0.f, gN11 = 0.f, gN21 = 0.f;
    f4 gx = f4{0.f, 0.f, 0.f, 0.f}, gy = gx;
    unsigned fl = 0u;
    const uint2 *sgp = nullptr;
    uint2 go0 = make_uint2(0u, 0u), gl0 = go0, gu0 = go0, gp0 = go0, go1 = go0, gl1 = go0, gu1 = go0, gp1 = go0;
    const bool has_l = inimg && x >= 1, has_u = inimg && y >= 1;
    const bool reg_on = REG && a.g_reg != nullptr;
    const size_t sg_plane = (size_t)a.T * a.H * a.W, sg_f1 = has1 ? (size_t)a.H * a.W : 0;
    if constexpr (REG) {
        if (inimg && a.g_asum) {
            size_t pix = ((size_t)t0 * a.H + y) * a.W + x;
            gN10 = a.g_asum[pix * 2 + 0]; gN20 = 2.0f * a.g_asum[pix * 2 + 1];
            pix += sg_f1;
            gN11 = a.g_asum[pix * 2 + 0]; gN21 = 2.0f * a.g_asum[pix * 2 + 1];
        }
        if (reg_on) {
            gx = f4{a.g_reg[0], a.g_reg[0], a.g_reg[0], a.g_reg[2]}; gy = f4{a.g_reg[1], a.g_reg[1], a.g_reg[1], a.g_reg[3]};
            const int xc = min(max(x, 0), a.W - 1), yc = min(max(y, 0), a.H - 1);
            sgp = reinterpret_cast<const uint2 *>(a.reg_signs) + ((size_t)t0 * a.H + yc) * a.W + xc;
            if (inimg) fl = a.reg_flags[(size_t)y * a.W + x];
        }
    }
    float Tr0 = 1.0f, P0 = 0.0f, Tr1 = 1.0f, P1 = 0.0f;
    const TapStep st = make_tap_step<F16>(a.Hs, a.Ws);
    const unsigned my_tile_id = (unsigned)(tile_y * a.tiles_x + tile_x);
    const unsigned my_tile = (unsigned)((tile_y & (PW == 64 ? 7 : 15)) << 3 | (tile_x & 7));
    const unsigned toff_thread = (unsigned)(row * a.Ws + col);
    const cint_p wrec = (cint_p)a.plan + plan_win_off(a.D) + (size_t)my_tile_id * a.D * 4;
    typedef typename TapVal<F16, ORDER>::type tapv_t;
    for (int d = 0; d < a.D; ++d, plane0 += plane_stride_b, gplane0 += plane_stride_b) {
        float h[VL3D_HN];
        load_uniform(a.homos + VL3D_HS * d, h);
        const int X0 = wrec[4 * d], Y0 = wrec[4 * d + 1], wwh = wrec[4 * d + 2];
        const int ww = wwh & 0xffff, wh = (wwh >> 16) & 0x3fff;
        const bool apart = (wwh & 0x40000000) != 0;
        const int buf = d & 1;
        const unsigned short *oplane = a.owner + (size_t)d * a.Hs * a.Ws;
        const unsigned e0 = oplane[(unsigned)(Y0 * a.Ws + X0) + toff_thread];
        if constexpr (REG) if (reg_on && (d & 3) == 0 && !VL3D_REGAB(16)) {
            const uint2 *w = sgp;
            sgp += sg_plane;
            const ptrdiff_t ol = has_l ? -1 : 0, ou = has_u ? -(ptrdiff_t)a.W : 0;
            const uint2 zz = make_uint2(0x55555555u, 0x55555555u);
            go0 = w[0]; gl0 = w[ol]; gu0 = w[ou];
            go1 = w[sg_f1]; gl1 = w[sg_f1 + ol]; gu1 = w[sg_f1 + ou];
            if (!has_l) { gl0 = zz; gl1 = zz; }
            if (!has_u) { gu0 = zz; gu1 = zz; }
            if (fl & 12u) {
                const uint2 *pw = reinterpret_cast<const uint2 *>(a.reg_patch) + (w - reinterpret_cast<const uint2 *>(a.reg_signs));
                gp0 = pw[0]; gp1 = pw[sg_f1];
            }
        }
        float2 tc = make_float2(0.f, 0.f);
        float4 gv0 = make_float4(0.f, 0.f, 0.f, 0.f), gv1 = gv0;
        if (inimg) {
            const Taps2 tp = make_taps2<COORD, BORDER>(h, px, py, a.Hs, a.Ws, a.sx, a.sy, a.ox, a.oy);
            tapv_t tv0[4], tv1[4];
            load_taps2<F16>(plane0, tp, st, tv0);
            load_taps2<F16>(plane0 + f1, tp, st, tv1);
            f4 pre0, pre1;
            const f4 o0 = shade2<ORDER, RACT, AACT>(tp, tv0, &pre0);
            const f4 o1 = shade2<ORDER, RACT, AACT>(tp, tv1, &pre1);
            f4 ex0 = f4{0.f, 0.f, 0.f, 0.f}, ex1 = ex0;
            if constexpr (REG) {
                if (reg_on && !VL3D_REGAB(8)) {
                    const bool hi = (d & 2) != 0;
                    const unsigned bo = 16u * (d & 1);
                    ex0 = reg_grad32(hi ? go0.y : go0.x, hi ? gl0.y : gl0.x, hi ? gu0.y : gu0.x, hi ? gp0.y : gp0.x, bo, fl, gx, gy);
                    ex1 = reg_grad32(hi ? go1.y : go1.x, hi ? gl1.y : gl1.x, hi ? gu1.y : gu1.x, hi ? gp1.y : gp1.x, bo, fl, gx, gy);
                }
                ex0.w += fmaf(gN20, o0.w, gN10);
                ex1.w += fmaf(gN21, o1.w, gN11);
            }
            VL3D_PAIR_GRAD(o0, pre0, Gr0, Gg0, Gb0, gA0, S0, P0, Tr0, gv0, ex0)
            VL3D_PAIR_GRAD(o1, pre1, Gr1, Gg1, Gb1, gA1, S1, P1, Tr1, gv1, ex1)
            tc = make_float2(tp.tx, tp.ty);
            if (!(tp.cov > 0.0f)) { gv0 = make_float4(0.f, 0.f, 0.f, 0.f); gv1 = gv0; }
        }
        s_t[buf][tid] = tc;
        s_g[buf][0][tid] = gv0;
        s_g[buf][1][tid] = gv1;
        __syncthreads();
        pair_gather_plane<ORDER, RACT, AACT, F16, ADAM, PW>(a, s_g[buf][0], s_g[buf][1], s_t[buf], X0, Y0, ww, wh, apart, my_tile, e0, oplane, plane0,
                                                        gplane0, f1, frame_b, has1, col, row, d, t0);
    }
}

template <int COORD, int BORDER, int ORDER, int RACT, int AACT, bool F16, bool REG = false, bool ADAM = false>
void launch_pair(const RenderArgs &a, hipStream_t s, const BwdChoice &) {
    constexpr int SHAPE = BWD_32X16, PW = BWD_REGIONS[SHAPE].width, RH = BWD_HALO, IW = bwd_interior_w(SHAPE), IH = bwd_interior_h(SHAPE);
    static_assert(PROWS == BWD_REGIONS[SHAPE].rows, "render_bwd_pair_k's rows are not the shape table's");
    RenderArgs b = a;
    b.tiles_x = (a.W + IW - 1) / IW; b.tiles_y = (a.H + IH - 1) / IH;
    const int nwin = b.tiles_x * b.tiles_y * a.D;
    hipLaunchKernelGGL((bwd_windows_k<COORD>), dim3((nwin + 255) / 256), dim3(256), 0, s, b, IW, IH, RH, b.tiles_x, b.tiles_y,
                       reinterpret_cast<int *>(const_cast<float *>(a.plan)) + plan_win_off(a.D));
    hipLaunchKernelGGL(bwd_owner_table_k, dim3((a.Ws + 63) / 64, (a.Hs + 3) / 4, a.D), dim3(256), 0, s, b, IW, IH, RH, b.tiles_x,
                       const_cast<unsigned short *>(a.owner), PW, bwd_slot_bits(SHAPE));
    hipLaunchKernelGGL((render_bwd_pair_k<COORD, BORDER, ORDER, RACT, AACT, F16, REG, ADAM, PW>),
                       dim3((unsigned)(b.tiles_x * b.tiles_y * ((a.T + 1) / 2))), dim3(PW * PROWS), 0, s, b);
}

constexpr int P12W = 64, P12ROWS = 12;
template <int COORD, int BORDER, int ORDER, int RACT, int AACT, bool F16>
__global__ __launch_bounds__(P12W * P12ROWS, 6) void render_bwd_pair12_k(RenderArgs a) {
    constexpr int PW = P12W, PR = P12ROWS, PNT = PW * PR;
    if (!reinterpret_cast<const int *>(a.plan)[0]) return;
    __shared__ float4 s_g[2][2][PNT];
    __shared__ float2 s_t[2][PNT];
    const int tid = threadIdx.x, col = tid & (PW - 1), row = tid / PW;
    const int bid = xcd_remap(blockIdx.x, gridDim.x);
    const int tile_x = bid % a.tiles_x, rest = bid / a.tiles_x;
    const int tile_y = rest % a.tiles_y, t0 = (rest / a.tiles_y) * 2;
    const bool has1 = t0 + 1 < a.T;
    const int rx0 = tile_x * (PW - 2) - 1, ry0 = tile_y * (PR - 2) - 1;
    const int x = rx0 + col, y = ry0 + row;
    const bool inimg = (x >= 0) && (x < a.W) && (y >= 0) && (y < a.H);
    const float px = (float)(a.col0 + x) + a.pc, py = (float)(a.row0 + y) + a.pc;
    constexpr size_t TEXB = F16 ? 8 : 16;
    const size_t frame_b = (size_t)a.Hs * a.Ws * TEXB;
    const size_t plane_stride_b = (size_t)a.T * frame_b;
    const char *plane0 = reinterpret_cast<const char *>(a.stack) + (size_t)t0 * frame_b;
    char *gplane0 = reinterpret_cast<char *>(a.g_stack) + (size_t)t0 * frame_b;
    const size_t f1 = has1 ? frame_b : 0;
    float Gr0 = 0.f, Gg0 = 0.f, Gb0 = 0.f, gA0 = 0.f, S0 = 0.f, Gr1 = 0.f, Gg1 = 0.f, Gb1 = 0.f, gA1 = 0.f, S1 = 0.f;
    if (inimg) {
        size_t pix = ((size_t)t0 * a.H + y) * a.W + x;
        Gr0 = a.g_rgb[pix * 3 + 0]; Gg0 = a.g_rgb[pix * 3 + 1]; Gb0 = a.g_rgb[pix * 3 + 2];
        gA0 = a.g_alpha ? a.g_alpha[pix] : 0.0f;
        S0 = dot3p(Gr0, a.rgb[pix * 3 + 0], Gg0, a.rgb[pix * 3 + 1], Gb0, a.rgb[pix * 3 + 2], gA0 * a.alpha[pix]);
        if (has1) pix += (size_t)a.H * a.W;
        Gr1 = a.g_rgb[pix * 3 + 0]; Gg1 = a.g_rgb[pix * 3 + 1]; Gb1 = a.g_rgb[pix * 3 + 2];
        gA1 = a.g_alpha ? a.g_alpha[pix] : 0.0f;
        S1 = dot3p(Gr1, a.rgb[pix * 3 + 0], Gg1, a.rgb[pix * 3 + 1], Gb1, a.rgb[pix * 3 + 2], gA1 * a.alpha[pix]);
    }
    float Tr0 = 1.0f, P0 = 0.0f, Tr1 = 1.0f, P1 = 0.0f;
    const TapStep st = make_tap_step<F16>(a.Hs, a.Ws);
    const unsigned my_tile_id = (unsigned)(tile_y * a.tiles_x + tile_x);
    const unsigned my_tile = (unsigned)((tile_y & 7) << 3 | (tile_x & 7));
    const unsigned toff_thread = (unsigned)(row * a.Ws + col);
    const cint_p wrec = (cint_p)a.plan + plan_win_off(a.D) + (size_t)my_tile_id * a.D * 4;
    typedef typename TapVal<F16, ORDER>::type tapv_t;
    const f4 ex = f4{0.f, 0.f, 0.f, 0.f};
    for (int d = 0; d < a.D; ++d, plane0 += plane_stride_b, gplane0 += plane_stride_b) {
        float h[VL3D_HN];
        load_uniform(a.homos + VL3D_HS * d, h);
        const int X0 = wrec[4 * d], Y0 = wrec[4 * d + 1], wwh = wrec[4 * d + 2];
        const int ww = wwh & 0xffff, wh = (wwh >> 16) & 0x3fff;
        const bool apart = (wwh & 0x40000000) != 0;
        const int buf = d & 1;
        const unsigned short *oplane = a.owner + (size_t)d * a.Hs * a.Ws;
        const unsigned e0 = oplane[(unsigned)(Y0 * a.Ws + X0) + toff_thread];
        float2 tc = make_float2(0.f, 0.f);
        float4 gv0 = make_float4(0.f, 0.f, 0.f, 0.f), gv1 = gv0;
        if (inimg) {
            const Taps2 tp = make_taps2<COORD, BORDER>(h, px, py, a.Hs, a.Ws, a.sx, a.sy, a.ox, a.oy);
            tapv_t tv0[4], tv1[4];
            load_taps2<F16>(plane0, tp, st, tv0);
            load_taps2<F16>(plane0 + f1, tp, st, tv1);
            f4 pre0, pre1;
            const f4 o0 = shade2<ORDER, RACT, AACT>(tp, tv0, &pre0);
            const f4 o1 = shade2<ORDER, RACT, AACT>(tp, tv1, &pre1);
            VL3D_PAIR_GRAD(o0, pre0, Gr0, Gg0, Gb0, gA0, S0, P0, Tr0, gv0, ex)
            VL3D_PAIR_GRAD(o1, pre1, Gr1, Gg1, Gb1, gA1, S1, P1, Tr1, gv1, ex)
            tc = make_float2(tp.tx, tp.ty);
            if (!(tp.cov > 0.0f)) { gv0 = make_float4(0.f, 0.f, 0.f, 0.f); gv1 = gv0; }
        }
        s_t[buf][tid] = tc;
        s_g[buf][0][tid] = gv0;
        s_g[buf][1][tid] = gv1;
        __syncthreads();
        pair_gather_plane<ORDER, RACT, AACT, F16, false, PW, PR>(a, s_g[buf][0], s_g[buf][1], s_t[buf], X0, Y0, ww, wh, apart, my_tile, e0, oplane, plane0,
                                                                 gplane0, f1, frame_b, has1, col, row, d, t0);
    }
}

#undef VL3D_PAIR_GRAD

template <int COORD, int BORDER, int ORDER, int RACT, int AACT, bool F16>
void launch_pair12(const RenderArgs &a, hipStream_t s, const BwdChoice &) {
    constexpr int SHAPE = BWD_64X12, RH = BWD_HALO, IW = bwd_interior_w(SHAPE), IH = bwd_interior_h(SHAPE);
    static_assert(P12W == BWD_REGIONS[SHAPE].width && P12ROWS == BWD_REGIONS[SHAPE].rows, "render_bwd_pair12_k's region is not the shape table's");
    RenderArgs b = a;
    b.tiles_x = (a.W + IW - 1) / IW; b.tiles_y = (a.H + IH - 1) / IH;
    const int nwin = b.tiles_x * b.tiles_y * a.D;
    hipLaunchKernelGGL((bwd_windows_k<COORD>), dim3((nwin + 255) / 256), dim3(256), 0, s, b, IW, IH, RH, b.tiles_x, b.tiles_y,
                       reinterpret_cast<int *>(const_cast<float *>(a.plan)) + plan_win_off(a.D));
    hipLaunchKernelGGL(bwd_owner_table_k, dim3((a.Ws + 63) / 64, (a.Hs + 3) / 4, a.D), dim3(256), 0, s, b, IW, IH, RH, b.tiles_x,
                       const_cast<unsigned short *>(a.owner), P12W, bwd_slot_bits(SHAPE));
    hipLaunchKernelGGL((render_bwd_pair12_k<COORD, BORDER, ORDER, RACT, AACT, F16>),
                       dim3((unsigned)(b.tiles_x * b.tiles_y * ((a.T + 1) / 2))), dim3(P12W * P12ROWS), 0, s, b);
}

template <int COORD, int BORDER, int ORDER, int RACT, int AACT, bool F16, bool MASK = false>
__global__ __launch_bounds__(512) void render_fwd_reg_k(RenderArgs a, int tiles_x, int tiles_y) {
    constexpr int FW = 64, FH = 8, NT = FW * FH;
    __shared__ float4 s_o[2][NT];
    __shared__ float red[4][FH];
    const int b = xcd_remap(blockIdx.x, gridDim.x);
    const int tile_x = b % tiles_x, rest = b / tiles_x;
    const int tile_y = rest % tiles_y, t = rest / tiles_y;
    const int tid = threadIdx.x, lane = tid & 63, row = tid >> 6;
    const int x = tile_x * (FW - 1) + lane, y = tile_y * (FH - 1) + row;
    const bool inimg = (x < a.W) && (y < a.H);
    const bool owner = inimg && lane < FW - 1 && row < FH - 1;
    const unsigned fl = owner ? a.reg_flags[(size_t)y * a.W + x] : 0u;
    const bool own_r = owner && x + 1 < a.W && !(fl & 1u), own_d = owner && y + 1 < a.H && !(fl & 2u);
    const size_t sg_plane = (size_t)a.T * a.H * a.W;
    uint2 *sgq = reinterpret_cast<uint2 *>(a.reg_signs) + ((size_t)t * a.H + min(y, a.H - 1)) * a.W + min(x, a.W - 1);
    unsigned sg_lo = 0u, sg_hi = 0u;
    const float px = (float)(a.col0 + min(x, a.W - 1)) + a.pc, py = (float)(a.row0 + min(y, a.H - 1)) + a.pc;
    const size_t frame_b = (size_t)a.Hs * a.Ws * (F16 ? 8 : 16), plane_stride_b = (size_t)a.T * frame_b;
    const char *plane = reinterpret_cast<const char *>(a.stack) + (size_t)t * frame_b;
    float Tr = 1.0f, cr = 0.f, cg = 0.f, cb = 0.f, A = 0.f, n1 = 0.f, n2 = 0.f;
    float sxc = 0.f, syc = 0.f, sxa = 0.f, sya = 0.f;
    const TapStep st = make_tap_step<F16>(a.Hs, a.Ws);
    typedef typename TapVal<F16, ORDER>::type tapv_t;
    tapv_t vA[4], vB[4];
    static_assert(!(MASK && F16), "the loop-mask channel: fp32 stage-1 stacks");
    float mA[4] = {0.f, 0.f, 0.f, 0.f}, mB[4] = {0.f, 0.f, 0.f, 0.f}, lab = 0.f;
    const float *mplane = MASK ? a.mask + (size_t)t * a.Hs * a.Ws : nullptr;
    const size_t mplane_stride = (size_t)a.T * a.Hs * a.Ws;
#define VL3D_PLANE(T_, V_, BUF_, S_, M_)                                                                  \
    {                                                                                                     \
        const f4 o = shade2<ORDER, RACT, AACT>(T_, V_);                                                   \
        const f4 ol = inimg ? o * T_.cov : f4{0.f, 0.f, 0.f, 0.f};                                        \
        if (!VL3D_REGAB(4)) s_o[BUF_][tid] = make_float4(ol.x, ol.y, ol.z, ol.w);                         \
        const float w = o.w * Tr;                                                                         \
        cr += w * o.x; cg += w * o.y; cb += w * o.z; A += w;                                              \
        n1 += o.w; n2 = fmaf(o.w, o.w, n2);                                                               \
        Tr *= (1.0f - o.w);                                                                               \
        if constexpr (MASK) lab = fmaf(w, act_fwd<VL3D_ACT_SIGMOID>(mask_blend(M_, T_.w)), lab);          \
        if (!VL3D_REGAB(4)) __syncthreads();                                                              \
        int code = (int)REG_ZERO;                                                                         \
        if (own_r && !VL3D_REGAB(2)) {                                                                    \
            const float4 r = s_o[BUF_][tid + 1];                                                          \
            const f4 df = ol - f4{r.x, r.y, r.z, r.w};                                                    \
            sxc += fabsf(df.x) + fabsf(df.y) + fabsf(df.z);                                               \
            sxa += fabsf(df.w);                                                                           \
            if (!VL3D_REGAB(1)) code += reg_signs4(df);                                                   \
        }                                                                                                 \
        if (own_d && !VL3D_REGAB(2)) {                                                                    \
            const float4 r = s_o[BUF_][tid + FW];                                                         \
            const f4 df = ol - f4{r.x, r.y, r.z, r.w};                                                    \
            syc += fabsf(df.x) + fabsf(df.y) + fabsf(df.z);                                               \
            sya += fabsf(df.w);                                                                           \
            if (!VL3D_REGAB(1)) code += reg_signs4(df) << 8;                                              \
        }                                                                                                 \
        if (VL3D_REGAB(1)) { }                                                                            \
        else if (S_ == 0) sg_lo = (unsigned)code;                                                         \
        else if (S_ == 1) sg_lo |= (unsigned)code << 16;                                                  \
        else if (S_ == 2) sg_hi = (unsigned)code;                                                         \
        else {                                                                                            \
            sg_hi |= (unsigned)code << 16;                                                                \
            if (owner) *sgq = make_uint2(sg_lo, sg_hi);                                                   \
            sgq += sg_plane;                                                                              \
        }                                                                                                 \
    }
    const QuadCull noq = QuadCull{nullptr, 0, 0, 0.f, 0.f, 0.f, 0.f, 0};
    Taps2 tA = make_taps2<COORD, BORDER>(a.homos, px, py, a.Hs, a.Ws, a.sx, a.sy, a.ox, a.oy, noq, UvNoise{a.uv_seed, 0}), tB = tA;
    load_taps2<F16>(plane, tA, st, vA);
    if constexpr (MASK) load_mask_taps(mplane, tA.off, st, mA);
#define VL3D_FETCH(T_, V_, DN_, M_)                                                                       \
    {                                                                                                     \
        const int dn = min(DN_, a.D - 1);                                                                 \
        float h[VL3D_HN];                                                                                 \
        load_uniform(a.homos + VL3D_HS * dn, h);                                                          \
        T_ = make_taps2<COORD, BORDER>(h, px, py, a.Hs, a.Ws, a.sx, a.sy, a.ox, a.oy, noq, UvNoise{a.uv_seed, dn});  \
        load_taps2<F16>(plane + (size_t)dn * plane_stride_b, T_, st, V_);                                 \
        if constexpr (MASK) load_mask_taps(mplane + (size_t)dn * mplane_stride, T_.off, st, M_);          \
        asm volatile("" ::: "memory");                                                                    \
    }
    int d = 0;
    for (;; d += 4) {
        VL3D_FETCH(tB, vB, d + 1, mB)
        VL3D_PLANE(tA, vA, 0, 0, mA)
        if (d + 1 >= a.D) break;
        VL3D_FETCH(tA, vA, d + 2, mA)
        VL3D_PLANE(tB, vB, 1, 1, mB)
        if (d + 2 >= a.D) break;
        VL3D_FETCH(tB, vB, d + 3, mB)
        VL3D_PLANE(tA, vA, 0, 2, mA)
        if (d + 3 >= a.D) break;
        VL3D_FETCH(tA, vA, d + 4, mA)
        VL3D_PLANE(tB, vB, 1, 3, mB)
        if (d + 4 >= a.D) break;
    }
    if ((a.D & 3) && owner) *sgq = make_uint2(sg_lo, (a.D & 3) == 3 ? sg_hi : 0u);
#undef VL3D_FETCH
#undef VL3D_PLANE
    if (owner) {
        const size_t pix = ((size_t)t * a.H + y) * a.W + x;
        a.rgb[pix * 3 + 0] = cr; a.rgb[pix * 3 + 1] = cg; a.rgb[pix * 3 + 2] = cb;
        a.alpha[pix] = A;
        if (a.asum) { a.asum[pix * 2 + 0] = n1; a.asum[pix * 2 + 1] = n2; }
        if constexpr (MASK) a.label[pix] = lab;
    }
    float v[4] = {sxc, syc, sxa, sya};
#pragma unroll
    for (int k = 0; k < 4; ++k) {
#pragma unroll
        for (int off = 32; off > 0; off >>= 1) v[k] += __shfl_down(v[k], off, 64);
        if (lane == 0) red[k][row] = v[k];
    }
    __syncthreads();
    if (tid < 4) {
        double sum = 0.0;
        for (int r = 0; r < FH; ++r) sum += (double)red[tid][r];
        atomicAdd(a.reg_sums + tid, sum);
    }
}

template <int COORD, int BORDER, int ORDER, int RACT, int AACT, int SHAPE, bool REG, bool F16 = false, bool MASK = false, bool ADAM = false>
void launch_tile(const RenderArgs &a, hipStream_t s, const BwdChoice &c) {
    constexpr int RWT = BWD_REGIONS[SHAPE].width, ROWS = BWD_REGIONS[SHAPE].rows, RH = BWD_HALO, IW = bwd_interior_w(SHAPE), IH = bwd_interior_h(SHAPE);
    constexpr int SLOT_BITS = bwd_slot_bits(SHAPE);
    RenderArgs b = a;
    b.tiles_x = (a.W + IW - 1) / IW; b.tiles_y = (a.H + IH - 1) / IH;
    const int nwin = b.tiles_x * b.tiles_y * a.D;
    hipLaunchKernelGGL((bwd_windows_k<COORD>), dim3((nwin + 255) / 256), dim3(256), 0, s, b, IW, IH, RH, b.tiles_x, b.tiles_y,
                       reinterpret_cast<int *>(const_cast<float *>(a.plan)) + plan_win_off(a.D));
    if (c.owner4)
        hipLaunchKernelGGL(bwd_owner_table4_k, dim3(((a.Ws + 3) / 4 + 63) / 64, (a.Hs + 3) / 4, a.D), dim3(256), 0, s, b, IW, IH, RH,
                           const_cast<unsigned short *>(a.owner), RWT, SLOT_BITS);
    else
        hipLaunchKernelGGL(bwd_owner_table_k, dim3((a.Ws + 63) / 64, (a.Hs + 3) / 4, a.D), dim3(256), 0, s, b, IW, IH, RH, b.tiles_x,
                           const_cast<unsigned short *>(a.owner), RWT, SLOT_BITS);
    const dim3 grid((unsigned)(b.tiles_x * b.tiles_y * a.T)), block(RWT * ROWS);
    if constexpr (ADAM) {
        hipLaunchKernelGGL((render_bwd_tile_k<COORD, BORDER, ORDER, RACT, AACT, ROWS, true, false, true, false, true, RWT>), grid, block, 0, s, b);
    } else if constexpr (MASK) {
        hipLaunchKernelGGL((render_bwd_tile_k<COORD, BORDER, ORDER, RACT, AACT, ROWS, REG, F16, false, true, false, RWT>), grid, block, 0, s, b);
    } else if (c.cull)
        hipLaunchKernelGGL((render_bwd_tile_k<COORD, BORDER, ORDER, RACT, AACT, ROWS, REG, F16, true, false, false, RWT>), grid, block, 0, s, b);
    else
        hipLaunchKernelGGL((render_bwd_tile_k<COORD, BORDER, ORDER, RACT, AACT, ROWS, REG, F16, false, false, false, RWT>), grid, block, 0, s, b);
}

using BwdLauncher = void (*)(const RenderArgs &, hipStream_t, const BwdChoice &);

inline BwdFacts bwd_facts_of(const RenderArgs &a, int coord, int border, int order, int ract, int aact, bool f16, int plane_record) {
    BwdFacts f{};
    f.coord = coord; f.border = border; f.order = order; f.ract = ract; f.aact = aact; f.f16 = f16; f.plane_record = plane_record;
    f.T = a.T; f.H = a.H; f.W = a.W; f.Hs = a.Hs; f.Ws = a.Ws;
    f.set = BwdSetting{(BwdPolicy)a.bwd_policy, a.gather9 != 0, a.owner4 != 0};
    f.reg = a.g_reg || a.g_asum; f.mask = a.mask != nullptr; f.adam = a.ad.p != nullptr; f.qk = a.quad_keep != nullptr;
    f.gcu = a.grad_culled_unwritten != 0;
    return f;
}

inline int bwd_not_built(const BwdChoice &c) {
    char msg[160];
    snprintf(msg, sizeof msg, "render backward: no kernel built for the choice (family %d, %d x %d regions, reg %d mask %d adam %d cull %d f16 %d)",
             c.family, BWD_REGIONS[c.shape].width, BWD_REGIONS[c.shape].rows, (int)c.reg, (int)c.mask, (int)c.adam, (int)c.cull, (int)c.f16);
    vl3d_set_error(msg);
    return VL3D_EUNSUPPORTED;
}

template <bool BWD, int COORD, int BORDER, int ORDER, int RACT, int AACT, bool F16>
int launch_t(const RenderArgs &a, hipStream_t s) {
    dim3 grid((a.W + TILE_X - 1) / TILE_X, (a.H + TILE_Y - 1) / TILE_Y, a.T), block(TILE_X * TILE_Y);
    constexpr bool MASKABLE = COORD == VL3D_COORD_AFFINE && BORDER == VL3D_BORDER_HARDCUT && ORDER == VL3D_ACT_POST &&
                              RACT == VL3D_ACT_SIGMOID && AACT == VL3D_ACT_SIGMOID && !F16;
    if constexpr (BWD) {
        constexpr bool SHIPPED9 = MASKABLE && VL3D_HS == 9, SIG = RACT == VL3D_ACT_SIGMOID && AACT == VL3D_ACT_SIGMOID;
        const BwdChoice c = choose_bwd(bwd_facts_of(a, COORD, BORDER, ORDER, RACT, AACT, F16, VL3D_HS));
        if (c.family != VL3D_BWD_ATOMICS) {
            BwdLauncher go = nullptr;
#define VL3D_CONV COORD, BORDER, ORDER, RACT, AACT
#define VL3D_BWD_CASE(BUILT, KEY, ...)      \
    case bwd_key KEY:                       \
        if constexpr (BUILT) go = &__VA_ARGS__; \
        break;
            switch (bwd_key(c)) {
                VL3D_BWD_CASE(MASKABLE, (VL3D_BWD_TILE, BWD_64X8, true, true), launch_tile<VL3D_CONV, BWD_64X8, true, false, true>)
                VL3D_BWD_CASE(MASKABLE, (VL3D_BWD_TILE, BWD_64X8, false, true), launch_tile<VL3D_CONV, BWD_64X8, false, false, true>)
                VL3D_BWD_CASE(MASKABLE, (VL3D_BWD_TILE, BWD_64X16, true, true), launch_tile<VL3D_CONV, BWD_64X16, true, false, true>)
                VL3D_BWD_CASE(MASKABLE, (VL3D_BWD_TILE, BWD_64X16, false, true), launch_tile<VL3D_CONV, BWD_64X16, false, false, true>)
                VL3D_BWD_CASE(SHIPPED9, (VL3D_BWD_TILE, BWD_32X16, true, false, true), launch_tile<VL3D_CONV, BWD_32X16, true, false, false, true>)
                VL3D_BWD_CASE(SHIPPED9, (VL3D_BWD_TILE, BWD_64X16, true, false, true), launch_tile<VL3D_CONV, BWD_64X16, true, false, false, true>)
                VL3D_BWD_CASE(SHIPPED9, (VL3D_BWD_PAIR, BWD_32X16, true, false, true), launch_pair<VL3D_CONV, false, true, true>)
                VL3D_BWD_CASE(SHIPPED9, (VL3D_BWD_PAIR, BWD_32X16, false, false, true), launch_pair<VL3D_CONV, false, false, true>)
                VL3D_BWD_CASE(SIG, (VL3D_BWD_PAIR, BWD_32X16, false), launch_pair<VL3D_CONV, F16>)
                VL3D_BWD_CASE(SIG, (VL3D_BWD_PAIR12, BWD_64X12, false), launch_pair12<VL3D_CONV, F16>)
                VL3D_BWD_CASE(SIG && COORD != VL3D_COORD_UTILS_MPI, (VL3D_BWD_PAIR, BWD_32X16, true), launch_pair<VL3D_CONV, F16, true>)
                VL3D_BWD_CASE(SHIPPED9, (VL3D_BWD_TILE, BWD_32X16, true), launch_tile<VL3D_CONV, BWD_32X16, true, false>)
                VL3D_BWD_CASE(SHIPPED9, (VL3D_BWD_TILE, BWD_32X16, false), launch_tile<VL3D_CONV, BWD_32X16, false, false>)
                VL3D_BWD_CASE(SHIPPED9, (VL3D_BWD_TILE, BWD_64X8, false), launch_tile<VL3D_CONV, BWD_64X8, false, false>)
                VL3D_BWD_CASE(true, (VL3D_BWD_TILE, BWD_64X16, true), launch_tile<VL3D_CONV, BWD_64X16, true, F16>)
                VL3D_BWD_CASE(true, (VL3D_BWD_TILE, BWD_64X16, false), launch_tile<VL3D_CONV, BWD_64X16, false, F16>)
            }
#undef VL3D_BWD_CASE
#undef VL3D_CONV
            if (!go || c.f16 != F16) return bwd_not_built(c);
            hipLaunchKernelGGL((bwd_plan_k<COORD>), dim3(1), dim3(64), 0, s, a, 16, const_cast<float *>(a.plan));
            const size_t n8 = (size_t)a.D * a.T * a.Hs * a.Ws * (a.g_f16 ? 1 : 2);
            hipLaunchKernelGGL(bwd_fill_zero_if_infeasible_k, dim3(4096), dim3(256), 0, s, reinterpret_cast<float2 *>(a.g_stack), n8, a.plan);
            if (c.mask) hipLaunchKernelGGL(bwd_fill_zero_f32_if_infeasible_k, dim3(1024), dim3(256), 0, s, a.g_mask, (size_t)a.D * a.T * a.Hs * a.Ws, a.plan);
            go(a, s, c);
        }
        if constexpr (MASKABLE) {
            if (a.mask) {
                hipLaunchKernelGGL((render_bwd_k<COORD, BORDER, ORDER, RACT, AACT, false, true>), grid, block, 0, s, a);
                return VL3D_OK;
            }
        }
        hipLaunchKernelGGL((render_bwd_k<COORD, BORDER, ORDER, RACT, AACT, F16>), grid, block, 0, s, a);
        return VL3D_OK;
    } else {
        if (a.reg_fwd == 2) {
            launch_reg_prepass<COORD, BORDER, ORDER, RACT, AACT, F16>(a, s);
            const int tx = (a.W + 62) / 63, ty = (a.H + 6) / 7;
            bool with_mask = false;
            if constexpr (MASKABLE) {
                if (a.mask) {
                    hipLaunchKernelGGL((render_fwd_reg_k<COORD, BORDER, ORDER, RACT, AACT, false, true>), dim3((unsigned)(tx * ty * a.T)), dim3(512), 0, s, a, tx, ty);
                    with_mask = true;
                }
            }
            if (!with_mask)
                hipLaunchKernelGGL((render_fwd_reg_k<COORD, BORDER, ORDER, RACT, AACT, F16>), dim3((unsigned)(tx * ty * a.T)), dim3(512), 0, s, a, tx, ty);
            launch_reg_slots<COORD, BORDER, ORDER, RACT, AACT, F16, true>(a, s);
            return VL3D_OK;
        }
        if (a.reg_fwd == 3) {
            launch_reg_prepass<COORD, BORDER, ORDER, RACT, AACT, F16>(a, s);
            launch_reg_slots<COORD, BORDER, ORDER, RACT, AACT, F16, false, true>(a, s);
            return VL3D_OK;
        }
        if (a.reg_fwd) {
            launch_reg_prepass<COORD, BORDER, ORDER, RACT, AACT, F16>(a, s);
            launch_reg_slots<COORD, BORDER, ORDER, RACT, AACT, F16, false>(a, s);
            return VL3D_OK;
        }
        if constexpr (MASKABLE) {
            if (a.mask) {
                const int tiles_x = (a.W + 63) / 64, tiles_y = (a.H + 7) / 8;
                hipLaunchKernelGGL((render_fwd2_k<COORD, BORDER, ORDER, RACT, AACT, 8, true, false, false, true>), dim3((unsigned)(tiles_x * tiles_y * a.T)),
                                   dim3(64 * 8), 0, s, a, tiles_x, tiles_y);
                return VL3D_OK;
            }
        }
        if constexpr (RACT == VL3D_ACT_SIGMOID && AACT == VL3D_ACT_SIGMOID) {
            if (a.T >= 2 && a.fwd_variant != 6 && !a.uv_seed) { launch_fwd2x<COORD, BORDER, ORDER, RACT, AACT, F16>(a, s); return VL3D_OK; }
        }
        launch_fwd2<COORD, BORDER, ORDER, RACT, AACT, 8, true, F16>(a, s);
        return VL3D_OK;
    }
}

template <bool BWD, int COORD, int BORDER, int ORDER, int RACT, int AACT>
int launch(const RenderArgs &a, hipStream_t s) {
    if constexpr (RACT == VL3D_ACT_SIGMOID && AACT == VL3D_ACT_SIGMOID) {
        if (a.g_f16) return launch_t<BWD, COORD, BORDER, ORDER, RACT, AACT, true>(a, s);
    }
    return launch_t<BWD, COORD, BORDER, ORDER, RACT, AACT, false>(a, s);
}

}
```

Baseline: 2877 Mpix/s.

## Fuse backward prepass launches and loop owner-table rows per block

Result: slower. 2818 Mpix/s (-2.0%).

```diff
diff --git a/include/vl3d.h b/include/vl3d.h
--- a/include/vl3d.h
+++ b/include/vl3d.h
@@ -34,6 +34,7 @@
     uint32_t uv_noise_seed;
 } vl3d_render_desc;
 enum { VL3D_GRAD_CULLED_UNWRITTEN = 1 };
+enum { VL3D_VARIANT_BWD_PREPASS_UNLOOPED = 0x10000 };
 
 int vl3d_render_fwd(const vl3d_render_desc *desc, const void *stack, const float *homos, const uint8_t *quad_keep, int32_t QH, int32_t QW,
                     void *cull_scratch, float *rgb, float *alpha, float *alpha_sums, vl3d_stream_t stream);
diff --git a/videoloop3d_amd/csrc/vl3d_render.hip b/videoloop3d_amd/csrc/vl3d_render.hip
--- a/videoloop3d_amd/csrc/vl3d_render.hip
+++ b/videoloop3d_amd/csrc/vl3d_render.hip
@@ -87,6 +87,7 @@
 }
 static void set_bwd_setting(RenderArgs &a, const vl3d_render_desc *desc, const BwdSetting &set, void *scratch) {
     a.bwd_policy = set.policy; a.gather9 = set.gather9; a.owner4 = set.owner4;
+    if (desc->variant & VL3D_VARIANT_BWD_PREPASS_UNLOOPED) a.ablate |= BWD_PREPASS_UNLOOPED;
     if (set.policy == BWD_NONE) return;
     a.plan = (const float *)scratch;
     a.owner = reinterpret_cast<const unsigned short *>(reinterpret_cast<const char *>(scratch) + owner_table_off(desc));
diff --git a/videoloop3d_amd/csrc/vl3d_render_core.h b/videoloop3d_amd/csrc/vl3d_render_core.h
--- a/videoloop3d_amd/csrc/vl3d_render_core.h
+++ b/videoloop3d_amd/csrc/vl3d_render_core.h
@@ -572,12 +572,8 @@
 
 constexpr int TILE_X = 64, TILE_Y = 4;
 
-template <int COORD, int BORDER, int ORDER, int RACT, int AACT, bool F16, bool MASK = false>
-__global__ __launch_bounds__(TILE_X *TILE_Y) void render_bwd_k(RenderArgs a) {
-    if (a.plan && reinterpret_cast<const int *>(a.plan)[0]) return;
-    const int x = blockIdx.x * TILE_X + (threadIdx.x & (TILE_X - 1));
-    const int y = blockIdx.y * TILE_Y + (threadIdx.x / TILE_X);
-    const int t = blockIdx.z;
+template <int COORD, int BORDER, int ORDER, int RACT, int AACT, bool F16, bool MASK>
+__device__ __forceinline__ void render_bwd_pixel(const RenderArgs &a, int x, int y, int t) {
     if (x >= a.W || y >= a.H) return;
     const float px = (float)(a.col0 + x) + a.pc, py = (float)(a.row0 + y) + a.pc;
     constexpr size_t TEXB = F16 ? 8 : 16;
@@ -640,6 +636,15 @@
                 atomic_add_grad_texel<F16>(gplane, (size_t)tp.off + ((i & 1) ? gst.dx : 0u) + ((i & 2) ? gst.dy : 0u), c);
             }
         }
+    }
+}
+template <int COORD, int BORDER, int ORDER, int RACT, int AACT, bool F16, bool MASK = false>
+__global__ __launch_bounds__(TILE_X *TILE_Y) void render_bwd_k(RenderArgs a, int tiles_x, int tiles_y) {
+    if (a.plan && reinterpret_cast<const int *>(a.plan)[0]) return;
+    const int per_frame = tiles_x * tiles_y, n = per_frame * a.T;
+    for (int i = blockIdx.x; i < n; i += gridDim.x) {
+        const int t = i / per_frame, tile = i - t * per_frame, tile_y = tile / tiles_x, tile_x = tile - tile_y * tiles_x;
+        render_bwd_pixel<COORD, BORDER, ORDER, RACT, AACT, F16, MASK>(a, tile_x * TILE_X + (threadIdx.x & (TILE_X - 1)), tile_y * TILE_Y + (threadIdx.x / TILE_X), t);
     }
 }
 
@@ -1030,7 +1035,7 @@
 }
 
 template <int COORD>
-__global__ void bwd_plan_k(RenderArgs a, int rows, float *plan) {
+__device__ __forceinline__ void bwd_plan_block(const RenderArgs &a, float *plan) {
     __shared__ int ok_all;
     if (threadIdx.x == 0) ok_all = 1;
     __syncthreads();
@@ -1071,10 +1076,13 @@
     if (threadIdx.x >= 8 && threadIdx.x < 16) plan[threadIdx.x] = 0.0f;
     if (threadIdx.x == 2 || threadIdx.x == 3) plan[threadIdx.x] = 0.0f;
 }
-
 template <int COORD>
-__global__ __launch_bounds__(256) void bwd_windows_k(RenderArgs a, int iw, int ih, int rh, int tiles_x, int tiles_y, int *win) {
-    const int i = blockIdx.x * 256 + threadIdx.x;
+__global__ void bwd_plan_k(RenderArgs a, int rows, float *plan) {
+    bwd_plan_block<COORD>(a, plan);
+}
+
+template <int COORD>
+__device__ __forceinline__ void bwd_window_record(const RenderArgs &a, int i, int iw, int ih, int rh, int tiles_x, int tiles_y, int *win) {
     if (i >= tiles_x * tiles_y * a.D) return;
     const int d = i % a.D, tile = i / a.D, tile_x = tile % tiles_x, tile_y = tile / tiles_x;
     const int ix0 = tile_x * iw, ix1 = min(ix0 + iw - 1, a.W - 1), iy0 = tile_y * ih, iy1 = min(iy0 + ih - 1, a.H - 1);
@@ -1135,6 +1143,15 @@
     }
     reinterpret_cast<int4 *>(win)[i] = rec;
 }
+template <int COORD>
+__global__ __launch_bounds__(256) void bwd_windows_k(RenderArgs a, int iw, int ih, int rh, int tiles_x, int tiles_y, int *win) {
+    bwd_window_record<COORD>(a, blockIdx.x * 256 + threadIdx.x, iw, ih, rh, tiles_x, tiles_y, win);
+}
+template <int COORD>
+__global__ __launch_bounds__(256) void bwd_plan_windows_k(RenderArgs a, int iw, int ih, int rh, int tiles_x, int tiles_y, float *plan, int *win) {
+    if (blockIdx.x == 0) bwd_plan_block<COORD>(a, plan);
+    else bwd_window_record<COORD>(a, (blockIdx.x - 1) * 256 + threadIdx.x, iw, ih, rh, tiles_x, tiles_y, win);
+}
 
 __device__ __forceinline__ void lattice_texel(const RenderArgs &a, int x, int y, float &lx, float &ly) {
     lx = (float)x; ly = (float)y;
@@ -1152,6 +1169,18 @@
     const float rz = fast_rcp(Z);
     px = X * rz - pc - (float)col0;
     py = Y * rz - pc - (float)row0;
+}
+template <bool Z_FUSED, typename HP>
+__device__ __forceinline__ void owner_pixel_exact(HP hi, float tx, float ty, float pc, int col0, int row0, float &px, float &py) {
+#pragma clang fp contract(off)
+    const float X = fmaf(hi[0], tx, hi[1] * ty) + hi[2];
+    const float Y = fmaf(hi[3], tx, hi[4] * ty) + hi[5];
+    float Z;
+    if constexpr (Z_FUSED) Z = fmaf(hi[6], tx, hi[7] * ty) + hi[8];
+    else Z = (hi[6] * tx + hi[7] * ty) + hi[8];
+    const float rz = fast_rcp(Z);
+    px = fmaf(X, rz, -pc) - (float)col0;
+    py = fmaf(Y, rz, -pc) - (float)row0;
 }
 
 __device__ __forceinline__ bool adam_texel(const RenderArgs &a, int d, int cx, int cy, int &from, unsigned &off) {
@@ -1192,16 +1221,13 @@
     adam_texel_step_mv(a, fb, off, from, pcur, g, *reinterpret_cast<const f4 *>(mb + (size_t)off), *reinterpret_cast<const f4 *>(vb + (size_t)off));
 }
 
-__global__ __launch_bounds__(256) void bwd_owner_table_k(RenderArgs a, int iw, int ih, int rh, int tiles_x, unsigned short *owner, int rw = 64,
-                                                         int slot_bits = 10) {
-    if (!reinterpret_cast<const int *>(a.plan)[0]) return;
-    const int x = blockIdx.x * 64 + (threadIdx.x & 63);
-    const int y = blockIdx.y * 4 + (threadIdx.x >> 6);
-    const int d = blockIdx.z;
+template <bool ADAM = true, typename HP>
+__device__ __forceinline__ void owner_table_texel(const RenderArgs &a, HP hi, int x, int y, int d, int iw, int ih, int rh,
+                                                  int tiles_x, unsigned short *owner, int rw, int slot_bits) {
     if (x >= a.Ws || y >= a.Hs) return;
     float qx, qy, lx, ly;
     lattice_texel(a, x, y, lx, ly);
-    owner_pixel(a.plan + PLAN_HDR + PLAN_REC * d, lx, ly, a.pc, a.col0, a.row0, qx, qy);
+    owner_pixel_exact<true>(hi, lx, ly, a.pc, a.col0, a.row0, qx, qy);
     const float rxf = fminf(fmaxf(rintf(qx), 0.0f), (float)(a.W - 1)), ryf = fminf(fmaxf(rintf(qy), 0.0f), (float)(a.H - 1));
     const int rx = (int)rxf, ry = (int)ryf;
     const int tx = (int)((rxf + 0.5f) * (1.0f / (float)iw)), ty = (int)((ryf + 0.5f) * (1.0f / (float)ih));
@@ -1216,7 +1242,7 @@
         *dst = (unsigned short)ent;
     }
     int cls = 1;
-    if (a.ad.p && a.ad.cls) {
+    if (ADAM && a.ad.p && a.ad.cls) {
         const int X = a.ad.x0 + x, Y = a.ad.y0 + y;
         bool inbox = true;
         if (a.ad.boxes) {
@@ -1232,7 +1258,7 @@
     const bool safe = (qx > 0.5f) && (qx < (float)a.W - 1.5f) && (qy > 0.5f) && (qy < (float)a.H - 1.5f);
     if (safe) return;
     const size_t frame = (size_t)a.Hs * a.Ws;
-    if (a.ad.p) {
+    if (ADAM && a.ad.p) {
         const int4 rec = reinterpret_cast<const int4 *>(reinterpret_cast<const int *>(a.plan) + plan_win_off(a.D))[(size_t)(ty * tiles_x + tx) * a.D + d];
         const int ww = rec.z & 0xffff, wh = (rec.z >> 16) & 0x3fff;
         if (rec.z >= 0 && x >= rec.x && x < rec.x + ww && y >= rec.y && y < rec.y + wh) return;
@@ -1267,14 +1293,17 @@
         for (int t = 0; t < a.T; ++t, g += frame) *g = 0.f;
     }
 }
-
-__global__ __launch_bounds__(256) void bwd_owner_table4_k(RenderArgs a, int iw, int ih, int rh, unsigned short *owner, int rw, int slot_bits) {
+__global__ __launch_bounds__(256) void bwd_owner_table_k(RenderArgs a, int iw, int ih, int rh, int tiles_x, unsigned short *owner, int rw = 64,
+                                                         int slot_bits = 10) {
     if (!reinterpret_cast<const int *>(a.plan)[0]) return;
-    const int x0 = (blockIdx.x * 64 + (threadIdx.x & 63)) * 4;
-    const int y = blockIdx.y * 4 + (threadIdx.x >> 6);
-    const int d = blockIdx.z;
+    owner_table_texel(a, a.plan + PLAN_HDR + PLAN_REC * blockIdx.z, blockIdx.x * 64 + (threadIdx.x & 63), blockIdx.y * 4 + (threadIdx.x >> 6), blockIdx.z,
+                      iw, ih, rh, tiles_x, owner, rw, slot_bits);
+}
+
+template <typename HP>
+__device__ __forceinline__ void owner_table_texel4(const RenderArgs &a, HP hi, int x0, int y, int d, int iw, int ih, int rh,
+                                                   unsigned short *owner, int rw, int slot_bits) {
     if (x0 >= a.Ws || y >= a.Hs) return;
-    const float *hi = a.plan + PLAN_HDR + PLAN_REC * d;
     const unsigned ymask = slot_bits == 9 ? 15u : 7u;
     const float inv_iw = 1.0f / (float)iw, inv_ih = 1.0f / (float)ih;
     unsigned ent[4];
@@ -1283,7 +1312,8 @@
     for (int k = 0; k < 4; ++k) {
         float qx, qy, lx, ly;
         lattice_texel(a, x0 + k, y, lx, ly);
-        owner_pixel(hi, lx, ly, a.pc, a.col0, a.row0, qx, qy);
+        if (k == 0) owner_pixel_exact<true>(hi, lx, ly, a.pc, a.col0, a.row0, qx, qy);
+        else owner_pixel_exact<false>(hi, lx, ly, a.pc, a.col0, a.row0, qx, qy);
         const float rxf = fminf(fmaxf(rintf(qx), 0.0f), (float)(a.W - 1)), ryf = fminf(fmaxf(rintf(qy), 0.0f), (float)(a.H - 1));
         const int rx = (int)rxf, ry = (int)ryf;
         const int tx = (int)((rxf + 0.5f) * inv_iw), ty = (int)((ryf + 0.5f) * inv_ih);
@@ -1308,6 +1338,45 @@
         if (a.g_mask) a.g_mask[row + x0 + k] = 0.f;
     }
 }
+__global__ __launch_bounds__(256) void bwd_owner_table4_k(RenderArgs a, int iw, int ih, int rh, unsigned short *owner, int rw, int slot_bits) {
+    if (!reinterpret_cast<const int *>(a.plan)[0]) return;
+    owner_table_texel4(a, a.plan + PLAN_HDR + PLAN_REC * blockIdx.z, (blockIdx.x * 64 + (threadIdx.x & 63)) * 4, blockIdx.y * 4 + (threadIdx.x >> 6),
+                       blockIdx.z, iw, ih, rh, owner, rw, slot_bits);
+}
+
+#ifndef VL3D_OWNER_ROW_GROUPS
+#define VL3D_OWNER_ROW_GROUPS 4
+#endif
+#ifndef VL3D_OWNER4_ROW_GROUPS
+#define VL3D_OWNER4_ROW_GROUPS 8
+#endif
+constexpr int BWD_FALLBACK_BLOCKS = 2048;
+template <bool FOUR, bool ADAM = false>
+__global__ __launch_bounds__(256) void bwd_owner_loop_k(RenderArgs a, int iw, int ih, int rh, int tiles_x, unsigned short *owner, int rw, int slot_bits,
+                                                        int groups, int strips, int chunks) {
+    if (!reinterpret_cast<const int *>(a.plan)[0]) {
+        const size_t texels = (size_t)a.D * a.T * a.Hs * a.Ws, n8 = texels * (a.g_f16 ? 1 : 2);
+        const size_t i0 = (size_t)blockIdx.x * 256 + threadIdx.x, step = (size_t)gridDim.x * 256;
+        float2 *g = reinterpret_cast<float2 *>(a.g_stack);
+        for (size_t i = i0; i < n8; i += step) g[i] = make_float2(0.f, 0.f);
+        if (a.g_mask)
+            for (size_t i = i0; i < texels; i += step) a.g_mask[i] = 0.f;
+        return;
+    }
+    const int strip = blockIdx.x % strips, chunk = (blockIdx.x / strips) % chunks, d = blockIdx.x / (strips * chunks);
+    const cfloat_p hi = (cfloat_p)(a.plan + PLAN_HDR + PLAN_REC * d);
+    const int col = strip * 64 + (threadIdx.x & 63);
+    if constexpr (ADAM) {
+        static_assert(!FOUR, "the fused step keeps its per-texel records");
+        owner_table_texel<true>(a, hi, col, chunk * 4 + (threadIdx.x >> 6), d, iw, ih, rh, tiles_x, owner, rw, slot_bits);
+    } else {
+        int y = chunk * groups * 4 + (threadIdx.x >> 6);
+        for (int r = 0; r < groups && y < a.Hs; ++r, y += 4) {
+            if constexpr (FOUR) owner_table_texel4(a, hi, col * 4, y, d, iw, ih, rh, owner, rw, slot_bits);
+            else owner_table_texel<false>(a, hi, col, y, d, iw, ih, rh, tiles_x, owner, rw, slot_bits);
+        }
+    }
+}
 
 __global__ __launch_bounds__(256) void bwd_fill_zero_if_infeasible_k(float2 *g, size_t n8, const float *plan) {
     if (reinterpret_cast<const int *>(plan)[0]) return;
@@ -1316,6 +1385,38 @@
 __global__ __launch_bounds__(256) void bwd_fill_zero_f32_if_infeasible_k(float *g, size_t n, const float *plan) {
     if (reinterpret_cast<const int *>(plan)[0]) return;
     for (size_t i = (size_t)blockIdx.x * 256 + threadIdx.x; i < n; i += (size_t)gridDim.x * 256) g[i] = 0.f;
+}
+
+constexpr int BWD_PREPASS_UNLOOPED = 0x100;
+template <int COORD>
+void launch_bwd_prepass(const RenderArgs &b, hipStream_t s, int shape, bool owner4, bool mask) {
+    const int IW = bwd_interior_w(shape), IH = bwd_interior_h(shape), RH = BWD_HALO, RWT = BWD_REGIONS[shape].width, SLOT_BITS = bwd_slot_bits(shape);
+    float *plan = const_cast<float *>(b.plan);
+    int *win = reinterpret_cast<int *>(plan) + plan_win_off(b.D);
+    unsigned short *owner = const_cast<unsigned short *>(b.owner);
+    const int nwin = b.tiles_x * b.tiles_y * b.D;
+    const int strips = owner4 ? ((b.Ws + 3) / 4 + 63) / 64 : (b.Ws + 63) / 64, row_groups = (b.Hs + 3) / 4;
+    if (b.ablate & BWD_PREPASS_UNLOOPED) {
+        hipLaunchKernelGGL((bwd_plan_k<COORD>), dim3(1), dim3(64), 0, s, b, 16, plan);
+        const size_t n8 = (size_t)b.D * b.T * b.Hs * b.Ws * (b.g_f16 ? 1 : 2);
+        hipLaunchKernelGGL(bwd_fill_zero_if_infeasible_k, dim3(4096), dim3(256), 0, s, reinterpret_cast<float2 *>(b.g_stack), n8, b.plan);
+        if (mask) hipLaunchKernelGGL(bwd_fill_zero_f32_if_infeasible_k, dim3(1024), dim3(256), 0, s, b.g_mask, (size_t)b.D * b.T * b.Hs * b.Ws, b.plan);
+        hipLaunchKernelGGL((bwd_windows_k<COORD>), dim3((nwin + 255) / 256), dim3(256), 0, s, b, IW, IH, RH, b.tiles_x, b.tiles_y, win);
+        if (owner4)
+            hipLaunchKernelGGL(bwd_owner_table4_k, dim3(strips, row_groups, b.D), dim3(256), 0, s, b, IW, IH, RH, owner, RWT, SLOT_BITS);
+        else
+            hipLaunchKernelGGL(bwd_owner_table_k, dim3(strips, row_groups, b.D), dim3(256), 0, s, b, IW, IH, RH, b.tiles_x, owner, RWT, SLOT_BITS);
+        return;
+    }
+    hipLaunchKernelGGL((bwd_plan_windows_k<COORD>), dim3(1 + (nwin + 255) / 256), dim3(256), 0, s, b, IW, IH, RH, b.tiles_x, b.tiles_y, plan, win);
+    const int groups = b.ad.p ? 1 : owner4 ? VL3D_OWNER4_ROW_GROUPS : VL3D_OWNER_ROW_GROUPS, chunks = (row_groups + groups - 1) / groups;
+    const dim3 grid((unsigned)(strips * chunks * b.D));
+    if (owner4)
+        hipLaunchKernelGGL((bwd_owner_loop_k<true>), grid, dim3(256), 0, s, b, IW, IH, RH, b.tiles_x, owner, RWT, SLOT_BITS, groups, strips, chunks);
+    else if (b.ad.p)
+        hipLaunchKernelGGL((bwd_owner_loop_k<false, true>), grid, dim3(256), 0, s, b, IW, IH, RH, b.tiles_x, owner, RWT, SLOT_BITS, groups, strips, chunks);
+    else
+        hipLaunchKernelGGL((bwd_owner_loop_k<false>), grid, dim3(256), 0, s, b, IW, IH, RH, b.tiles_x, owner, RWT, SLOT_BITS, groups, strips, chunks);
 }
 
 template <int COORD, int BORDER, int ORDER, int RACT, int AACT, int ROWS, bool REG, bool F16, bool CULL = false, bool MASK = false, bool ADAM = false, int RWT = 64>
@@ -1778,15 +1879,11 @@
 
 template <int COORD, int BORDER, int ORDER, int RACT, int AACT, bool F16, bool REG = false, bool ADAM = false>
 void launch_pair(const RenderArgs &a, hipStream_t s, const BwdChoice &) {
-    constexpr int SHAPE = BWD_32X16, PW = BWD_REGIONS[SHAPE].width, RH = BWD_HALO, IW = bwd_interior_w(SHAPE), IH = bwd_interior_h(SHAPE);
+    constexpr int SHAPE = BWD_32X16, PW = BWD_REGIONS[SHAPE].width, IW = bwd_interior_w(SHAPE), IH = bwd_interior_h(SHAPE);
     static_assert(PROWS == BWD_REGIONS[SHAPE].rows, "render_bwd_pair_k's rows are not the shape table's");
     RenderArgs b = a;
     b.tiles_x = (a.W + IW - 1) / IW; b.tiles_y = (a.H + IH - 1) / IH;
-    const int nwin = b.tiles_x * b.tiles_y * a.D;
-    hipLaunchKernelGGL((bwd_windows_k<COORD>), dim3((nwin + 255) / 256), dim3(256), 0, s, b, IW, IH, RH, b.tiles_x, b.tiles_y,
-                       reinterpret_cast<int *>(const_cast<float *>(a.plan)) + plan_win_off(a.D));
-    hipLaunchKernelGGL(bwd_owner_table_k, dim3((a.Ws + 63) / 64, (a.Hs + 3) / 4, a.D), dim3(256), 0, s, b, IW, IH, RH, b.tiles_x,
-                       const_cast<unsigned short *>(a.owner), PW, bwd_slot_bits(SHAPE));
+    launch_bwd_prepass<COORD>(b, s, SHAPE, false, false);
     hipLaunchKernelGGL((render_bwd_pair_k<COORD, BORDER, ORDER, RACT, AACT, F16, REG, ADAM, PW>),
                        dim3((unsigned)(b.tiles_x * b.tiles_y * ((a.T + 1) / 2))), dim3(PW * PROWS), 0, s, b);
 }
@@ -1869,15 +1966,11 @@
 
 template <int COORD, int BORDER, int ORDER, int RACT, int AACT, bool F16>
 void launch_pair12(const RenderArgs &a, hipStream_t s, const BwdChoice &) {
-    constexpr int SHAPE = BWD_64X12, RH = BWD_HALO, IW = bwd_interior_w(SHAPE), IH = bwd_interior_h(SHAPE);
+    constexpr int SHAPE = BWD_64X12, IW = bwd_interior_w(SHAPE), IH = bwd_interior_h(SHAPE);
     static_assert(P12W == BWD_REGIONS[SHAPE].width && P12ROWS == BWD_REGIONS[SHAPE].rows, "render_bwd_pair12_k's region is not the shape table's");
     RenderArgs b = a;
     b.tiles_x = (a.W + IW - 1) / IW; b.tiles_y = (a.H + IH - 1) / IH;
-    const int nwin = b.tiles_x * b.tiles_y * a.D;
-    hipLaunchKernelGGL((bwd_windows_k<COORD>), dim3((nwin + 255) / 256), dim3(256), 0, s, b, IW, IH, RH, b.tiles_x, b.tiles_y,
-                       reinterpret_cast<int *>(const_cast<float *>(a.plan)) + plan_win_off(a.D));
-    hipLaunchKernelGGL(bwd_owner_table_k, dim3((a.Ws + 63) / 64, (a.Hs + 3) / 4, a.D), dim3(256), 0, s, b, IW, IH, RH, b.tiles_x,
-                       const_cast<unsigned short *>(a.owner), P12W, bwd_slot_bits(SHAPE));
+    launch_bwd_prepass<COORD>(b, s, SHAPE, false, false);
     hipLaunchKernelGGL((render_bwd_pair12_k<COORD, BORDER, ORDER, RACT, AACT, F16>),
                        dim3((unsigned)(b.tiles_x * b.tiles_y * ((a.T + 1) / 2))), dim3(P12W * P12ROWS), 0, s, b);
 }
@@ -2003,19 +2096,10 @@
 
 template <int COORD, int BORDER, int ORDER, int RACT, int AACT, int SHAPE, bool REG, bool F16 = false, bool MASK = false, bool ADAM = false>
 void launch_tile(const RenderArgs &a, hipStream_t s, const BwdChoice &c) {
-    constexpr int RWT = BWD_REGIONS[SHAPE].width, ROWS = BWD_REGIONS[SHAPE].rows, RH = BWD_HALO, IW = bwd_interior_w(SHAPE), IH = bwd_interior_h(SHAPE);
-    constexpr int SLOT_BITS = bwd_slot_bits(SHAPE);
+    constexpr int RWT = BWD_REGIONS[SHAPE].width, ROWS = BWD_REGIONS[SHAPE].rows, IW = bwd_interior_w(SHAPE), IH = bwd_interior_h(SHAPE);
     RenderArgs b = a;
     b.tiles_x = (a.W + IW - 1) / IW; b.tiles_y = (a.H + IH - 1) / IH;
-    const int nwin = b.tiles_x * b.tiles_y * a.D;
-    hipLaunchKernelGGL((bwd_windows_k<COORD>), dim3((nwin + 255) / 256), dim3(256), 0, s, b, IW, IH, RH, b.tiles_x, b.tiles_y,
-                       reinterpret_cast<int *>(const_cast<float *>(a.plan)) + plan_win_off(a.D));
-    if (c.owner4)
-        hipLaunchKernelGGL(bwd_owner_table4_k, dim3(((a.Ws + 3) / 4 + 63) / 64, (a.Hs + 3) / 4, a.D), dim3(256), 0, s, b, IW, IH, RH,
-                           const_cast<unsigned short *>(a.owner), RWT, SLOT_BITS);
-    else
-        hipLaunchKernelGGL(bwd_owner_table_k, dim3((a.Ws + 63) / 64, (a.Hs + 3) / 4, a.D), dim3(256), 0, s, b, IW, IH, RH, b.tiles_x,
-                           const_cast<unsigned short *>(a.owner), RWT, SLOT_BITS);
+    launch_bwd_prepass<COORD>(b, s, SHAPE, c.owner4, c.mask);
     const dim3 grid((unsigned)(b.tiles_x * b.tiles_y * a.T)), block(RWT * ROWS);
     if constexpr (ADAM) {
         hipLaunchKernelGGL((render_bwd_tile_k<COORD, BORDER, ORDER, RACT, AACT, ROWS, true, false, true, false, true, RWT>), grid, block, 0, s, b);
@@ -2049,7 +2133,6 @@
 
 template <bool BWD, int COORD, int BORDER, int ORDER, int RACT, int AACT, bool F16>
 int launch_t(const RenderArgs &a, hipStream_t s) {
-    dim3 grid((a.W + TILE_X - 1) / TILE_X, (a.H + TILE_Y - 1) / TILE_Y, a.T), block(TILE_X * TILE_Y);
     constexpr bool MASKABLE = COORD == VL3D_COORD_AFFINE && BORDER == VL3D_BORDER_HARDCUT && ORDER == VL3D_ACT_POST &&
                               RACT == VL3D_ACT_SIGMOID && AACT == VL3D_ACT_SIGMOID && !F16;
     if constexpr (BWD) {
@@ -2083,19 +2166,18 @@
 #undef VL3D_BWD_CASE
 #undef VL3D_CONV
             if (!go || c.f16 != F16) return bwd_not_built(c);
-            hipLaunchKernelGGL((bwd_plan_k<COORD>), dim3(1), dim3(64), 0, s, a, 16, const_cast<float *>(a.plan));
-            const size_t n8 = (size_t)a.D * a.T * a.Hs * a.Ws * (a.g_f16 ? 1 : 2);
-            hipLaunchKernelGGL(bwd_fill_zero_if_infeasible_k, dim3(4096), dim3(256), 0, s, reinterpret_cast<float2 *>(a.g_stack), n8, a.plan);
-            if (c.mask) hipLaunchKernelGGL(bwd_fill_zero_f32_if_infeasible_k, dim3(1024), dim3(256), 0, s, a.g_mask, (size_t)a.D * a.T * a.Hs * a.Ws, a.plan);
             go(a, s, c);
         }
+        const int tiles_x = (a.W + TILE_X - 1) / TILE_X, tiles_y = (a.H + TILE_Y - 1) / TILE_Y, nb = tiles_x * tiles_y * a.T;
+        const bool capped = c.family != VL3D_BWD_ATOMICS && !(a.ablate & BWD_PREPASS_UNLOOPED);
+        const dim3 grid((unsigned)(capped && nb > BWD_FALLBACK_BLOCKS ? BWD_FALLBACK_BLOCKS : nb)), block(TILE_X * TILE_Y);
         if constexpr (MASKABLE) {
             if (a.mask) {
-                hipLaunchKernelGGL((render_bwd_k<COORD, BORDER, ORDER, RACT, AACT, false, true>), grid, block, 0, s, a);
+                hipLaunchKernelGGL((render_bwd_k<COORD, BORDER, ORDER, RACT, AACT, false, true>), grid, block, 0, s, a, tiles_x, tiles_y);
                 return VL3D_OK;
             }
         }
-        hipLaunchKernelGGL((render_bwd_k<COORD, BORDER, ORDER, RACT, AACT, F16>), grid, block, 0, s, a);
+        hipLaunchKernelGGL((render_bwd_k<COORD, BORDER, ORDER, RACT, AACT, F16>), grid, block, 0, s, a, tiles_x, tiles_y);
         return VL3D_OK;
     } else {
         if (a.reg_fwd == 2) {
```
